# PearCoding/PearRay

Hardware: AMD Instinct MI355X
Metric: Msamples/s (higher is better)
Workload: dtype f32; 1 GPU; C4: Cornell box + 999968-triangle soup (1000000 triangles), 1920x1080, `direct` integrator (NEE+MIS+RR, depth 64), sobol 1024-spp schedule, hero wavelengths (spd CMIS), 308 iterations timed; parallelism=tiles1, collective=none (one rank)

## Files before the change

include/prgpu.h:

```cpp
#ifndef PRGPU_H
#define PRGPU_H

#include <stddef.h>
#include <stdint.h>

#ifdef __cplusplus
extern "C" {
#endif

#define PRGPU_API_VERSION 8
#define PRGPU_INVALID_ID 0xFFFFFFFFu

enum {
	PRGPU_OK          = 0,
	PRGPU_EINVAL      = -1,
	PRGPU_ENODEVICE   = -2,
	PRGPU_EDEVICE     = -3,
	PRGPU_EUNSUPPORTED = -4,
	PRGPU_EIO         = -5
};

enum { PRGPU_SPEC_CONST = 0, PRGPU_SPEC_PARAMETRIC = 1, PRGPU_SPEC_PARAMETRIC_SCALED = 2,
       PRGPU_SPEC_TABLE = 3, PRGPU_SPEC_MUL = 4, PRGPU_SPEC_SELLMEIER = 5, PRGPU_SPEC_CHECKER = 6 };

// ... 84 lines not shown
	float local_direction[3], local_right[3], local_up[3];
	float fstop, aperture_radius;
	uint32_t kind;
	float theta_start, theta_end, phi_start, phi_end;
	float fov;
	uint32_t fisheye_map;
	uint32_t clip_range;
	uint32_t reserved;
} prgpu_camera;

enum { PRGPU_SAMPLER_RANDOM = 0, PRGPU_SAMPLER_MJITT = 1, PRGPU_SAMPLER_SOBOL = 2, PRGPU_SAMPLER_HALTON = 3, PRGPU_SAMPLER_HAMMERSLEY = 4,
       PRGPU_SAMPLER_UNIFORM = 5,
       PRGPU_SAMPLER_STRATIFIED = 6 };
enum { PRGPU_MAPPER_SPD_CMIS = 0, PRGPU_MAPPER_RANDOM = 1, PRGPU_MAPPER_SPD_HERO = 2,
       PRGPU_MAPPER_CIE = 3,
       PRGPU_MAPPER_CIE_Y = 4,
       PRGPU_MAPPER_AGH_CMIS = 5,
       PRGPU_MAPPER_AGH_HERO = 6 };
enum { PRGPU_FILTER_BLOCK = 0, PRGPU_FILTER_TRIANGLE = 1, PRGPU_FILTER_GAUSSIAN = 2,
       PRGPU_FILTER_MITCHELL = 3, PRGPU_FILTER_LANCZOS = 4 };
enum { PRGPU_MIS_BALANCE = 0, PRGPU_MIS_POWER = 1 };

typedef struct prgpu_settings {
	uint32_t width, height;
	uint64_t seed;
	uint32_t aa_sampler;
	uint32_t aa_samples;
	uint32_t lens_samples, time_samples, spectral_samples;
	uint32_t mapper;
	uint32_t filter;
	uint32_t filter_radius;
	uint32_t max_ray_depth;
	uint32_t soft_max_ray_depth;
	uint32_t mis;
	uint32_t nee, direct, emissive_scatter;
	float    spectral_start, spectral_end;
	uint32_t spectral_hero;
	uint32_t spectral_mono;
	uint32_t aa_base_x, aa_base_y;
	uint32_t aa_burnin;
	uint32_t reserved;
} prgpu_settings;

typedef struct prgpu_scene_desc {
	uint32_t api_version;
	uint32_t n_vertices;
	const float*    positions;
	const float*    normals;
	const float*    uvs;
	uint32_t n_triangles;
	const uint32_t* indices;
	const uint32_t* tri_material;
	uint32_t n_entities;
	const prgpu_entity* entities;
	uint32_t n_materials;
	const prgpu_material* materials;
	uint32_t n_emissions;
	const prgpu_emission* emissions;
	uint32_t n_spectra;
	const prgpu_spectrum* spectra;
	uint32_t n_spectral_table_values;
	const float* spectral_tables;
	prgpu_camera   camera;
	prgpu_settings settings;
	uint32_t n_lights;
	const prgpu_light* lights;
} prgpu_scene_desc;

typedef struct prgpu_tile { uint32_t x0, y0, x1, y1; } prgpu_tile;

enum { PRGPU_STAT_CAMERA_RAYS = 0, PRGPU_STAT_LIGHT_RAYS, PRGPU_STAT_PRIMARY_RAYS, PRGPU_STAT_BOUNCE_RAYS,
       PRGPU_STAT_SHADOW_RAYS, PRGPU_STAT_MONOCHROME_RAYS, PRGPU_STAT_PIXEL_SAMPLES, PRGPU_STAT_ENTITY_HITS,
       PRGPU_STAT_BACKGROUND_HITS, PRGPU_STAT_CAMERA_DEPTH, PRGPU_STAT_LIGHT_DEPTH, PRGPU_STAT_COUNT };

typedef struct prgpu_trace_counters {
	uint64_t rays_closest, rays_any;
	uint64_t nodes_closest, leaves_closest;
	uint64_t nodes_any, leaves_any;
	uint32_t node_bytes, leaf_bytes;
	uint32_t ray_bytes, hit_bytes;
	uint64_t wave_steps_closest, wave_steps_any;
	uint64_t shade_batches, shade_lanes;
	uint64_t shade_ticks, idle_ticks, total_ticks;
} prgpu_trace_counters;

typedef struct prgpu_scene prgpu_scene;

const char* prgpu_last_error(void);
int  prgpu_device_count(void);
void prgpu_settings_default(prgpu_settings* s);

int  prgpu_rgb_to_coeffs(const float rgb[3], float coeffs[3]);
int  prgpu_write_rgb_coeff_table(const char* path, uint32_t resolution, int threads);

int  prgpu_scene_create(const prgpu_scene_desc* desc, int device, prgpu_scene** out);
void prgpu_scene_destroy(prgpu_scene* s);

int  prgpu_set_tiles(prgpu_scene* s, const prgpu_tile* tiles, uint32_t n_tiles);

int  prgpu_set_stream(prgpu_scene* s, void* hip_stream);

int  prgpu_bind_framebuffer(prgpu_scene* s, void* d_xyz, void* d_samples, void* d_feedback);

int  prgpu_render(prgpu_scene* s, uint32_t iter_begin, uint32_t iter_end);
int  prgpu_sync(prgpu_scene* s);

int  prgpu_download(prgpu_scene* s, float* xyz, uint32_t* samples, uint32_t* feedback);
int  prgpu_stats(prgpu_scene* s, uint64_t out[PRGPU_STAT_COUNT]);
int  prgpu_film_size(prgpu_scene* s, uint32_t* width, uint32_t* height);
int  prgpu_trace_counters_get(prgpu_scene* s, prgpu_trace_counters* out);
enum { PRGPU_KERNEL_NONE = 0, PRGPU_KERNEL_THROUGHPUT = 1, PRGPU_KERNEL_LATENCY = 2 };
typedef struct prgpu_pipeline_info {
	uint32_t mode;
	int32_t  shader_waves;
	float    shading_share;
	uint32_t calibration_launches;
	uint32_t kernel;
	uint32_t blocks, slots_per_block;
	uint64_t launches;
	uint32_t bvh_width;
	uint32_t bvh_top;
	uint32_t bvh_stack_bound;
	float    bvh_cost_4_wide, bvh_cost_6_wide;
} prgpu_pipeline_info;
int  prgpu_pipeline_info_get(prgpu_scene* s, prgpu_pipeline_info* out);
int  prgpu_set_instrumentation(prgpu_scene* s, int enabled);

int  prgpu_trace_closest(prgpu_scene* s, uint32_t n, const float* org, const float* dir,
                         const float* tmin, const float* tmax,
                         uint32_t* entity, uint32_t* prim, float* u, float* v, float* t);
int  prgpu_trace_any(prgpu_scene* s, uint32_t n, const float* org, const float* dir,
                     const float* tmin, const float* distance, uint8_t* occluded);

int  prgpu_download_primary_hits(prgpu_scene* s, uint32_t* entity, uint32_t* prim);

int  prgpu_set_timing(prgpu_scene* s, int enabled);
int  prgpu_kernel_time_ms(prgpu_scene* s, const char* family, double* total_ms, uint64_t* launches);

#define PRGPU_COMM_ID_BYTES 128
typedef struct prgpu_comm prgpu_comm;
int  prgpu_comm_unique_id(uint8_t id[PRGPU_COMM_ID_BYTES]);
int  prgpu_comm_create(const uint8_t id[PRGPU_COMM_ID_BYTES], int n_ranks, int rank, int device, prgpu_comm** out);
void prgpu_comm_destroy(prgpu_comm* comm);
int  prgpu_comm_size(const prgpu_comm* comm);
int  prgpu_comm_query(const prgpu_comm* comm, int* rccl_ranks, int* rccl_rank);
int  prgpu_reduce(prgpu_scene* s, prgpu_comm* comm, int root);
int  prgpu_reduced_planes(prgpu_scene* s, void** d_xyz, void** d_samples, void** d_feedback);

enum { PRGPU_AOV_POSITION = 0, PRGPU_AOV_NORMAL, PRGPU_AOV_NORMAL_G, PRGPU_AOV_TANGENT, PRGPU_AOV_BITANGENT, PRGPU_AOV_VIEW,
       PRGPU_AOV_ENTITY_ID, PRGPU_AOV_MATERIAL_ID, PRGPU_AOV_EMISSION_ID, PRGPU_AOV_DEPTH,
       PRGPU_AOV_COUNT };
int      prgpu_enable_aovs(prgpu_scene* s, uint32_t mask);
uint32_t prgpu_aov_channels(uint32_t aov);
int      prgpu_download_aov(prgpu_scene* s, uint32_t aov, float* out);
int prgpu_enable_variance(prgpu_scene* s);
int prgpu_download_variance(prgpu_scene* s, float* mean, float* variance);

#define PRGPU_LPE_MAX 4
#define PRGPU_LPE_MAX_STATES 32
int prgpu_lpe_check(const char* expression);
int prgpu_lpe_match(const char* expression, const uint8_t* symbols, uint32_t count);
int prgpu_enable_lpe(prgpu_scene* s, uint32_t n, const char* const* expressions);
int prgpu_download_lpe(prgpu_scene* s, uint32_t index, float* xyz);

int prgpu_enable_ambient_occlusion(prgpu_scene* s, uint32_t sample_count);
int prgpu_download_ao_counts(prgpu_scene* s, uint32_t* occluded);
int prgpu_download_ao_samples(prgpu_scene* s, uint64_t* rng_state, float* org, float* dir, uint8_t* occluded);

int prgpu_path_cost(prgpu_scene* s, uint32_t* vertices);
enum { PRGPU_TONE_SRGB = 0, PRGPU_TONE_XYZ = 1, PRGPU_TONE_XYZ_NORM = 2, PRGPU_TONE_LUMINANCE = 3 };
int prgpu_tonemap(uint32_t mode, float scale, const float* xyz, const float* weight, float* rgb, uint32_t out_elems, size_t pixel_count);
typedef struct prgpu_image_stats {
	uint64_t n;
	float min, min_ref, min_diff, max, max_ref, max_diff;
	float mean, mean_ref, mean_diff, mean_sqr, mean_sqr_ref;
	float mse, mape;
	uint64_t inf_count, nan_count;
} prgpu_image_stats;
int  prgpu_image_compare(const float* image, uint32_t image_stride, const float* reference, uint32_t reference_stride, uint32_t width,
                         uint32_t height, const uint32_t crop[4], prgpu_image_stats* out);
void prgpu_image_stats_merge(prgpu_image_stats* dst, const prgpu_image_stats* src);
enum { PRGPU_CHANNEL_SPECTRAL = 0, PRGPU_CHANNEL_3D = 1, PRGPU_CHANNEL_1D = 2, PRGPU_CHANNEL_COUNTER = 3 };
enum { PRGPU_SPECTRAL_OUTPUT = 0, PRGPU_SPECTRAL_ONLINE_MEAN = 1, PRGPU_SPECTRAL_ONLINE_VARIANCE = 2 };
enum { PRGPU_COUNTER_SAMPLES = 0, PRGPU_COUNTER_FEEDBACK = 1 };
typedef struct prgpu_output_channel {
	uint32_t file;
	uint32_t kind;
	uint32_t variable;
	uint32_t tone;
	char     name[64];
	char     lpe[64];
} prgpu_output_channel;
int prgpu_outputs_enable(prgpu_scene* s, const prgpu_output_channel* channels, uint32_t n_channels);
int prgpu_outputs_save(prgpu_scene* s, const prgpu_output_channel* channels, uint32_t n_channels, uint32_t file, const char* path);
int prgpu_write_exr(const char* path, uint32_t width, uint32_t height, uint32_t n_channels, const char* const* names,
                    const float* const* planes, const uint32_t* strides);

typedef struct prgpu_prc prgpu_prc;
typedef struct prgpu_prc_sky {
	const char*  light_name;
	const float* table;
	uint32_t     azimuth_count, elevation_count;
} prgpu_prc_sky;
typedef struct prgpu_prc_options {
	uint32_t width, height;
	uint32_t aa_samples;
// ... 33 lines not shown
```

pearray_amd/_cabi.py:

```python
import ctypes as C
import os

_HERE = os.path.dirname(os.path.abspath(__file__))
LIB_PATH = os.environ.get("PRGPU_LIBRARY") or os.path.join(_HERE, "csrc", "libprgpu.so")

PRGPU_API_VERSION = 8
INVALID_ID = 0xFFFFFFFF
COMM_ID_BYTES = 128

SPEC_CONST, SPEC_PARAMETRIC, SPEC_PARAMETRIC_SCALED, SPEC_TABLE, SPEC_MUL, SPEC_SELLMEIER, SPEC_CHECKER = range(7)
MAT_LAMBERT, MAT_DIELECTRIC, MAT_CONDUCTOR, MAT_ROUGH_CONDUCTOR, MAT_ROUGH_DIELECTRIC, MAT_PRINCIPLED, MAT_MIRROR = 0, 1, 2, 3, 4, 5, 6
MATF_ANISOTROPIC, MATF_NO_VNDF, MATF_HAS_TRANSMISSION = 1, 2, 4
PRINCIPLED_PARAMS = ("diffuse_transmission", "specular_transmission", "specular_tint", "anisotropic", "flatness", "metallic", "sheen",
                     "sheen_tint", "clearcoat", "clearcoat_gloss")
ENTITY_MESH, ENTITY_PLANE, ENTITY_SPHERE, ENTITY_QUADRIC = 0, 1, 2, 3
LIGHT_ENVIRONMENT, LIGHT_DISTANT, LIGHT_SKY, LIGHT_SUN, LIGHT_CIE_SKY = 0, 1, 2, 3, 4
ENVF_TEXTURED, ENVF_NO_DISTRIBUTION = 16, 32
SKYF_EXTEND, SKYF_COMPENSATION, SKYF_CLOUDY = 1, 2, 8
SKY_BANDS = 11
LPE_MAX, LPE_MAX_STATES = 4, 32
CAMERA_PERSPECTIVE, CAMERA_ORTHO, CAMERA_SPHERICAL, CAMERA_FISHEYE = 0, 1, 2, 3
FISHEYE_CIRCULAR, FISHEYE_CROPPED, FISHEYE_FULL = 0, 1, 2
AOV_NAMES = ("position", "normal", "normal_g", "tangent", "bitangent", "view", "entity_id", "material_id", "emission_id", "depth")
EMS_DIFFUSE = 0
SAMPLER_RANDOM, SAMPLER_MJITT, SAMPLER_SOBOL, SAMPLER_HALTON, SAMPLER_HAMMERSLEY, SAMPLER_UNIFORM, SAMPLER_STRATIFIED = range(7)
MAPPER_SPD_CMIS, MAPPER_RANDOM, MAPPER_SPD_HERO, MAPPER_CIE, MAPPER_CIE_Y, MAPPER_AGH_CMIS, MAPPER_AGH_HERO = range(7)
FILTER_BLOCK, FILTER_TRIANGLE, FILTER_GAUSSIAN, FILTER_MITCHELL, FILTER_LANCZOS = range(5)
MIS_BALANCE, MIS_POWER = range(2)
INTEGRATOR_DIRECT, INTEGRATOR_AO = range(2)

STAT_NAMES = ("camera_rays", "light_rays", "primary_rays", "bounce_rays", "shadow_rays", "monochrome_rays",
              "pixel_samples", "entity_hits", "background_hits", "camera_depth", "light_depth")
STAT_COUNT = len(STAT_NAMES)


class Spectrum(C.Structure):
    _fields_ = [("kind", C.c_uint32), ("p", C.c_float * 4), ("table_offset", C.c_uint32),
                ("table_count", C.c_uint32), ("wl_start", C.c_float), ("wl_end", C.c_float),
                ("lhs", C.c_uint32), ("rhs", C.c_uint32)]


class Material(C.Structure):
    _fields_ = [("kind", C.c_uint32), ("albedo", C.c_uint32), ("two_sided", C.c_uint32), ("ior", C.c_uint32),
                ("transmission", C.c_uint32), ("thin", C.c_uint32), ("k", C.c_uint32), ("flags", C.c_uint32),
                ("roughness_x", C.c_float), ("roughness_y", C.c_float), ("principled", C.c_float * 10)]


class Emission(C.Structure):
    _fields_ = [("kind", C.c_uint32), ("radiance", C.c_uint32)]


class Entity(C.Structure):
    _fields_ = [("first_tri", C.c_uint32), ("n_tris", C.c_uint32), ("emission", C.c_uint32),
                ("has_normals", C.c_uint32), ("kind", C.c_uint32), ("radius", C.c_float), ("has_uvs", C.c_uint32), ("params", C.c_uint32), ("transform", C.c_float * 16)]


class Light(C.Structure):
    _fields_ = [("kind", C.c_uint32), ("radiance", C.c_uint32), ("background", C.c_uint32), ("flags", C.c_uint32),
                ("direction", C.c_float * 3), ("cos_theta", C.c_float), ("transform", C.c_float * 16),
                ("table_offset", C.c_uint32), ("azimuth_count", C.c_uint32), ("elevation_count", C.c_uint32), ("ground_brightness", C.c_float)]


class Camera(C.Structure):
    _fields_ = [("transform", C.c_float * 16), ("width", C.c_float), ("height", C.c_float),
                ("near_t", C.c_float), ("far_t", C.c_float), ("local_direction", C.c_float * 3),
                ("local_right", C.c_float * 3), ("local_up", C.c_float * 3), ("fstop", C.c_float),
                ("aperture_radius", C.c_float), ("kind", C.c_uint32),
                ("theta_start", C.c_float), ("theta_end", C.c_float), ("phi_start", C.c_float), ("phi_end", C.c_float),
                ("fov", C.c_float), ("fisheye_map", C.c_uint32), ("clip_range", C.c_uint32), ("reserved", C.c_uint32)]


class Settings(C.Structure):
    _fields_ = [("width", C.c_uint32), ("height", C.c_uint32), ("seed", C.c_uint64),
                ("aa_sampler", C.c_uint32), ("aa_samples", C.c_uint32), ("lens_samples", C.c_uint32),
                ("time_samples", C.c_uint32), ("spectral_samples", C.c_uint32), ("mapper", C.c_uint32),
                ("filter", C.c_uint32), ("filter_radius", C.c_uint32), ("max_ray_depth", C.c_uint32),
                ("soft_max_ray_depth", C.c_uint32), ("mis", C.c_uint32), ("nee", C.c_uint32),
                ("direct", C.c_uint32), ("emissive_scatter", C.c_uint32), ("spectral_start", C.c_float),
                ("spectral_end", C.c_float), ("spectral_hero", C.c_uint32), ("spectral_mono", C.c_uint32),
                ("aa_base_x", C.c_uint32), ("aa_base_y", C.c_uint32), ("aa_burnin", C.c_uint32), ("reserved", C.c_uint32)]


class SceneDesc(C.Structure):
    _fields_ = [("api_version", C.c_uint32), ("n_vertices", C.c_uint32), ("positions", C.POINTER(C.c_float)),
                ("normals", C.POINTER(C.c_float)), ("uvs", C.POINTER(C.c_float)), ("n_triangles", C.c_uint32),
                ("indices", C.POINTER(C.c_uint32)), ("tri_material", C.POINTER(C.c_uint32)),
                ("n_entities", C.c_uint32), ("entities", C.POINTER(Entity)), ("n_materials", C.c_uint32),
                ("materials", C.POINTER(Material)), ("n_emissions", C.c_uint32),
                ("emissions", C.POINTER(Emission)), ("n_spectra", C.c_uint32), ("spectra", C.POINTER(Spectrum)),
                ("n_spectral_table_values", C.c_uint32), ("spectral_tables", C.POINTER(C.c_float)),
                ("camera", Camera), ("settings", Settings), ("n_lights", C.c_uint32), ("lights", C.POINTER(Light))]


class Tile(C.Structure):
    _fields_ = [("x0", C.c_uint32), ("y0", C.c_uint32), ("x1", C.c_uint32), ("y1", C.c_uint32)]


class TraceCounters(C.Structure):
    _fields_ = [("rays_closest", C.c_uint64), ("rays_any", C.c_uint64), ("nodes_closest", C.c_uint64),
                ("leaves_closest", C.c_uint64), ("nodes_any", C.c_uint64), ("leaves_any", C.c_uint64),
                ("node_bytes", C.c_uint32), ("leaf_bytes", C.c_uint32), ("ray_bytes", C.c_uint32),
                ("hit_bytes", C.c_uint32), ("wave_steps_closest", C.c_uint64), ("wave_steps_any", C.c_uint64),
                ("shade_batches", C.c_uint64), ("shade_lanes", C.c_uint64),
                ("shade_ticks", C.c_uint64), ("idle_ticks", C.c_uint64), ("total_ticks", C.c_uint64)]


class ImageStats(C.Structure):
    _fields_ = [("n", C.c_uint64), ("min", C.c_float), ("min_ref", C.c_float), ("min_diff", C.c_float), ("max", C.c_float),
                ("max_ref", C.c_float), ("max_diff", C.c_float), ("mean", C.c_float), ("mean_ref", C.c_float), ("mean_diff", C.c_float),
                ("mean_sqr", C.c_float), ("mean_sqr_ref", C.c_float), ("mse", C.c_float), ("mape", C.c_float),
                ("inf_count", C.c_uint64), ("nan_count", C.c_uint64)]


class OutputChannel(C.Structure):
    _fields_ = [("file", C.c_uint32), ("kind", C.c_uint32), ("variable", C.c_uint32), ("tone", C.c_uint32), ("name", C.c_char * 64),
                ("lpe", C.c_char * 64)]


CHANNEL_SPECTRAL, CHANNEL_3D, CHANNEL_1D, CHANNEL_COUNTER = range(4)
TONE_SRGB, TONE_XYZ, TONE_XYZ_NORM, TONE_LUMINANCE = range(4)


class PrcSky(C.Structure):
    _fields_ = [("light_name", C.c_char_p), ("table", C.POINTER(C.c_float)), ("azimuth_count", C.c_uint32), ("elevation_count", C.c_uint32)]


class PrcOptions(C.Structure):
    _fields_ = [("width", C.c_uint32), ("height", C.c_uint32), ("aa_samples", C.c_uint32), ("force_direct", C.c_uint32),
                ("seed", C.c_uint64), ("n_skies", C.c_uint32), ("reserved", C.c_uint32), ("skies", C.POINTER(PrcSky))]


def default_settings(width, height):
    s = Settings()
    s.width, s.height, s.seed = width, height, 42
    s.aa_sampler, s.aa_samples = SAMPLER_SOBOL, 128
    s.lens_samples = s.time_samples = s.spectral_samples = 1
    s.mapper, s.filter, s.filter_radius = MAPPER_SPD_CMIS, FILTER_MITCHELL, 1
    s.max_ray_depth, s.soft_max_ray_depth, s.mis = 64, 4, MIS_BALANCE
    s.nee = s.direct = s.emissive_scatter = 1
    s.spectral_start, s.spectral_end, s.spectral_hero, s.spectral_mono = 390.0, 830.0, 1, 0
    return s


class PipelineInfo(C.Structure):
    _fields_ = [("mode", C.c_uint32), ("shader_waves", C.c_int32), ("shading_share", C.c_float), ("calibration_launches", C.c_uint32),
                ("kernel", C.c_uint32), ("blocks", C.c_uint32), ("slots_per_block", C.c_uint32), ("launches", C.c_uint64),
                ("bvh_width", C.c_uint32), ("bvh_top", C.c_uint32), ("bvh_stack_bound", C.c_uint32), ("bvh_cost_4_wide", C.c_float), ("bvh_cost_6_wide", C.c_float)]


class SkyParams(C.Structure):
    _fields_ = [("sun_elevation", C.c_float), ("sun_azimuth", C.c_float), ("turbidity", C.c_float), ("albedo", C.c_float * 11)]


_VP, _U32P, _F32P, _U8P, _U64P = C.c_void_p, C.POINTER(C.c_uint32), C.POINTER(C.c_float), C.POINTER(C.c_uint8), C.POINTER(C.c_uint64)
SYMBOLS = {
    "prgpu_last_error": (C.c_char_p, []),
    "prgpu_device_count": (C.c_int, []),
    "prgpu_settings_default": (None, [C.POINTER(Settings)]),
    "prgpu_rgb_to_coeffs": (C.c_int, [_F32P, _F32P]),
    "prgpu_write_rgb_coeff_table": (C.c_int, [C.c_char_p, C.c_uint32, C.c_int]),
    "prgpu_scene_create": (C.c_int, [C.POINTER(SceneDesc), C.c_int, C.POINTER(_VP)]),
    "prgpu_scene_destroy": (None, [_VP]),
    "prgpu_set_tiles": (C.c_int, [_VP, C.POINTER(Tile), C.c_uint32]),
    "prgpu_set_stream": (C.c_int, [_VP, _VP]),
    "prgpu_bind_framebuffer": (C.c_int, [_VP, _VP, _VP, _VP]),
    "prgpu_render": (C.c_int, [_VP, C.c_uint32, C.c_uint32]),
    "prgpu_sync": (C.c_int, [_VP]),
    "prgpu_download": (C.c_int, [_VP, _F32P, _U32P, _U32P]),
    "prgpu_stats": (C.c_int, [_VP, _U64P]),
    "prgpu_trace_counters_get": (C.c_int, [_VP, C.POINTER(TraceCounters)]),
    "prgpu_set_instrumentation": (C.c_int, [_VP, C.c_int]),
    "prgpu_trace_closest": (C.c_int, [_VP, C.c_uint32, _F32P, _F32P, _F32P, _F32P, _U32P, _U32P, _F32P, _F32P, _F32P]),
    "prgpu_trace_any": (C.c_int, [_VP, C.c_uint32, _F32P, _F32P, _F32P, _F32P, _U8P]),
    "prgpu_download_primary_hits": (C.c_int, [_VP, _U32P, _U32P]),
    "prgpu_set_timing": (C.c_int, [_VP, C.c_int]),
    "prgpu_kernel_time_ms": (C.c_int, [_VP, C.c_char_p, C.POINTER(C.c_double), _U64P]),
    "prgpu_comm_unique_id": (C.c_int, [_U8P]),
    "prgpu_comm_create": (C.c_int, [_U8P, C.c_int, C.c_int, C.c_int, C.POINTER(_VP)]),
    "prgpu_comm_destroy": (None, [_VP]),
    "prgpu_comm_size": (C.c_int, [_VP]),
    "prgpu_comm_query": (C.c_int, [_VP, C.POINTER(C.c_int), C.POINTER(C.c_int)]),
    "prgpu_reduced_planes": (C.c_int, [_VP, C.POINTER(_VP), C.POINTER(_VP), C.POINTER(_VP)]),
    "prgpu_pipeline_info_get": (C.c_int, [_VP, C.POINTER(PipelineInfo)]),
    "prgpu_reduce": (C.c_int, [_VP, _VP, C.c_int]),
    "prgpu_film_size": (C.c_int, [_VP, _U32P, _U32P]),
    "prgpu_enable_variance": (C.c_int, [_VP]),
    "prgpu_download_variance": (C.c_int, [_VP, _F32P, _F32P]),
    "prgpu_path_cost": (C.c_int, [_VP, _U32P]),
    "prgpu_enable_ambient_occlusion": (C.c_int, [_VP, C.c_uint32]),
    "prgpu_download_ao_counts": (C.c_int, [_VP, _U32P]),
    "prgpu_download_ao_samples": (C.c_int, [_VP, _U64P, _F32P, _F32P, _U8P]),
    "prgpu_lpe_check": (C.c_int, [C.c_char_p]),
    "prgpu_lpe_match": (C.c_int, [C.c_char_p, _U8P, C.c_uint32]),
    "prgpu_enable_lpe": (C.c_int, [_VP, C.c_uint32, C.POINTER(C.c_char_p)]),
    "prgpu_download_lpe": (C.c_int, [_VP, C.c_uint32, _F32P]),
    "prgpu_image_compare": (C.c_int, [_F32P, C.c_uint32, _F32P, C.c_uint32, C.c_uint32, C.c_uint32, _U32P, C.POINTER(ImageStats)]),
    "prgpu_image_stats_merge": (None, [C.POINTER(ImageStats), C.POINTER(ImageStats)]),
    "prgpu_tonemap": (C.c_int, [C.c_uint32, C.c_float, _F32P, _F32P, _F32P, C.c_uint32, C.c_size_t]),
    "prgpu_outputs_enable": (C.c_int, [_VP, C.POINTER(OutputChannel), C.c_uint32]),
    "prgpu_outputs_save": (C.c_int, [_VP, C.POINTER(OutputChannel), C.c_uint32, C.c_uint32, C.c_char_p]),
    "prgpu_prc_outputs": (C.POINTER(OutputChannel), [_VP, _U32P]),
    "prgpu_prc_output_name": (C.c_char_p, [_VP, C.c_uint32]),
    "prgpu_enable_aovs": (C.c_int, [_VP, C.c_uint32]),
    "prgpu_aov_channels": (C.c_uint32, [C.c_uint32]),
    "prgpu_download_aov": (C.c_int, [_VP, C.c_uint32, _F32P]),
    "prgpu_write_exr": (C.c_int, [C.c_char_p, C.c_uint32, C.c_uint32, C.c_uint32, C.POINTER(C.c_char_p), C.POINTER(_F32P), _U32P]),
    "prgpu_sun_position": (None, [C.c_int] * 5 + [C.c_float] * 4 + [_F32P, _F32P]),
    "prgpu_sun_radiance": (C.c_float, [C.c_float] * 3),
    "prgpu_sky_table": (C.c_int, [C.c_float, C.c_float, C.c_float, _F32P, C.c_uint32, C.c_uint32, _F32P]),
    "prgpu_prc_sky_info": (C.c_int, [_VP, C.c_uint32, C.POINTER(SkyParams)]),
    "prgpu_prc_load_file": (C.c_int, [C.c_char_p, C.POINTER(PrcOptions), C.POINTER(_VP)]),
    "prgpu_prc_load_string": (C.c_int, [C.c_char_p, C.c_char_p, C.POINTER(PrcOptions), C.POINTER(_VP)]),
    "prgpu_prc_desc": (C.POINTER(SceneDesc), [_VP]),
    "prgpu_prc_warnings": (C.c_char_p, [_VP]),
    "prgpu_prc_integrator": (C.c_int, [_VP, _U32P, _U32P]),
    "prgpu_prc_last_error": (C.c_char_p, []),
    "prgpu_prc_free": (None, [_VP]),
}

_lib = None


def load():
    global _lib
    if _lib is not None:
        return _lib
    if not os.path.exists(LIB_PATH):
        raise ImportError("HIP backend %s not built -- run `python -c 'import __graft_entry__ as g; g.build()'` "
                          "(there is no CPU fallback)" % LIB_PATH)
    lib = C.CDLL(LIB_PATH)
# ... 15 lines not shown
```

pearray_amd/backend.py:

```python
import ctypes as C
import os

import numpy as np

from . import _cabi as abi


def _f32p(a):
    return a.ctypes.data_as(C.POINTER(C.c_float))


def _u32p(a):
    return a.ctypes.data_as(C.POINTER(C.c_uint32))


class RenderContext:

    def __init__(self, scene, device=0):
        self.lib = abi.load()
        self.scene = scene
        self._h = C.c_void_p()
        abi.check(self.lib.prgpu_scene_create(C.byref(scene.desc), int(device), C.byref(self._h)))
        self.width, self.height = scene.width, scene.height
        self.iterations_done = 0
        self.ao_sample_count = 0
        if getattr(scene, "integrator", abi.INTEGRATOR_DIRECT) == abi.INTEGRATOR_AO:
            self.enableAmbientOcclusion(scene.ao_sample_count)

    def close(self):
        if self._h:
            self.lib.prgpu_scene_destroy(self._h)
            self._h = C.c_void_p()

    def __del__(self):
        try:
            self.close()
        except Exception:
            pass

    def setTiles(self, tiles):
        tiles = list(tiles)
        arr = (abi.Tile * max(1, len(tiles)))(*[abi.Tile(*t) for t in tiles])
        abi.check(self.lib.prgpu_set_tiles(self._h, arr, len(tiles)))

    def setStream(self, stream_handle):
        abi.check(self.lib.prgpu_set_stream(self._h, C.c_void_p(stream_handle)))

    def bindFramebuffer(self, xyz_ptr, samples_ptr, feedback_ptr=None):
        abi.check(self.lib.prgpu_bind_framebuffer(self._h, C.c_void_p(xyz_ptr), C.c_void_p(samples_ptr),
                                                  C.c_void_p(feedback_ptr) if feedback_ptr else None))

    def reduce(self, comm, root=0):
        abi.check(self.lib.prgpu_reduce(self._h, comm._h, int(root)))

    def reducedPlanes(self):
        x, s, f = C.c_void_p(), C.c_void_p(), C.c_void_p()
        rc = self.lib.prgpu_reduced_planes(self._h, C.byref(x), C.byref(s), C.byref(f))
        if rc < 0:
            abi.check(rc)
        return (x.value, s.value, f.value) if rc == 1 else None

    def pipelineInfo(self):
        info = abi.PipelineInfo()
        abi.check(self.lib.prgpu_pipeline_info_get(self._h, C.byref(info)))
        out = {f: getattr(info, f) for f, _ in info._fields_}
        out["kernel"] = {0: "none", 1: "throughput", 2: "latency"}.get(out["kernel"], str(out["kernel"]))
        return out

    def setInstrumentation(self, on):
        abi.check(self.lib.prgpu_set_instrumentation(self._h, 1 if on else 0))

    def setTiming(self, on):
        abi.check(self.lib.prgpu_set_timing(self._h, 1 if on else 0))

    def render(self, iterations):
        b = self.iterations_done
        abi.check(self.lib.prgpu_render(self._h, b, b + int(iterations)))
        self.iterations_done = b + int(iterations)

    def start(self):
        self.render(self.scene.spp - self.iterations_done)

    def waitForFinish(self):
        abi.check(self.lib.prgpu_sync(self._h))

    def statistics(self):
        out = (C.c_uint64 * abi.STAT_COUNT)()
        abi.check(self.lib.prgpu_stats(self._h, out))
        return {n: int(out[i]) for i, n in enumerate(abi.STAT_NAMES)}

    def traceCounters(self):
        tc = abi.TraceCounters()
        abi.check(self.lib.prgpu_trace_counters_get(self._h, C.byref(tc)))
        return {f: int(getattr(tc, f)) for f, _ in tc._fields_}

    def kernelTime(self, family):
        ms, n = C.c_double(), C.c_uint64()
        abi.check(self.lib.prgpu_kernel_time_ms(self._h, family.encode(), C.byref(ms), C.byref(n)))
        return ms.value, int(n.value)

    def output(self):
        n = self.width * self.height
        xyz = np.empty(n * 3, dtype=np.float32)
        smp = np.empty(n, dtype=np.uint32)
        fb = np.empty(n, dtype=np.uint32)
        abi.check(self.lib.prgpu_download(self._h, _f32p(xyz), _u32p(smp), _u32p(fb)))
        return xyz.reshape(self.height, self.width, 3), smp.reshape(self.height, self.width), fb.reshape(self.height, self.width)

    def enableAOVs(self, names):
        mask = 0
        for n in names:
            mask |= 1 << abi.AOV_NAMES.index(n)
        abi.check(self.lib.prgpu_enable_aovs(self._h, mask))

    def enableVariance(self):
        abi.check(self.lib.prgpu_enable_variance(self._h))

    def variance(self):
        n = self.width * self.height * 3
        mean, var = np.empty(n, np.float32), np.empty(n, np.float32)
        abi.check(self.lib.prgpu_download_variance(self._h, _f32p(mean), _f32p(var)))
        return mean.reshape(self.height, self.width, 3), var.reshape(self.height, self.width, 3)

    def enableLPE(self, expressions):
        arr = (C.c_char_p * max(1, len(expressions)))(*[e.encode() for e in expressions])
        abi.check(self.lib.prgpu_enable_lpe(self._h, len(expressions), arr))

    def lpe(self, index):
        out = np.empty(self.width * self.height * 3, dtype=np.float32)
        abi.check(self.lib.prgpu_download_lpe(self._h, int(index), _f32p(out)))
        return out.reshape(self.height, self.width, 3)

    def enableAmbientOcclusion(self, sample_count):
        abi.check(self.lib.prgpu_enable_ambient_occlusion(self._h, int(sample_count)))
        self.ao_sample_count = int(sample_count)

    def aoCounts(self):
        out = np.empty(self.width * self.height, dtype=np.uint32)
        abi.check(self.lib.prgpu_download_ao_counts(self._h, _u32p(out)))
        return out.reshape(self.height, self.width)

    def aoSamples(self):
        n, k = self.width * self.height, self.ao_sample_count
        state = np.empty(n, dtype=np.uint64)
        org, direction = np.empty(n * k * 3, dtype=np.float32), np.empty(n * k * 3, dtype=np.float32)
        occ = np.empty(n * k, dtype=np.uint8)
        abi.check(self.lib.prgpu_download_ao_samples(self._h, state.ctypes.data_as(C.POINTER(C.c_uint64)), _f32p(org), _f32p(direction),
                                                     occ.ctypes.data_as(C.POINTER(C.c_uint8))))
# ... 187 lines not shown
```

pearray_amd/csrc/device/bvh.h:

```cpp
#pragma once
#include <string>
#include <vector>

#include "pr_device.h"

namespace prd {
struct BvhBuildInput {
	uint32_t n_tris, n_entities;
	const float* positions;
	const uint32_t* indices;
	const uint32_t* tri_entity;
	const DevEntity* entities;
	const uint8_t* tri_class = nullptr;
	uint32_t stack_capacity = 0xFFFFFFFFu;
	int width = 0;
	int top = -1;
	int parity = -1;
};
struct BvhBuildOutput {
	Rec64* recs = nullptr;
	uint32_t* leaf_units = nullptr;
	uint32_t n_inner = 0, n_leaf = 0, n_units = 0;
	uint32_t stack_bound = 0;
	int top = 0;
	bool wide = false;
	float cost4 = 0.0f, cost6 = 0.0f;
};
bool build_lbvh(const BvhBuildInput& in, BvhBuildOutput& out, hipStream_t stream, std::string& err);
}
```

pearray_amd/csrc/device/bvh.hip:

```cpp
#include "bvh.h"

#include <hipcub/hipcub.hpp>
#include <algorithm>
#include <cstring>

namespace prd {
namespace {

__device__ __forceinline__ uint32_t float_to_ordered(float f)
{
	const uint32_t b = __float_as_uint(f);
	return (b & 0x80000000u) ? ~b : (b | 0x80000000u);
}
__device__ __forceinline__ float ordered_to_float(uint32_t u)
{
	return __uint_as_float((u & 0x80000000u) ? (u & 0x7FFFFFFFu) : ~u);
}

__global__ void k_world_tris(uint32_t n, const float* __restrict__ positions, const uint32_t* __restrict__ indices,
							 const uint32_t* __restrict__ tri_entity, const DevEntity* __restrict__ entities,
							 float4* __restrict__ wv, uint32_t* __restrict__ ebounds )
{
	const uint32_t t = blockIdx.x * blockDim.x + threadIdx.x;
	if (t >= n)
// ... 259 lines not shown
	if (width <= 0) {
		for (int side = 0; side < 2; ++side) {
			const int c = side == 0 ? left[i] : right[i];
			bool expandable;
			const ChildRef direct = make_child(c, expandable, wv, sorted_tri, range_first, range_last, boxes, inner_idx, leaf_idx);
			if (!expandable || (width < 0 && i == 0)) {
				tmp[nc++] = direct;
			} else {
				bool e2;
				tmp[nc++] = make_child(left[c], e2, wv, sorted_tri, range_first, range_last, boxes, inner_idx, leaf_idx);
				tmp[nc++] = make_child(right[c], e2, wv, sorted_tri, range_first, range_last, boxes, inner_idx, leaf_idx);
			}
		}
	} else {
		bool ex[MAX_WIDE];
		tmp[0] = make_child(left[i], ex[0], wv, sorted_tri, range_first, range_last, boxes, inner_idx, leaf_idx);
		tmp[1] = make_child(right[i], ex[1], wv, sorted_tri, range_first, range_last, boxes, inner_idx, leaf_idx);
		nc	   = 2;
		while (nc < width) {
			int best	= -1;
			float bestA = -1.0f;
			for (int k = 0; k < nc; ++k) {
				const float A = half_area(tmp[k]);
				if (ex[k] && (A > bestA || (A == bestA && tmp[k].count > tmp[best].count))) {
					best  = k;
					bestA = A;
				}
			}
			if (best < 0)
				break;
			const int c = tmp[best].node;
			for (int k = nc; k > best + 1; --k) {
				tmp[k] = tmp[k - 1];
				ex[k]  = ex[k - 1];
			}
			tmp[best]	  = make_child(left[c], ex[best], wv, sorted_tri, range_first, range_last, boxes, inner_idx, leaf_idx);
			tmp[best + 1] = make_child(right[c], ex[best + 1], wv, sorted_tri, range_first, range_last, boxes, inner_idx, leaf_idx);
			++nc;
		}
	}
	int n = 0;
	for (int k = 0; k < nc; ++k)
		if (tmp[k].leaf)
			ch[n++] = tmp[k];
	for (int k = 0; k < nc; ++k)
		if (!tmp[k].leaf)
			ch[n++] = tmp[k];
	return nc;
}
__global__ void k_area_sum(int n, const uint32_t* __restrict__ flag, const float* __restrict__ boxes, double* __restrict__ sum)
{
	const int i = blockIdx.x * blockDim.x + threadIdx.x;
	double a	= 0.0;
	if (i < n - 1 && flag[i]) {
		const double dx = (double)boxes[6 * i + 3] - boxes[6 * i], dy = (double)boxes[6 * i + 4] - boxes[6 * i + 1], dz = (double)boxes[6 * i + 5] - boxes[6 * i + 2];
		a				= dx * dy + dy * dz + dz * dx;
	}
	for (int o = 32; o > 0; o >>= 1)
		a += __shfl_down(a, o, 64);
	if ((threadIdx.x & 63) == 0 && a != 0.0)
		atomicAdd(sum, a);
}
__global__ void k_mark_records(int n_front, const int* __restrict__ front, int width, const float4* __restrict__ wv, const uint32_t* __restrict__ sorted_tri,
							   const int* __restrict__ left, const int* __restrict__ right, const int* __restrict__ range_first, const int* __restrict__ range_last,
							   const float* __restrict__ boxes, uint32_t* __restrict__ inner_flag, int* __restrict__ next, uint32_t* __restrict__ n_next,
							   uint32_t* __restrict__ stack_bound , uint32_t* __restrict__ max_stack_bound)
{
	const int t = blockIdx.x * blockDim.x + threadIdx.x;
	if (t >= n_front)
		return;
	ChildRef ch[MAX_WIDE];
	const int nc = gather_children(front[t], ch, width, wv, sorted_tri, left, right, range_first, range_last, boxes, inner_flag , inner_flag);
	const uint32_t below = stack_bound[front[t]] + (uint32_t)(nc - 1);
	atomicMax(max_stack_bound, below);
	for (int k = 0; k < nc; ++k)
		if (!ch[k].leaf) {
			inner_flag[ch[k].node]		= 1u;
			stack_bound[ch[k].node]		= below;
			next[atomicAdd(n_next, 1u)] = ch[k].node;
		}
}

constexpr double GRID_MARGIN = 1.0 / 16384.0;
__device__ void write_inner_q(Rec64* __restrict__ rec, const ChildRef* ch, int nc, uint32_t base_unit, const uint32_t* offs)
{
	float org[3];
	uint32_t ebyte[3];
	uint32_t qlo[3][MAX_WIDE], qhi[3][MAX_WIDE];
	for (int a = 0; a < 3; ++a) {
		float lo = INFINITY, hi = -INFINITY;
		for (int k = 0; k < nc; ++k) {
			lo = fminf(lo, ch[k].lo[a]);
			hi = fmaxf(hi, ch[k].hi[a]);
		}
		const float ext_eff = (hi - lo) + 4.0f * fmaxf(fabsf(lo), fabsf(hi)) * 1.1920929e-7f;
		int e				= (int)fminf(fmaxf((float)ilogbf(fmaxf(ext_eff * (1.0f / 255.0f), 1e-30f)), -100.0f), 30.0f);
		bool fits			= false;
		float o				= lo;
		for (; e <= 30 && !fits; ++e) {
			const double s = ldexp(1.0, e), m = s * GRID_MARGIN;
			o = (float)((double)lo - m);
			if ((double)o > (double)lo - m)
				o = nextafterf(o, -INFINITY);
			fits = true;
			for (int k = 0; k < nc; ++k) {
				const double want_lo = (double)ch[k].lo[a] - m, want_hi = (double)ch[k].hi[a] + m;
				double ql = floor((want_lo - (double)o) / s);
				ql		  = ql < 0.0 ? 0.0 : (ql > 255.0 ? 255.0 : ql);
				while (ql > 0.0 && (double)o + ql * s > want_lo)
					ql -= 1.0;
				double qh = ceil((want_hi - (double)o) / s);
				qh		  = qh < 0.0 ? 0.0 : qh;
				while (qh <= 255.0 && (double)o + qh * s < want_hi)
					qh += 1.0;
				if (qh > 255.0 || (double)o + ql * s > want_lo) {
					fits = false;
					break;
				}
				qlo[a][k] = (uint32_t)ql;
				qhi[a][k] = (uint32_t)qh;
			}
		}
		--e;
		if (!fits)
			for (int k = 0; k < nc; ++k) {
				qlo[a][k] = 0u;
				qhi[a][k] = 255u;
			}
		org[a]	 = o;
		ebyte[a] = (uint32_t)(e + 127);
	}
	uint32_t w[16];
	for (int k = 0; k < 16; ++k)
		w[k] = 0u;
	w[0] = __float_as_uint(org[0]);
	w[1] = __float_as_uint(org[1]);
	w[2] = __float_as_uint(org[2]);
	w[3] = ebyte[0] | (ebyte[1] << 8) | (ebyte[2] << 16);
	for (int k = 0; k < 4; ++k) {
		const bool used = k < nc;
		for (int a = 0; a < 3; ++a) {
			const uint32_t l = used ? qlo[a][k] : 255u, h = used ? qhi[a][k] : 0u;
			w[4 + a] |= l << (8 * k);
			w[7 + a] |= h << (8 * k);
		}
		const int src = used ? k : 0;
		w[11] |= ((offs[src] << REC_UNIT_SHIFT) | (ch[src].leaf ? REC_LEAF_BIT : 0u)) << (8 * k);
	}
	w[10]	   = base_unit << REC_UNIT_SHIFT;
	for (int k = 4; k < 6; ++k) {
		const bool used = k < nc;
		const int j		= k - 4;
		const uint32_t lx = used ? qlo[0][k] : 255u, ly = used ? qlo[1][k] : 255u, lz = used ? qlo[2][k] : 255u;
		const uint32_t hx = used ? qhi[0][k] : 0u, hy = used ? qhi[1][k] : 0u, hz = used ? qhi[2][k] : 0u;
		w[12] |= (lx << (8 * j)) | (ly << (16 + 8 * j));
		w[13] |= (hx << (8 * j)) | (hy << (16 + 8 * j));
		w[14] |= (lz << (8 * j)) | (hz << (16 + 8 * j));
		const int src = used ? k : 0;
		w[15] |= ((offs[src] << REC_UNIT_SHIFT) | (ch[src].leaf ? REC_LEAF_BIT : 0u)) << (8 * j);
	}
	uint4* dst = reinterpret_cast<uint4*>(rec);
	for (int q = 0; q < 4; ++q)
		dst[q] = make_uint4(w[4 * q], w[4 * q + 1], w[4 * q + 2], w[4 * q + 3]);
}

__global__ void k_group_sizes(int n, int width, const float4* __restrict__ wv, const uint32_t* __restrict__ sorted_tri, const int* __restrict__ left,
							  const int* __restrict__ right, const int* __restrict__ range_first, const int* __restrict__ range_last,
							  const float* __restrict__ boxes, const uint32_t* __restrict__ inner_flag, const uint32_t* __restrict__ inner_idx,
							  const uint32_t* __restrict__ leaf_idx, uint32_t* __restrict__ gsize)
{
	const int i = blockIdx.x * blockDim.x + threadIdx.x;
	if (i >= n - 1 || !inner_flag[i])
		return;
	ChildRef ch[MAX_WIDE];
	const int nc = gather_children(i, ch, width, wv, sorted_tri, left, right, range_first, range_last, boxes, inner_idx, leaf_idx);
	uint32_t units = 0;
	for (int k = 0; k < nc; ++k)
		units += ch[k].leaf ? 2u : 1u;
	gsize[inner_idx[i]] = (units + 1u) & ~1u;
}
__global__ void k_assign_units(int n, int width, const float4* __restrict__ wv, const uint32_t* __restrict__ sorted_tri, const int* __restrict__ left,
							   const int* __restrict__ right, const int* __restrict__ range_first, const int* __restrict__ range_last,
							   const float* __restrict__ boxes, const uint32_t* __restrict__ inner_flag, const uint32_t* __restrict__ inner_idx,
							   const uint32_t* __restrict__ leaf_idx, const uint32_t* __restrict__ gbase, uint32_t* __restrict__ inner_unit,
							   uint32_t* __restrict__ leaf_unit)
{
	const int i = blockIdx.x * blockDim.x + threadIdx.x;
	if (i >= n - 1 || !inner_flag[i])
		return;
	if (i == 0)
		inner_unit[inner_idx[0]] = 0u;
	ChildRef ch[MAX_WIDE];
	const int nc  = gather_children(i, ch, width, wv, sorted_tri, left, right, range_first, range_last, boxes, inner_idx, leaf_idx);
	uint32_t unit = 2u + gbase[inner_idx[i]];
	for (int k = 0; k < nc; ++k) {
		if (ch[k].leaf)
			leaf_unit[ch[k].id] = unit;
		else
			inner_unit[ch[k].id] = unit;
		unit += ch[k].leaf ? 2u : 1u;
	}
}
__global__ void k_emit_inner(int n, int width, const float4* __restrict__ wv, const uint32_t* __restrict__ sorted_tri, const int* __restrict__ left,
							 const int* __restrict__ right, const int* __restrict__ range_first, const int* __restrict__ range_last,
							 const float* __restrict__ boxes, const uint32_t* __restrict__ inner_flag, const uint32_t* __restrict__ inner_idx,
							 const uint32_t* __restrict__ leaf_idx, const uint32_t* __restrict__ gbase, const uint32_t* __restrict__ inner_unit,
							 Rec64* __restrict__ recs)
{
	const int i = blockIdx.x * blockDim.x + threadIdx.x;
	if (i >= n - 1 || !inner_flag[i])
		return;
	ChildRef ch[MAX_WIDE];
	const int nc = gather_children(i, ch, width, wv, sorted_tri, left, right, range_first, range_last, boxes, inner_idx, leaf_idx);
	uint32_t offs[MAX_WIDE] = { 0u, 0u, 0u, 0u, 0u, 0u }, off = 0u;
	for (int k = 0; k < nc; ++k) {
		offs[k] = off;
		off += ch[k].leaf ? 2u : 1u;
	}
	write_inner_q(recs + inner_unit[inner_idx[i]], ch, nc, 2u + gbase[inner_idx[i]], offs);
}

__global__ void k_validate(uint32_t n_inner, const uint32_t* __restrict__ inner_unit, const Rec64* __restrict__ recs, uint32_t n_units, uint32_t* __restrict__ bad)
{
	const uint32_t i = blockIdx.x * blockDim.x + threadIdx.x;
	if (i >= n_inner)
		return;
	const uint32_t unit = inner_unit[i];
	if (unit >= n_units) {
		atomicAdd(bad, 1u);
		return;
	}
	const uint32_t* w	= reinterpret_cast<const uint32_t*>(recs + unit);
	const uint32_t base = w[10], pw = w[11];
	bool ok				= (base & 3u) == 0u && base >= (2u << REC_UNIT_SHIFT);
	for (int a = 0; a < 3 && ok; ++a) {
		const uint32_t e = (w[3] >> (8 * a)) & 0xFFu;
		ok				 = e >= 27u && e <= 157u;
	}
	for (int k = 0; k < MAX_WIDE && ok; ++k) {
		const uint32_t ref = base + (((k < 4 ? pw : w[15]) >> (8 * (k & 3))) & 0xFFu), cu = ref >> REC_UNIT_SHIFT;
		ok				   = ok && (ref & 2u) == 0u;
		if (ref & REC_LEAF_BIT) {
			ok = (cu & 1u) == 0u && cu + 2u <= n_units;
			if (ok) {
				const uint32_t cnt = reinterpret_cast<const uint32_t*>(recs + cu)[30];
				ok				   = cnt >= 1u && cnt <= 3u;
			}
		} else {
			ok = cu + 1u <= n_units;
			if (ok) {
				const uint32_t ce = reinterpret_cast<const uint32_t*>(recs + cu)[3] & 0xFFu;
				ok				  = ce >= 27u && ce <= 157u;
			}
		}
	}
	if (!ok)
		atomicAdd(bad, 1u);
}

__global__ void k_emit_leaves(uint32_t n, const float4* __restrict__ wv, const uint32_t* __restrict__ sorted_tri, const uint32_t* __restrict__ leaf_flag,
							  const uint32_t* __restrict__ leaf_count, const uint32_t* __restrict__ leaf_idx, const uint32_t* __restrict__ leaf_unit, Rec64* __restrict__ recs,
							  const uint8_t* __restrict__ tri_class)
{
	const uint32_t pos = blockIdx.x * blockDim.x + threadIdx.x;
	if (pos >= n || !leaf_flag[pos])
		return;
	const uint32_t cnt = leaf_count[pos];
	float f[32];
	for (int k = 0; k < 32; ++k)
		f[k] = 0.0f;
	uint32_t classes = 0u;
	for (uint32_t k = 0; k < cnt; ++k) {
		const uint32_t t = sorted_tri[pos + k];
		classes |= (tri_class ? (uint32_t)tri_class[t] : 0u) << (8u * k);
		if (wv[3 * t].w != 0.0f) {
			const float4 c = wv[3 * t + 2];
			f[10 * k]	   = c.x;
			f[10 * k + 1]  = c.y;
			f[10 * k + 2]  = c.z;
			f[10 * k + 3]  = c.w;
			f[10 * k + 9]  = __uint_as_float(t | PRIM_SPHERE_BIT);
			continue;
		}
		for (int v = 0; v < 3; ++v) {
			const float4 p		 = wv[3 * t + v];
			f[10 * k + 3 * v]	 = p.x;
			f[10 * k + 3 * v + 1] = p.y;
			f[10 * k + 3 * v + 2] = p.z;
		}
		f[10 * k + 9] = __uint_as_float(t);
	}
	f[30]		= __uint_as_float(cnt);
	f[31]		= __uint_as_float(classes);
	float4* dst = reinterpret_cast<float4*>(recs + leaf_unit[leaf_idx[pos]]);
	for (int q = 0; q < 8; ++q)
		dst[q] = make_float4(f[4 * q], f[4 * q + 1], f[4 * q + 2], f[4 * q + 3]);
}

__global__ void k_tiny_scene(uint32_t n, const float4* __restrict__ wv, const uint32_t* __restrict__ sorted_tri, Rec64* __restrict__ recs, uint32_t* __restrict__ leaf_unit,
							 const uint8_t* __restrict__ tri_class)
{
	if (blockIdx.x != 0 || threadIdx.x != 0)
		return;
	float lo[3] = { INFINITY, INFINITY, INFINITY }, hi[3] = { -INFINITY, -INFINITY, -INFINITY };
	float leaf[32];
	for (int k = 0; k < 32; ++k)
		leaf[k] = 0.0f;
	uint32_t classes = 0u;
	for (uint32_t i = 0; i < n; ++i) {
		float a[3], b[3];
		const uint32_t t = sorted_tri[i];
		classes |= (tri_class ? (uint32_t)tri_class[t] : 0u) << (8u * i);
		tri_box(wv, t, a, b);
		for (int k = 0; k < 3; ++k) {
			lo[k] = fminf(lo[k], a[k]);
			hi[k] = fmaxf(hi[k], b[k]);
		}
		if (wv[3 * t].w != 0.0f) {
			const float4 c	 = wv[3 * t + 2];
			leaf[10 * i]	 = c.x;
			leaf[10 * i + 1] = c.y;
			leaf[10 * i + 2] = c.z;
			leaf[10 * i + 3] = c.w;
			leaf[10 * i + 9] = __uint_as_float(t | PRIM_SPHERE_BIT);
			continue;
		}
		for (int v = 0; v < 3; ++v) {
			const float4 p		  = wv[3 * t + v];
			leaf[10 * i + 3 * v]	  = p.x;
			leaf[10 * i + 3 * v + 1] = p.y;
			leaf[10 * i + 3 * v + 2] = p.z;
		}
		leaf[10 * i + 9] = __uint_as_float(t);
	}
	leaf[30] = __uint_as_float(n);
	leaf[31] = __uint_as_float(classes);
	pad_box(lo, hi);
	ChildRef only;
	for (int a = 0; a < 3; ++a) {
		only.lo[a] = lo[a];
		only.hi[a] = hi[a];
	}
	only.leaf			 = true;
	only.id				 = 0u;
	const uint32_t off0[4] = { 0u, 0u, 0u, 0u };
	write_inner_q(recs, &only, 1, 2u, off0);
	leaf_unit[0] = 2u;
	float4* d1	 = reinterpret_cast<float4*>(recs + 2);
	for (int q = 0; q < 8; ++q)
		d1[q] = make_float4(leaf[4 * q], leaf[4 * q + 1], leaf[4 * q + 2], leaf[4 * q + 3]);
}

#define HIPC(x)                                  \
	do {                                         \
		hipError_t _e = (x);                     \
		if (_e != hipSuccess) {                  \
			err = std::string(#x) + ": " + hipGetErrorString(_e); \
			goto done;                           \
		}                                        \
	} while (0)

}

namespace {
struct EntityBox {
	float lo[3], hi[3];
	double weight;
	uint32_t id;
};
void entity_codes_split(std::vector<EntityBox>& set, size_t first, size_t count, uint32_t prefix, int bits_left, std::vector<uint32_t>& code)
{
	if (count == 1 || bits_left == 0) {
		for (size_t k = 0; k < count; ++k)
			code[set[first + k].id] = prefix;
		return;
	}
	const size_t cap = size_t(1) << (bits_left - 1);
	double best_cost = INFINITY;
	int best_axis	 = 0;
	size_t best_left = count / 2;
	std::vector<double> right_area(count), right_weight(count);
	for (int axis = 0; axis < 3; ++axis) {
		std::sort(set.begin() + first, set.begin() + first + count,
				  [axis](const EntityBox& a, const EntityBox& b) { return a.lo[axis] + a.hi[axis] < b.lo[axis] + b.hi[axis] || (a.lo[axis] + a.hi[axis] == b.lo[axis] + b.hi[axis] && a.id < b.id); });
		auto area = [](const float* lo, const float* hi) {
			const double dx = (double)hi[0] - lo[0], dy = (double)hi[1] - lo[1], dz = (double)hi[2] - lo[2];
			return dx * dy + dy * dz + dz * dx;
		};
		float lo[3] = { INFINITY, INFINITY, INFINITY }, hi[3] = { -INFINITY, -INFINITY, -INFINITY };
		double w = 0.0;
		for (size_t k = count; k-- > 1;) {
			for (int a = 0; a < 3; ++a) {
				lo[a] = std::min(lo[a], set[first + k].lo[a]);
				hi[a] = std::max(hi[a], set[first + k].hi[a]);
			}
			w += set[first + k].weight;
			right_area[k]	= area(lo, hi);
			right_weight[k] = w;
		}
		for (int a = 0; a < 3; ++a) {
			lo[a] = INFINITY;
			hi[a] = -INFINITY;
		}
		w = 0.0;
		for (size_t k = 1; k < count; ++k) {
			for (int a = 0; a < 3; ++a) {
				lo[a] = std::min(lo[a], set[first + k - 1].lo[a]);
				hi[a] = std::max(hi[a], set[first + k - 1].hi[a]);
			}
			w += set[first + k - 1].weight;
			if (k > cap || count - k > cap)
				continue;
			const double cost = area(lo, hi) * w + right_area[k] * right_weight[k];
			if (cost < best_cost) {
				best_cost = cost;
				best_axis = axis;
				best_left = k;
			}
		}
	}
	size_t heavy = 0;
	for (size_t k = 1; k < count; ++k)
		if (set[first + k].weight > set[first + heavy].weight)
			heavy = k;
	{
		auto area = [](const float* lo, const float* hi) {
			const double dx = (double)hi[0] - lo[0], dy = (double)hi[1] - lo[1], dz = (double)hi[2] - lo[2];
// ... 192 lines not shown
				const uint32_t one = 1u;
				const int root	   = 0;
				HIPC(hipMemcpyAsync(greedy_flag, &one, 4, hipMemcpyHostToDevice, stream));
				HIPC(hipMemcpyAsync(front, &root, 4, hipMemcpyHostToDevice, stream));
				uint32_t n_front = 1u;
				while (n_front != 0u) {
					HIPC(hipMemsetAsync(front_count, 0, sizeof(uint32_t), stream));
					hipLaunchKernelGGL(k_mark_records, dim3((n_front + B - 1) / B), dim3(B), 0, stream, (int)n_front, front, MAX_WIDE, wv, vals_sorted, left, right, rf, rl, boxes,
									   greedy_flag, front_next, front_count, stack_bound, bounds_dev + 2);
					HIPC(hipMemcpyAsync(&n_front, front_count, 4, hipMemcpyDeviceToHost, stream));
					HIPC(hipStreamSynchronize(stream));
					std::swap(front, front_next);
				}
				hipLaunchKernelGGL(k_area_sum, dim3(G), dim3(B), 0, stream, (int)n, greedy_flag, boxes, area_sums + 2);
			}
			{
				double sums[3] = { 0.0, 0.0, 0.0 };
				float root_box[6];
				hipLaunchKernelGGL(k_area_sum, dim3(G), dim3(B), 0, stream, (int)n, inner_flag, boxes, area_sums);
				hipLaunchKernelGGL(k_area_sum, dim3(G), dim3(B), 0, stream, (int)n, odd_flag, boxes, area_sums + 1);
				HIPC(hipMemcpyAsync(bounds_host, bounds_dev, sizeof(bounds_host), hipMemcpyDeviceToHost, stream));
				HIPC(hipMemcpyAsync(sums, area_sums, sizeof(sums), hipMemcpyDeviceToHost, stream));
				HIPC(hipMemcpyAsync(root_box, boxes, sizeof(root_box), hipMemcpyDeviceToHost, stream));
				HIPC(hipStreamSynchronize(stream));
				const double rx = (double)root_box[3] - root_box[0], ry = (double)root_box[4] - root_box[1], rz = (double)root_box[5] - root_box[2];
				const double ra = std::max(rx * ry + ry * rz + rz * rx, 1e-300);
				const uint32_t bound_even = 3u * (bounds_host[0] + 1u), bound_odd = 3u * (bounds_host[1] + 1u), bound6 = bounds_host[2];
				const bool fit_even = bound_even <= in.stack_capacity, fit_odd = bound_odd <= in.stack_capacity;
				const bool odd = in.parity >= 0 ? in.parity == 1 : fit_odd && (!fit_even || sums[1] < sums[0]);
				const uint32_t bound4 = odd ? bound_odd : bound_even;
				if (in.parity >= 0 && in.width != 6 && bound4 > in.stack_capacity) {
					err = "the four-wide BVH of the forced parity is " + std::to_string(bound4) + " stack entries deep in the worst case, the traversal stack holds "
						  + std::to_string(in.stack_capacity);
					goto done;
				}
				if (odd) {
					width = -1;
					std::swap(inner_flag, odd_flag);
				}
				out.cost4		= (float)(sums[odd ? 1 : 0] / ra);
				out.stack_bound = bound4;
				if (in.width != 4) {
					out.cost6 = (float)(sums[2] / ra);
					const bool fit4 = bound4 <= in.stack_capacity, fit6 = bound6 <= in.stack_capacity;
					const bool cheaper6 = (double)out.cost6 * WIDE_STEP_COST < (double)out.cost4;
					if (in.width == 6 || (cheaper6 ? (fit6 || !fit4) : (!fit4 && fit6))) {
						out.stack_bound = bound6;
						width			= MAX_WIDE;
						out.wide		= true;
						std::swap(inner_flag, greedy_flag);
					}
				}
			}
			{
				const double cost = out.stack_bound > in.stack_capacity ? INFINITY
																		: (out.wide ? (double)out.cost6 * WIDE_STEP_COST : (double)out.cost4);
				if (pass < n_orders && (pass == 0 ? cost < best_cost : cost < 0.98 * first_cost && cost < best_cost)) {
					best_cost  = cost;
					best_order = order;
				}
				if (pass == 0)
					first_cost = cost;
				if (top_forced)
					break;
				if (pass + 1 < n_orders) {
					order = pass + 1;
					continue;
				}
				if (pass + 1 == n_orders && best_order != order) {
					order = best_order;
					continue;
				}
				break;
			}
		}
		if (n <= 3) {
			HIPC(hipMalloc(&out.recs, sizeof(Rec64) * 4));
			HIPC(hipMemsetAsync(out.recs, 0, sizeof(Rec64) * 4, stream));
			HIPC(hipMalloc(&out.leaf_units, sizeof(uint32_t)));
			hipLaunchKernelGGL(k_tiny_scene, dim3(1), dim3(64), 0, stream, n, wv, vals_sorted, out.recs, out.leaf_units, in.tri_class);
			out.n_inner = 1;
			out.n_leaf	= 1;
			out.n_units = 4;
		} else {
			HIPC(hipcub::DeviceScan::ExclusiveSum(nullptr, t2a, inner_flag, inner_idx, (int)n, stream));
			HIPC(hipcub::DeviceScan::ExclusiveSum(nullptr, t2b, leaf_flag, leaf_idx, (int)n, stream));
			temp2_bytes = std::max(t2a, t2b);
			HIPC(hipMalloc(&temp2, temp2_bytes));
			HIPC(hipcub::DeviceScan::ExclusiveSum(temp2, temp2_bytes, inner_flag, inner_idx, (int)n, stream));
			HIPC(hipcub::DeviceScan::ExclusiveSum(temp2, temp2_bytes, leaf_flag, leaf_idx, (int)n, stream));
			uint32_t last[4] = { 0, 0, 0, 0 };
			HIPC(hipMemcpyAsync(&last[0], inner_idx + (n - 1), 4, hipMemcpyDeviceToHost, stream));
			HIPC(hipMemcpyAsync(&last[1], inner_flag + (n - 1), 4, hipMemcpyDeviceToHost, stream));
			HIPC(hipMemcpyAsync(&last[2], leaf_idx + (n - 1), 4, hipMemcpyDeviceToHost, stream));
			HIPC(hipMemcpyAsync(&last[3], leaf_flag + (n - 1), 4, hipMemcpyDeviceToHost, stream));
			HIPC(hipStreamSynchronize(stream));
			if (out.stack_bound > in.stack_capacity) {
				err = "the BVH of this scene is " + std::to_string(out.stack_bound) + " stack entries deep in the worst case, the traversal stack holds "
					  + std::to_string(in.stack_capacity);
				goto done;
			}
			out.n_inner = last[0] + last[1];
			out.n_leaf	= last[2] + last[3];
			HIPC(hipMalloc(&gsize, sizeof(uint32_t) * (size_t(out.n_inner) + 1)));
			HIPC(hipMalloc(&gbase, sizeof(uint32_t) * (size_t(out.n_inner) + 1)));
			HIPC(hipMalloc(&inner_unit, sizeof(uint32_t) * std::max<size_t>(out.n_inner, 1)));
			HIPC(hipMalloc(&out.leaf_units, sizeof(uint32_t) * std::max<size_t>(out.n_leaf, 1)));
			HIPC(hipMemsetAsync(gsize, 0, sizeof(uint32_t) * (size_t(out.n_inner) + 1), stream));
			hipLaunchKernelGGL(k_group_sizes, dim3(G), dim3(B), 0, stream, (int)n, width, wv, vals_sorted, left, right, rf, rl, boxes, inner_flag, inner_idx, leaf_idx, gsize);
			HIPC(hipGetLastError());
			{
				size_t t3 = 0;
				HIPC(hipcub::DeviceScan::ExclusiveSum(nullptr, t3, gsize, gbase, (int)out.n_inner + 1, stream));
				if (t3 > temp2_bytes) {
					(void)hipFree(temp2);
					temp2 = nullptr;
					HIPC(hipMalloc(&temp2, t3));
					temp2_bytes = t3;
				}
				HIPC(hipcub::DeviceScan::ExclusiveSum(temp2, temp2_bytes, gsize, gbase, (int)out.n_inner + 1, stream));
			}
			uint32_t group_units = 0;
			HIPC(hipMemcpyAsync(&group_units, gbase + out.n_inner, 4, hipMemcpyDeviceToHost, stream));
			HIPC(hipStreamSynchronize(stream));
			out.n_units = 2u + group_units;
			if (size_t(out.n_units) >= (size_t(1) << 30)) {
				err = "the BVH needs more than 2^30 record units";
				goto done;
			}
			HIPC(hipMalloc(&out.recs, sizeof(Rec64) * size_t(out.n_units)));
			HIPC(hipMemsetAsync(out.recs, 0, sizeof(Rec64) * size_t(out.n_units), stream));
			hipLaunchKernelGGL(k_assign_units, dim3(G), dim3(B), 0, stream, (int)n, width, wv, vals_sorted, left, right, rf, rl, boxes, inner_flag, inner_idx, leaf_idx, gbase,
							   inner_unit, out.leaf_units);
			hipLaunchKernelGGL(k_emit_inner, dim3(G), dim3(B), 0, stream, (int)n, width, wv, vals_sorted, left, right, rf, rl, boxes, inner_flag, inner_idx, leaf_idx, gbase,
							   inner_unit, out.recs);
			hipLaunchKernelGGL(k_emit_leaves, dim3(G), dim3(B), 0, stream, n, wv, vals_sorted, leaf_flag, leaf_cnt, leaf_idx, out.leaf_units, out.recs, in.tri_class);
			HIPC(hipGetLastError());
			{
				uint32_t bad = 0;
				HIPC(hipMemsetAsync(gsize, 0, sizeof(uint32_t), stream));
				hipLaunchKernelGGL(k_validate, dim3((out.n_inner + B - 1) / B), dim3(B), 0, stream, out.n_inner, inner_unit, out.recs, out.n_units, gsize);
				HIPC(hipMemcpyAsync(&bad, gsize, 4, hipMemcpyDeviceToHost, stream));
				HIPC(hipStreamSynchronize(stream));
				if (bad != 0u) {
					err = "internal error: " + std::to_string(bad) + " inner records failed the structure check";
					goto done;
				}
			}
		}
		HIPC(hipGetLastError());
		HIPC(hipStreamSynchronize(stream));
		ok = true;
	}
done:
	(void)hipFree(wv); (void)hipFree(ebounds); (void)hipFree(entity_rank); (void)hipFree(keys); (void)hipFree(keys_sorted); (void)hipFree(vals); (void)hipFree(vals_sorted);
	(void)hipFree(left); (void)hipFree(right); (void)hipFree(rf); (void)hipFree(rl); (void)hipFree(parent); (void)hipFree(boxes); (void)hipFree(arrive);
	(void)hipFree(inner_flag); (void)hipFree(inner_idx); (void)hipFree(leaf_flag); (void)hipFree(leaf_cnt); (void)hipFree(leaf_idx);
	(void)hipFree(front); (void)hipFree(front_next); (void)hipFree(front_count); (void)hipFree(area_sums); (void)hipFree(greedy_flag); (void)hipFree(stack_bound); (void)hipFree(bounds_dev); (void)hipFree(odd_flag);
	(void)hipFree(temp); (void)hipFree(temp2); (void)hipFree(gsize); (void)hipFree(gbase); (void)hipFree(inner_unit);
	if (!ok) {
		(void)hipFree(out.recs);
		(void)hipFree(out.leaf_units);
		out.recs	   = nullptr;
		out.leaf_units = nullptr;
	}
	return ok;
}

}
```

pearray_amd/csrc/device/pr_device.h:

```cpp
#pragma once

#include <hip/hip_runtime.h>
#include <stdint.h>

#include "../../../include/prgpu.h"

#ifndef PR_INLINE_CLOSURES
#define PR_INLINE_CLOSURES 0
#endif

#if PR_INLINE_CLOSURES
#define PR_CLOSURE __forceinline__
#else
#define PR_CLOSURE __noinline__
#endif

namespace prd {

constexpr float PR_EPS		= 1.1920928955078125e-7f;
constexpr float PR_INV_PI_F = 0.31830988618379067154f;
constexpr float PR_PI_F	  = 3.14159265358979323846f;
constexpr uint32_t INVALID	= PRGPU_INVALID_ID;
constexpr float SHADOW_RAY_MIN = 0.0001f;
constexpr float BOUNCE_RAY_MIN = 0.0001f;
constexpr float DISTANCE_EPS   = 1e-5f;
constexpr float GEOMETRY_EPS   = 1e-5f;
constexpr float PDF_EPS		   = 1e-6f;
constexpr int CIE_SAMPLES	   = 441;
constexpr float CIE_START	   = 390.0f;
constexpr float CIE_END		   = 830.0f;
constexpr float CIE_Y_NORM_SUM = 113.042314572337f;
constexpr float CIE_RANGE	   = CIE_END - CIE_START;
constexpr float CIE_DELTA	   = CIE_RANGE / (CIE_SAMPLES - 1);
constexpr float CIE_Y_NORM	   = CIE_Y_NORM_SUM * CIE_DELTA;

struct __attribute__((aligned(64))) Rec64 {
	float4 q[4];
};
static_assert(sizeof(Rec64) == 64, "Rec64 must be 64 bytes");
constexpr uint32_t REC_LEAF_BIT = 1u;
constexpr uint32_t REC_EMPTY	= 0xFFFFFFFFu;
constexpr uint32_t REC_UNIT_SHIFT = 2u;
__host__ __device__ __forceinline__ const float4* rec_ptr(const Rec64* recs, uint32_t ref)
{
	return reinterpret_cast<const float4*>(reinterpret_cast<const char*>(recs) + (size_t(ref & ~3u) << 4));
}
constexpr float SLAB_REL		= 1.0000028610229492f;
constexpr float INV_D_MAX		= 1.2089258196146292e24f;
constexpr float SCENE_COORD_MAX = 268435456.0f;

struct DevEntity {
	float m[12];
	float nm[9];
	uint32_t first_tri, n_tris, emission, has_normals;
	float vol_scale, world_area;
	uint32_t light_id, kind;
	float sphere_r;
	uint32_t has_uvs;
};

constexpr uint32_t FEAT_DELTA_MATERIALS = 1u, FEAT_INFINITE_LIGHTS = 2u, FEAT_PLANES = 4u, FEAT_SPHERES = 8u, FEAT_AOVS = 16u, FEAT_SHAPE_LIGHTS = 32u, FEAT_TEXTURES = 64u,
				   FEAT_ROUGH_MATERIALS = 128u, FEAT_LPE = 256u, FEAT_QUADRICS = 512u, FEAT_ALL = 1023u;

struct DevQuadric {
	float p[10];
	float lo[3], hi[3];
	float wlo[3], whi[3];
	float inv[12];
	uint32_t tri;
	uint32_t entity;
};

struct DevShapeLight {
	float S[3], Ex[3], Ey[3], Ez[3], nrm[3];
	float width, height;
	float inv[12];
	float pdf_cache;
	float radius;
	float pad[2];
};
struct __attribute__((aligned(128))) DevLight {
	float m[12];
	float nm[9];
	uint32_t entity, kind, n_tris, tri_offset;
	uint32_t has_normals, radiance;
	float vol_scale;
	prgpu_spectrum node, lhs, rhs;
	uint32_t pad[3];
};
static_assert(sizeof(DevLight) == 256, "DevLight must be two 128-byte lines");
struct __attribute__((aligned(128))) DevMaterial {
	prgpu_material m;
	prgpu_spectrum albedo;
};
static_assert(sizeof(DevMaterial) == 128, "DevMaterial must be one 128-byte line");
constexpr uint32_t LIGHT_TRI_FLOATS = 20;
constexpr uint32_t PRIM_SPHERE_BIT = 0x40000000u;

struct DevInfLight {
	uint32_t kind, radiance, background, flags;
	float nm[9], inv_nm[9];
	float outgoing[3];
	float dx[3], dy[3];
	float cos_theta, cone_pdf;
	uint32_t table_offset, az_count, el_count;
	uint32_t dist_offset, dist_w, dist_h;
	float ground_brightness;
};
constexpr int SKY_BANDS			 = PRGPU_SKY_BANDS;
constexpr float SKY_BAND_START	 = 320.0f;
constexpr float SKY_BAND_DELTA	 = 40.0f;
constexpr float ELEVATION_RANGE = PR_PI_F * 0.5f;
constexpr float AZIMUTH_RANGE	 = PR_PI_F * 2;

struct DevCamera {
	float o[3], right[3], up[3], focal[3], xap[3], yap[3];
	float near_t, far_t;
	uint32_t dof, ortho;
	uint32_t kind;
	float angles[4];
	float fov, xaspect, yaspect;
	uint32_t clip;
};

struct DevScene {
	const Rec64* recs;
	uint32_t n_tris, n_inner, n_leaf;
	uint32_t bvh_wide;
	const float* positions;
// ... 1192 lines not shown
```

pearray_amd/csrc/device/render.h:

```cpp
#pragma once
#include "pr_device.h"

namespace prd {
constexpr int N_DEVICE_COUNTERS = PRGPU_STAT_COUNT + 30;

struct TraceWorkspace {
	uint32_t* queue_head = nullptr;
	uint2* spill		 = nullptr;
	uint32_t max_blocks	 = 0;
	int refill_below	 = 44;
	uint32_t* bl_list	 = nullptr;
	uint32_t* bl_word	 = nullptr;
	uint32_t* slot_unit	 = nullptr;
	size_t bl_entries	 = 0;
};
size_t trace_workspace_spill_entries(uint32_t max_blocks);
uint32_t trace_stack_capacity();

void launch_raygen(const DevScene& sc, const PathState& ps, uint32_t slot_base, uint32_t n_slots, uint32_t iter, unsigned long long* gstats, hipStream_t st);
void launch_trace_closest(const DevScene& sc, const PathState& ps, const uint32_t* active, uint32_t slot_base, uint32_t n_active, bool count,
						  const TraceWorkspace& ws, uint32_t* shade_counters, unsigned long long* gstats, hipStream_t st);
void launch_shade(const DevScene& sc, const PathState& ps, const uint32_t* active, uint32_t slot_base, uint32_t n_active, uint32_t* next_active,
				  uint32_t* counters, uint32_t* dead_list, uint32_t* queue_head_closest, uint32_t* queue_head_shadow, unsigned long long* gstats,
				  hipStream_t st);
void launch_regen(const DevScene& sc, const PathState& ps, const uint32_t* dead, uint32_t n_dead, uint32_t iter_end, uint32_t* next_active,
				  uint32_t* counters, unsigned long long* gstats, hipStream_t st);
void launch_trace_shadow(const DevScene& sc, const PathState& ps, uint32_t n_items, bool count, const TraceWorkspace& ws, unsigned long long* gstats,
						 hipStream_t st);
struct PersistentGeometry {
	uint32_t n_blocks, slots_per_block;
};
PersistentGeometry persistent_geometry(uint32_t n_owned, uint32_t max_blocks, uint32_t max_slots_per_block);
uint32_t persistent_slot_padding();
uint32_t slot_array_padding();
uint32_t persistent_block_threads();
int shade_ticks_counter();
struct PersistentTuning {
	uint32_t slots	  = 384;
	int shade_min	  = 64;
	int shade_partial = 16;
	int fin_batch	  = 16;
	int occupancy	  = 3;
	int shader_wave	  = -1;
	bool resident	  = true;
};
void launch_path_persistent(const DevScene& sc, const PathState& ps, const uint32_t* owned, uint32_t n_owned, uint32_t iter_begin, uint32_t iter_end,
							bool count, const TraceWorkspace& ws, const PersistentTuning& tune, int shader_waves , uint32_t* next_pixel, uint32_t* error,
							unsigned long long* gstats, hipStream_t st);
struct LatencyGeometry {
	uint32_t n_blocks, slots_per_wave, total_slots;
};
struct LatencyTuning {
	uint32_t slots_per_wave = 256;
	int shade_min			= 48;
	int refill_below		= 40;
};
LatencyGeometry latency_geometry(uint32_t n_owned, uint32_t max_blocks_throughput, uint32_t max_slots_per_wave);
bool latency_variant_built(uint32_t features);
void launch_path_latency(const DevScene& sc, const PathState& ps, const uint32_t* owned, uint32_t n_owned, uint32_t iter_begin, uint32_t iter_end, bool count,
						 const TraceWorkspace& ws, const LatencyTuning& tune, uint32_t* error, unsigned long long* gstats, hipStream_t st);
void launch_resolve(const DevScene& sc, const PathState& ps, uint32_t iter, hipStream_t st);
size_t sort_active_temp_bytes(uint32_t n_max);
void launch_sort_active(const DevScene& sc, const PathState& ps, const uint32_t* active, uint32_t n, uint32_t* keys_in, uint32_t* keys_out, uint32_t* active_out,
						void* temp, size_t temp_bytes, hipStream_t st);
void launch_service_closest(const DevScene& sc, uint32_t n, const float* org, const float* dir, const float* tmin, const float* tmax,
							uint32_t* entity, uint32_t* prim, float* u, float* v, float* t, const TraceWorkspace& ws, unsigned long long* gstats,
							hipStream_t st);
void launch_tri_slot(const DevScene& sc, const uint32_t* leaf_units , uint32_t* tri_slot, hipStream_t st);
void launch_service_closest_split(const DevScene& sc, uint32_t n, const float* org, const float* dir, const float* tmin, const float* tmax,
								  uint32_t* entity, uint32_t* prim, float* u, float* v, float* t, const TraceWorkspace& ws, uint32_t* tri_slot,
								  unsigned long long* gstats, hipStream_t st);
void launch_service_any(const DevScene& sc, uint32_t n, const float* org, const float* dir, const float* tmin, const float* distance,
						uint8_t* occluded, const TraceWorkspace& ws, unsigned long long* gstats, hipStream_t st);
struct AoState {
	float4* rec;
	uint32_t* occluded;
	const uint64_t* jump;
	uint32_t* counts;
	uint64_t jump_all;
	uint32_t sample_count;
	uint64_t* dbg_state;
	float* dbg_org;
	float* dbg_dir;
	uint8_t* dbg_occluded;
};

void launch_ao_hits(const DevScene& sc, const PathState& ps, const AoState& ao, uint32_t n_slots, bool instrumented, uint32_t* n_hits, uint32_t* queue_head_closest,
// ... 7 lines not shown
```

pearray_amd/csrc/device/render.hip:

```cpp
#ifndef PR_TU
#error "compile with -DPR_TU=0..5 or 11..15 (see the Makefile)"
#endif
#include "render.h"

#include <algorithm>
#if PR_TU == 0
#include <hipcub/hipcub.hpp>
#endif

namespace prd {

__device__ __forceinline__ unsigned long long lane_ballot(bool p) { return __builtin_amdgcn_ballot_w64(p); }
__device__ __forceinline__ bool lane_in(unsigned long long m) { return __builtin_amdgcn_inverse_ballot_w64(m); }
__device__ __forceinline__ int wave_popc(unsigned long long m)
{
	int n = __builtin_popcountll(m);
	asm volatile("" : "+s"(n));
	return n;
}

struct Hit {
	float t, u, v;
	uint32_t tri;
};

enum { CNT_NODES_CLOSEST = PRGPU_STAT_COUNT, CNT_TRIS_CLOSEST, CNT_NODES_ANY, CNT_TRIS_ANY, CNT_WAVE_ITERS_CLOSEST, CNT_WAVE_ITERS_ANY, CNT_SHADE_BATCHES, CNT_SHADE_LANES, CNT_SHADE_TICKS, CNT_IDLE_TICKS, CNT_TOTAL_TICKS, CNT_LEAF_TICKS, CNT_INNER_TICKS, CNT_TOTAL_CYCLES, CNT_REFILL_TICKS, CNT_FIN_TICKS, CNT_CAMERA_TICKS, CNT_VERTEX_TICKS,
	   CNT_CLS_TICKS0, CNT_CLS_BATCHES0 = CNT_CLS_TICKS0 + 4, CNT_CLS_LANES0 = CNT_CLS_BATCHES0 + 4 };

#ifndef PR_PEEK
#define PR_PEEK 0
#endif
#ifndef PR_PL_VARIANTS
#define PR_PL_VARIANTS 31
#endif
#ifndef PR_PP_BLOCK
#define PR_PP_BLOCK 256
#endif
constexpr int PP_BLOCK		= PR_PP_BLOCK;
constexpr int TRAV_BLOCK	= PR_TU >= 1 ? PP_BLOCK : 256;
constexpr int STACK_LDS		= 16;
constexpr int STACK_SPILL	= 64;

struct Stack {
	uint2* lds;
	uint2* spill;
	uint32_t spill_stride;
	int sp, base;
	__device__ __forceinline__ void reset() { sp = base = 0; }
	__device__ __forceinline__ void reserve(int k)
	{
		while (sp - base + k > STACK_LDS) {
			if (base < STACK_SPILL)
				spill[(uint32_t)base * spill_stride] = lds[(base & (STACK_LDS - 1)) * TRAV_BLOCK];
			++base;
		}
	}
	__device__ __forceinline__ void push_if(bool valid, uint32_t ref, uint32_t key)
	{
		lds[(sp & (STACK_LDS - 1)) * TRAV_BLOCK] = make_uint2(ref, key);
		sp += valid ? 1 : 0;
	}
	__device__ __forceinline__ uint2 peek() const { return lds[((sp - 1) & (STACK_LDS - 1)) * TRAV_BLOCK]; }
	__device__ __forceinline__ uint2 pop_peeked(uint2 top)
	{
		--sp;
		if (__builtin_expect(sp < base, 0)) {
			base = sp;
			top	 = make_uint2(REC_EMPTY, 0x7F800000u);
			if (sp < STACK_SPILL)
				top = spill[(uint32_t)sp * spill_stride];
		}
		return top;
	}
	__device__ __forceinline__ uint2 pop()
	{
		--sp;
		uint2 e = lds[(sp & (STACK_LDS - 1)) * TRAV_BLOCK];
		if (__builtin_expect(sp < base, 0)) {
			base = sp;
			e	 = make_uint2(REC_EMPTY, 0x7F800000u);
			if (sp < STACK_SPILL)
				e = spill[(uint32_t)sp * spill_stride];
		}
		return e;
	}
};
static_assert((STACK_LDS & (STACK_LDS - 1)) == 0, "STACK_LDS must be a power of two");

struct Trav {
	RayPre r;
	float tmin;
	Hit best;
	uint32_t cur;
	bool any;
	uint32_t cls;
};

enum { MODE_CLOSEST = 0, MODE_ANY = 1, MODE_MIXED = 2 };

template <typename STK>
__device__ __forceinline__ void trav_begin(Trav& s, STK& st, V3 o, V3 d, float tmin, float tmax, float eps_t)
{
	s.r	   = ray_prepare(o, d, eps_t);
	s.tmin = tmin + 0.0f;
	s.best = Hit{ tmax, 0.0f, 0.0f, INVALID };
	s.cur  = 0u;
	s.any  = false;
	s.cls  = 0u;
	st.reset();
}
// ... 13 lines not shown
			s.cur = e.x;
	}
}

#define PR_UB(w, k) ((float)(((w) >> (8 * (k))) & 0xFFu))
__device__ __forceinline__ void inner_keys(const Trav& s, const float4& q0, const float4& q1, const float4& q2, const float4& q3, bool wide, uint32_t key[6])
{
	const uint32_t eb = __float_as_uint(q0.w);
	const float sx = __uint_as_float((eb & 0xFFu) << 23), sy = __uint_as_float(((eb >> 8) & 0xFFu) << 23), sz = __uint_as_float(((eb >> 16) & 0xFFu) << 23);
	const bool nx = s.r.inv_d.x < 0.0f, ny = s.r.inv_d.y < 0.0f, nz = s.r.inv_d.z < 0.0f;
	const uint32_t wlx = __float_as_uint(q1.x), wly = __float_as_uint(q1.y), wlz = __float_as_uint(q1.z);
	const uint32_t whx = __float_as_uint(q1.w), why = __float_as_uint(q2.x), whz = __float_as_uint(q2.y);
	const uint32_t wnx = nx ? whx : wlx, wfx = nx ? wlx : whx, wny = ny ? why : wly, wfy = ny ? wly : why, wnz = nz ? whz : wlz, wfz = nz ? wlz : whz;
	const float Ax = sx * s.r.inv_d.x, Ay = sy * s.r.inv_d.y, Az = sz * s.r.inv_d.z;
	const float Bx = (q0.x - s.r.o.x) * s.r.inv_d.x, By = (q0.y - s.r.o.y) * s.r.inv_d.y, Bz = (q0.z - s.r.o.z) * s.r.inv_d.z;
	const uint32_t pw = __float_as_uint(q2.w);
#pragma unroll
	for (int k = 0; k < 4; ++k) {
		const float axk = __fmaf_rn(PR_UB(wnx, k), Ax, Bx), bxk = __fmaf_rn(PR_UB(wfx, k), Ax, Bx);
		const float ayk = __fmaf_rn(PR_UB(wny, k), Ay, By), byk = __fmaf_rn(PR_UB(wfy, k), Ay, By);
		const float azk = __fmaf_rn(PR_UB(wnz, k), Az, Bz), bzk = __fmaf_rn(PR_UB(wfz, k), Az, Bz);
		const float t0 = fmaxf(fmaxf(axk, ayk), fmaxf(azk, s.tmin));
		const float t1 = fminf(fminf(bxk, byk), fminf(bzk, s.best.t));
		const bool h   = t0 <= __fmaf_rn(t1, SLAB_REL, s.r.eps_t);
		key[k] = h ? __builtin_amdgcn_perm(__float_as_uint(t0), pw, 0x07060500u | (uint32_t)k) : 0xFFFFFFFFu;
	}
	if (wide) {
		const uint32_t ea = __float_as_uint(q3.x), eh = __float_as_uint(q3.y), ez = __float_as_uint(q3.z), pw2 = __float_as_uint(q3.w);
		const uint32_t enx = nx ? eh : ea, efx = nx ? ea : eh, eny = ny ? eh : ea, efy = ny ? ea : eh;
		const uint32_t ezn = nz ? (ez >> 16) : ez, ezf = nz ? ez : (ez >> 16);
#pragma unroll
		for (int k = 0; k < 2; ++k) {
			const float axk = __fmaf_rn(PR_UB(enx, k), Ax, Bx), bxk = __fmaf_rn(PR_UB(efx, k), Ax, Bx);
			const float ayk = __fmaf_rn(PR_UB(eny, 2 + k), Ay, By), byk = __fmaf_rn(PR_UB(efy, 2 + k), Ay, By);
			const float azk = __fmaf_rn(PR_UB(ezn, k), Az, Bz), bzk = __fmaf_rn(PR_UB(ezf, k), Az, Bz);
			const float t0 = fmaxf(fmaxf(axk, ayk), fmaxf(azk, s.tmin));
			const float t1 = fminf(fminf(bxk, byk), fminf(bzk, s.best.t));
			const bool h   = t0 <= __fmaf_rn(t1, SLAB_REL, s.r.eps_t);
			key[4 + k]	   = h ? __builtin_amdgcn_perm(__float_as_uint(t0), pw2, 0x07060500u | (uint32_t)k) : 0xFFFFFFFFu;
		}
	}
}
template <int M, typename STK>
__device__ __forceinline__ void trav_inner_rec(Trav& s, STK& st, const float4& q0, const float4& q1, const float4& q2, const float4& q3, bool wide, const uint2* top = nullptr)
{
	uint32_t key[6];
	inner_keys(s, q0, q1, q2, q3, wide, key);
#define PR_CSWAP(a, b)                                  \
	{                                                   \
		const uint32_t lo = min(key[a], key[b]);        \
		key[b]			  = max(key[a], key[b]);        \
		key[a]			  = lo;                         \
	}
	const uint32_t base = __float_as_uint(q2.z);
	if (wide) {
		PR_CSWAP(0, 5) PR_CSWAP(1, 3) PR_CSWAP(2, 4) PR_CSWAP(1, 2) PR_CSWAP(3, 4) PR_CSWAP(0, 3) PR_CSWAP(2, 5) PR_CSWAP(0, 1) PR_CSWAP(2, 3) PR_CSWAP(4, 5) PR_CSWAP(1, 2) PR_CSWAP(3, 4)
		st.reserve(5);
		st.push_if(key[5] != 0xFFFFFFFFu, base + (key[5] & 0xFFu), key[5]);
		st.push_if(key[4] != 0xFFFFFFFFu, base + (key[4] & 0xFFu), key[4]);
	} else {
		PR_CSWAP(0, 1) PR_CSWAP(2, 3) PR_CSWAP(0, 2) PR_CSWAP(1, 3) PR_CSWAP(1, 2)
		st.reserve(3);
	}
#undef PR_CSWAP
	st.push_if(key[3] != 0xFFFFFFFFu, base + (key[3] & 0xFFu), key[3]);
	st.push_if(key[2] != 0xFFFFFFFFu, base + (key[2] & 0xFFu), key[2]);
	st.push_if(key[1] != 0xFFFFFFFFu, base + (key[1] & 0xFFu), key[1]);
	s.cur = key[0] != 0xFFFFFFFFu ? base + (key[0] & 0xFFu) : REC_EMPTY;
	trav_pop<M>(s, st, top);
}
template <int M>
__device__ __forceinline__ void trav_inner(const DevScene& sc, Trav& s, Stack& st)
{
	const float4* __restrict__ rec = rec_ptr(sc.recs, s.cur);
	const float4 q0 = rec[0], q1 = rec[1], q2 = rec[2];
	const bool wide = sc.bvh_wide != 0u;
	float4 q3		= make_float4(0.0f, 0.0f, 0.0f, 0.0f);
	if (wide)
		q3 = rec[3];
	const uint2 top = st.peek();
	trav_inner_rec<M>(s, st, q0, q1, q2, q3, wide, &top);
}

template <int M, bool SPH, bool CLS = false>
__device__ __forceinline__ void leaf_test(Trav& s, const float4& q0, const float4& q1, const float4& q2, const float4& q3, const float4& q4, const float4& q5,
										  const float4& q6, const float4& q7)
{
	const bool ANY = M == MODE_ANY || (M == MODE_MIXED && s.any);
	const float f[32] = { q0.x, q0.y, q0.z, q0.w, q1.x, q1.y, q1.z, q1.w, q2.x, q2.y, q2.z, q2.w, q3.x, q3.y, q3.z, q3.w,
						  q4.x, q4.y, q4.z, q4.w, q5.x, q5.y, q5.z, q5.w, q6.x, q6.y, q6.z, q6.w, q7.x, q7.y, q7.z, q7.w };
	const uint32_t count = __float_as_uint(f[30]);
#pragma unroll
	for (int k = 0; k < 3; ++k) {
		if ((uint32_t)k < count) {
			float t, u, v;
			const uint32_t prim = __float_as_uint(f[10 * k + 9]);
			bool hit;
			if (SPH && (prim & PRIM_SPHERE_BIT)) {
				u = v = 0.0f;
				hit	  = sphere_hit(s.r, v3(f[10 * k], f[10 * k + 1], f[10 * k + 2]), f[10 * k + 3], s.tmin, s.best.t, t);
			} else {
				hit = woop(s.r, v3(f[10 * k], f[10 * k + 1], f[10 * k + 2]), v3(f[10 * k + 3], f[10 * k + 4], f[10 * k + 5]),
						   v3(f[10 * k + 6], f[10 * k + 7], f[10 * k + 8]), t, u, v)
					  && t > s.tmin;
			}
			if (hit) {
				const uint32_t tri = prim & ~PRIM_SPHERE_BIT;
				if (ANY) {
					if (t <= s.best.t)
						s.best.tri = tri;
				} else if (t < s.best.t || (t == s.best.t && tri < s.best.tri)) {
					s.best = Hit{ t, u, v, tri };
					if (CLS)
						s.cls = (__float_as_uint(f[31]) >> (8 * k)) & 0xFFu;
				}
			}
		}
	}
}
template <int M, bool SPH, bool CLS = false, typename STK>
__device__ __forceinline__ void trav_leaf_rec(Trav& s, STK& st, const float4& q0, const float4& q1, const float4& q2, const float4& q3, const float4& q4,
											  const float4& q5, const float4& q6, const float4& q7, const uint2* top = nullptr)
{
	const bool ANY = M == MODE_ANY || (M == MODE_MIXED && s.any);
	leaf_test<M, SPH, CLS>(s, q0, q1, q2, q3, q4, q5, q6, q7);
	s.cur = REC_EMPTY;
	if (ANY && s.best.tri != INVALID) {
		st.reset();
		return;
	}
	trav_pop<M>(s, st, top);
}
template <int M>
__device__ __forceinline__ void trav_leaf(const DevScene& sc, Trav& s, Stack& st)
{
	const float4* __restrict__ rec = rec_ptr(sc.recs, s.cur);
	const float4 q0 = rec[0], q1 = rec[1], q2 = rec[2], q3 = rec[3], q4 = rec[4], q5 = rec[5], q6 = rec[6], q7 = rec[7];
	const uint2 top = st.peek();
	trav_leaf_rec<M, true>(s, st, q0, q1, q2, q3, q4, q5, q6, q7, &top);
}

template <bool CLS>
__device__ __forceinline__ void trav_quadrics(const DevScene& sc, Trav& s, bool any)
{
	for (uint32_t k = 0; k < sc.n_quadrics; ++k) {
		const DevQuadric& Q = sc.quadrics[k];
		float tq;
		if (quadric_hit(Q, sc.entities[Q.entity].m, s.r.o, s.r.d, s.tmin, s.best.t, any, tq)) {
			if (any) {
				s.best.tri = Q.tri;
				s.best.t   = -INFINITY;
				break;
			}
			if (tq < s.best.t || (tq == s.best.t && Q.tri < s.best.tri)) {
				s.best = Hit{ tq, 0.0f, 0.0f, Q.tri };
				if (CLS)
					s.cls = sc.tri_class[Q.tri];
			}
		}
	}
}

template <bool ANY, bool COUNT, typename LoadF, typename StoreF>
__device__ __forceinline__ void trace_persistent(const DevScene& sc, uint32_t n_rays, uint32_t* queue_head, uint2* spill, int refill_below, LoadF load,
												 StoreF store, unsigned long long* gstats)
{
	__shared__ uint2 lds_stack[STACK_LDS * TRAV_BLOCK];
	Stack st;
	st.lds			= lds_stack + threadIdx.x;
	st.spill_stride = gridDim.x * TRAV_BLOCK;
	st.spill		= spill + (blockIdx.x * TRAV_BLOCK + threadIdx.x);
	st.reset();
	Trav s;
	s.cur			   = REC_EMPTY;
	uint32_t my_ray	   = 0;
	bool has_ray	   = false;
	bool exhausted	   = false;
	uint32_t cn = 0, cl = 0, witers = 0;
	const uint32_t lane = threadIdx.x & 63u;
	for (;;) {
		if (!exhausted) {
			const unsigned long long idle = __ballot(!has_ray);
			if (idle) {
				uint32_t base = 0;
				const int leader = __ffsll((long long)idle) - 1;
				if ((int)lane == leader)
					base = atomicAdd(queue_head, (uint32_t)__popcll(idle));
				base = __shfl(base, leader, 64);
				if (!has_ray) {
					const uint32_t i = base + __popcll(idle & ((1ull << lane) - 1ull));
					if (i < n_rays) {
						V3 o, d;
						float tmin, tmax;
						load(i, o, d, tmin, tmax);
						const V3 so = sane_ray(o, tmax);
						trav_begin(s, st, so, d, tmin, tmax, sc.eps_t);
						if (sc.n_quadrics)
							trav_quadrics<false>(sc, s, ANY);
						my_ray	= i;
						has_ray = true;
					}
				}
				exhausted = base + (uint32_t)__popcll(idle) >= n_rays;
			}
		}
		if (!__any(has_ray))
			break;
		unsigned long long m_has = lane_ballot(has_ray);
		for (;;) {
			const unsigned long long m_lb	 = lane_ballot((s.cur & REC_LEAF_BIT) != 0u);
			const unsigned long long m_leaf	 = m_has & m_lb, m_inner = m_has & ~m_lb;
			const int n_leaf = wave_popc(m_leaf), n_inner = wave_popc(m_inner);
			if (COUNT && lane == 0)
				++witers;
			const bool do_inner = n_inner >= n_leaf;
			if (lane_in(do_inner ? m_inner : m_leaf)) {
				if (do_inner) {
					if (COUNT)
						++cn;
					trav_inner<ANY>(sc, s, st);
				} else {
					if (COUNT)
// ... 1837 lines not shown
constexpr uint32_t BL_UNWRITTEN = 0xFFFFFFFEu, BL_HOLE = 0xFFFFFFFFu;

template <bool COUNT, uint32_t FEATS, int WIDE>
__device__ __forceinline__ void path_persistent(const DevScene& sc, const PathState& ps, const PersistentArgs& a)
{
	constexpr int NQ = (FEATS & FEAT_ROUGH_MATERIALS) ? 2 : 1;
	constexpr int QR = NQ;
	constexpr uint32_t FEATS_PLAIN = FEATS & ~FEAT_ROUGH_MATERIALS;
	__shared__ PPShared<NQ> sh;
	constexpr uint32_t RAY_MASK = 2 * PP_SLOTS_MAX - 1, SHADE_MASK = PP_SLOTS_MAX - 1;
	const uint32_t lane	 = threadIdx.x & 63u;
	const uint32_t block_slots = a.slots_per_block;
	const uint32_t slot0	   = blockIdx.x * block_slots;
	for (uint32_t i = threadIdx.x; i < 2 * PP_SLOTS_MAX; i += TRAV_BLOCK)
		sh.q_ray[i] = PP_EMPTY;
	for (uint32_t i = threadIdx.x; i < PP_SLOTS_MAX; i += TRAV_BLOCK) {
		sh.q_shade[QR][i] = i < block_slots ? i : PP_EMPTY;
		for (int q = 0; q < NQ; ++q)
			sh.q_shade[q][i] = PP_EMPTY;
		sh.pending[i] = 0;
		if (i < block_slots)
			ps.pixel[slot0 + i] = INVALID;
	}
	if (threadIdx.x == 0) {
		sh.ray_head = sh.ray_tail = 0;
		for (int q = 0; q < NQ; ++q)
			sh.shade_head[q] = sh.shade_tail[q] = 0;
		sh.shade_head[QR] = 0;
		sh.shade_tail[QR] = block_slots;
		sh.live					  = block_slots;
		sh.error				  = 0;
		sh.n_list = sh.unit_next = sh.exhausted = sh.n_frozen = 0;
	}
	uint32_t* const bl_list = a.bl_list + size_t(blockIdx.x) * a.bl_cap;
	uint32_t* const bl_word = a.bl_word + size_t(blockIdx.x) * a.bl_cap;
	if (a.resident)
		for (uint32_t i = threadIdx.x; i < a.bl_cap; i += TRAV_BLOCK) {
			bl_list[i] = BL_UNWRITTEN;
			bl_word[i] = 0u;
		}
	const bool wl_in_lds = sc.wl_cdf_size >= 2u && sc.wl_cdf_size <= WL_LDS && sc.cfg.mapper == PRGPU_MAPPER_SPD_CMIS;
	if (wl_in_lds)
		for (uint32_t i = threadIdx.x; i < sc.wl_cdf_size; i += TRAV_BLOCK)
			sh.wl_cdf[i] = sc.wl_cdf[i];
	stats_init(sh.bs);
	__syncthreads();
	if (wl_in_lds) {
		for (uint32_t b = threadIdx.x; b <= CDF_GUIDE_BUCKETS; b += TRAV_BLOCK) {
			const float x = (float)b / (float)CDF_GUIDE_BUCKETS;
			int first = 0, len = (int)sc.wl_cdf_size;
			while (len > 0) {
				const int half = len / 2, middle = first + half;
				if (sh.wl_cdf[middle] <= x) {
					first = middle + 1;
					len -= half + 1;
				} else {
					len = half;
				}
			}
			sh.wl_guide[b] = (uint16_t)first;
		}
		__syncthreads();
	}
	WlTable wlt;
	if (wl_in_lds) {
		wlt.cdf	  = sh.wl_cdf;
		wlt.guide = sh.wl_guide;
	}

	Stack st;
	st.lds			= sh.stack + threadIdx.x;
	st.spill_stride = gridDim.x * TRAV_BLOCK;
	st.spill		= a.spill + (blockIdx.x * TRAV_BLOCK + threadIdx.x);
	st.reset();
	Trav s;
	s.cur			  = REC_EMPTY;
	s.any			  = false;
	bool has_ray	  = false;
	uint32_t my_entry = 0;

	uint32_t spins	  = 0;
	unsigned long long t_idle_since = 0;
	uint32_t cn_c = 0, cl_c = 0, cn_a = 0, cl_a = 0, witers = 0, wleaf = 0, sbatches = 0, slanes = 0;
	unsigned long long t_shade = 0, t_idle = 0, t_leaf = 0, t_inner = 0, t_refill = 0, t_fin = 0, t_cam = 0, t_vert = 0;
	unsigned long long t_cls[4] = { 0, 0, 0, 0 };
	uint32_t b_cls[4] = { 0, 0, 0, 0 }, l_cls[4] = { 0, 0, 0, 0 };
	const unsigned long long t_start = COUNT ? wall_clock64() : 0ull;
	const unsigned long long c_start = COUNT ? (unsigned long long)clock64() : 0ull;

	const uint32_t shader_idx = 3u;
	const bool shader		  = a.shader_wave != 0u && ((threadIdx.x >> 6) & 3u) + a.shader_wave > shader_idx;
	const uint32_t shade_full = a.shader_wave != 0u ? PP_SHADE_HELP : a.shade_min;
	for (;;) {
		const int n_act	  = __popcll(__ballot(has_ray));
		uint32_t n_shade = wave_bcast0(lds_load(&sh.shade_tail[0]) - lds_load(&sh.shade_head[0]));
		int cls			 = 0;
		for (int q = 1; q < NQ + 1; ++q) {
			const uint32_t nq = wave_bcast0(lds_load(&sh.shade_tail[q]) - lds_load(&sh.shade_head[q]));
			if (nq > n_shade) {
				n_shade = nq;
				cls		= q;
			}
		}
		uint32_t n_queued = wave_bcast0(lds_load(&sh.ray_tail) - lds_load(&sh.ray_head));

		bool shade_now;
		if (shader)
			shade_now = n_shade > 0u;
		else if (a.shader_wave != 0u)
			shade_now = n_shade >= shade_full || (n_queued == 0u && n_shade > 0u && n_act == 0);
		else
			shade_now = n_shade >= a.shade_min || (n_queued == 0u && ((n_shade >= a.shade_partial && n_act < a.refill_below) || (n_shade > 0u && n_act == 0)));
		if (shade_now) {
			uint32_t first;
			const uint32_t n = ring_claim(&sh.shade_head[cls], &sh.shade_tail[cls], 64u, first);
			if (n) {
				spins			  = 0;
#if PR_SHADE_PRIO
				__builtin_amdgcn_s_setprio(PR_SHADE_PRIO);
#endif
				const unsigned long long t0 = COUNT ? wall_clock64() : 0ull;
				if (COUNT && lane == 0) {
					++sbatches;
					slanes += n;
				}
				const bool mine	  = lane < n;
				uint32_t slot_l	  = 0;
				const bool regen_pass = cls == QR;
				const bool regen	  = regen_pass;
				if (mine)
					slot_l = ring_take(sh.q_shade[cls], SHADE_MASK, first + lane);
				const uint32_t slot = slot0 + slot_l;
				if (mine) {
					const uint32_t pw = lds_load(&sh.pending[slot_l]);
					if (pw & PP_SHADOW) {
						const float4 x		 = ps.st[slot].sh_xyz;
						const uint32_t fbs	 = __float_as_uint(x.w);
						const uint32_t pixel = ps.pixel[slot];
						if (pw & PP_VISIBLE) {
							const float xyz[3] = { x.x, x.y, x.z };
							apply_fragment(ps, pixel, iter_entry(ps, slot, pixel), fbs & 0xFFu, xyz, (FEATS & FEAT_LPE) ? (fbs >> 16) & 0xFu : 0u);
						} else if ((fbs >> 8) & 0xFFu) {
							ps.feedback[pixel] |= (fbs >> 8) & 0xFFu;
						}
					}
				}
				bool alive = false, want_shadow = false;
				float4 sh_o = make_float4(0, 0, 0, 0), sh_d = sh_o, sh_xyz = sh_o;
				const unsigned long long t0v = COUNT ? wall_clock64() : 0ull;
				if (regen_pass) {
				} else if (NQ > 1 && cls == 1) {
					if (mine)
						shade_vertex<FEATS>(sc, ps, slot, sh.bs, alive, want_shadow, sh_o, sh_d, sh_xyz);
				} else {
					if (mine)
						shade_vertex<FEATS_PLAIN>(sc, ps, slot, sh.bs, alive, want_shadow, sh_o, sh_d, sh_xyz);
				}
				if (COUNT)
					t_vert += wall_clock64() - t0v;
				const bool to_regen = !regen_pass && mine && !alive && !want_shadow;
				const bool ended	= mine && regen;
				bool need_pixel	 = false;
				uint32_t iter	 = 0;
				if (ended) {
					const uint32_t pixel = ps.pixel[slot];
					need_pixel			 = true;
// ... 139 lines not shown
				{
					const uint32_t pslot = slot0 + (has_ray ? (my_entry & ~PP_ANY) : 0u);
					const bool pany		 = has_ray && (my_entry & PP_ANY) != 0;
					const float4 ro = pany ? ps.st[pslot].sh_o : ps.st[pslot].ray_o, rd = pany ? ps.st[pslot].sh_d : ps.st[pslot].ray_d;
					s.r	   = ray_prepare(v3(ro.x, ro.y, ro.z), v3(rd.x, rd.y, rd.z), sc.eps_t);
					s.tmin = ro.w + 0.0f;
					s.any  = pany;
				}
#if PR_SHADE_PRIO
				__builtin_amdgcn_s_setprio(0);
#endif
				if (COUNT)
					t_shade += wall_clock64() - t0;
				if (COUNT && lane == 0)
					for (int q = 0; q < NQ + 1; ++q)
						if (q == cls) {
							t_cls[q] += wall_clock64() - t0;
							b_cls[q] += 1u;
							l_cls[q] += n;
						}
			}
			continue;
		}

		const unsigned long long idle = __ballot(!has_ray);
		if (!shader && idle != 0ull && n_queued > 0u) {
#if PR_REFILL_PRIO
			__builtin_amdgcn_s_setprio(PR_REFILL_PRIO);
#endif
			const unsigned long long t0r = COUNT ? wall_clock64() : 0ull;
			uint32_t first;
			const uint32_t n = ring_claim(&sh.ray_head, &sh.ray_tail, (uint32_t)__popcll(idle), first);
			const uint32_t r = __popcll(idle & ((1ull << lane) - 1ull));
			if (!has_ray && r < n) {
				my_entry			= ring_take(sh.q_ray, RAY_MASK, first + r);
				const uint32_t slot = slot0 + (my_entry & ~PP_ANY);
				const bool any		= (my_entry & PP_ANY) != 0;
				const float4 ro = any ? ps.st[slot].sh_o : ps.st[slot].ray_o, rd = any ? ps.st[slot].sh_d : ps.st[slot].ray_d;
				trav_begin(s, st, v3(ro.x, ro.y, ro.z), v3(rd.x, rd.y, rd.z), ro.w, any ? rd.w - 0.001f : rd.w, sc.eps_t);
				s.any	= any;
				has_ray = true;
				if (FEATS & FEAT_QUADRICS)
					trav_quadrics<(NQ > 1)>(sc, s, any);
			}
#if PR_REFILL_PRIO
			__builtin_amdgcn_s_setprio(0);
#endif
			if (COUNT)
				t_refill += wall_clock64() - t0r;
		}
		if (!__any(has_ray)) {
			if (lds_load(&sh.live) == 0u || lds_load(&sh.error) != 0u)
				break;
			const unsigned long long t0 = COUNT ? wall_clock64() : 0ull;
			__builtin_amdgcn_s_sleep(8);
			if (COUNT)
				t_idle += wall_clock64() - t0;
			if (n_shade == 0u && n_queued == 0u) {
				if (spins++ == 0u)
					t_idle_since = wall_clock64();
				else if ((spins & 1023u) == 0u && wall_clock64() - t_idle_since > PP_IDLE_LIMIT_TICKS) {
					if (lane == 0) {
						__hip_atomic_store(&sh.error, 1u, __ATOMIC_RELAXED, __HIP_MEMORY_SCOPE_WORKGROUP);
						atomicExch(a.error, 1u);
					}
					break;
				}
			}
			continue;
		}
		spins = 0;
		unsigned long long m_has  = lane_ballot(has_ray);
		unsigned long long m_wait = m_has & lane_ballot(s.cur == REC_EMPTY);
		for (;;) {
			const unsigned long long m_lb	 = lane_ballot((s.cur & REC_LEAF_BIT) != 0u);
			const unsigned long long m_leaf	 = m_has & m_lb & ~m_wait;
			const unsigned long long m_inner = m_has & ~m_lb;
			const int n_leaf = wave_popc(m_leaf), n_inner = wave_popc(m_inner);
			if (COUNT && lane == 0)
				++witers;
			const bool do_inner = n_inner >= n_leaf;
			const unsigned long long t0s = COUNT ? wall_clock64() : 0ull;
			if (lane_in(do_inner ? m_inner : m_leaf)) {
				const float4* __restrict__ rec = rec_ptr(sc.recs, s.cur);
				const float4 q0 = rec[0], q1 = rec[1], q2 = rec[2];
				const bool wide = WIDE == 2 ? sc.bvh_wide != 0u : WIDE == 1;
				float4 qw		= make_float4(0.0f, 0.0f, 0.0f, 0.0f);
				if (wide && do_inner)
					qw = rec[3];
				const uint2 top_e	   = PR_PEEK ? st.peek() : make_uint2(0u, 0u);
				const uint2* const top = PR_PEEK ? &top_e : nullptr;
				if (do_inner) {
					if (COUNT) {
						cn_c += s.any ? 0 : 1;
						cn_a += s.any ? 1 : 0;
					}
					trav_inner_rec<MODE_MIXED>(s, st, q0, q1, q2, qw, wide, top);
				} else {
					const float4 q3 = rec[3], q4 = rec[4], q5 = rec[5], q6 = rec[6], q7 = rec[7];
					if (COUNT) {
						cl_c += s.any ? 0 : 1;
						cl_a += s.any ? 1 : 0;
					}
					trav_leaf_rec<MODE_MIXED, (FEATS & FEAT_SPHERES) != 0, (NQ > 1)>(s, st, q0, q1, q2, q3, q4, q5, q6, q7, top);
				}
			}
			if (COUNT) {
				if (do_inner)
					t_inner += wall_clock64() - t0s;
				else
					t_leaf += wall_clock64() - t0s;
			}
			const unsigned long long m_done = m_has & lane_ballot(s.cur == REC_EMPTY);
			unsigned long long m_fin		= m_done;
			if (a.fin_batch > 1) {
				const int n_done = wave_popc(m_done);
				const int n_run	 = wave_popc(m_has & ~m_done);
				if (n_done < a.fin_batch && n_run >= a.refill_below)
					m_fin = 0ull;
			}
			const unsigned long long t0f = COUNT ? wall_clock64() : 0ull;
			if (m_fin != 0ull) {
#if PR_FIN_PRIO
				__builtin_amdgcn_s_setprio(PR_FIN_PRIO);
#endif
				const bool fin = lane_in(m_fin);
				bool last	   = false;
				uint32_t entry = 0;
				int qcls	   = 0;
				if (fin) {
					const uint32_t slot_l = my_entry & ~PP_ANY;
					const uint32_t slot	  = slot0 + slot_l;
					uint32_t add = 0xFFFFFFFFu;
					if (s.any) {
						if (s.best.tri == INVALID)
							add += PP_VISIBLE;
					} else {
						ps.st[slot].hit = make_float4(s.best.t, s.best.u, s.best.v, __uint_as_float(s.best.tri));
						if (NQ > 1)
							add += (s.cls & 3u) << PP_CLS_SHIFT;
					}
					const uint32_t old = __hip_atomic_fetch_add(&sh.pending[slot_l], add, __ATOMIC_ACQ_REL, __HIP_MEMORY_SCOPE_WORKGROUP);
					last			   = (old & 0xFFu) == 1u;
					entry			   = slot_l;
					if (last && (old & PP_DEAD))
						qcls = QR;
					if (NQ > 1 && last && !(old & PP_DEAD))
						qcls = s.any ? (int)((old >> PP_CLS_SHIFT) & 3u) : (int)(s.cls & 3u);
				}
				m_has &= ~m_fin;
				for (int q = 0; q < NQ + 1; ++q)
					ring_push(sh.q_shade[q], SHADE_MASK, &sh.shade_tail[q], last && qcls == q, entry);
#if PR_FIN_PRIO
				__builtin_amdgcn_s_setprio(0);
#endif
				if (COUNT)
					t_fin += wall_clock64() - t0f;
			}
			m_wait			 = m_done & m_has;
			const int active = wave_popc(m_has);
			if (active == 0)
				break;
			if (active < a.refill_below) {
				uint32_t nsh = lds_load(&sh.shade_tail[0]) - lds_load(&sh.shade_head[0]);
				for (int q = 1; q < NQ + 1; ++q)
					nsh = max(nsh, lds_load(&sh.shade_tail[q]) - lds_load(&sh.shade_head[q]));
				const uint32_t nq = lds_load(&sh.ray_tail) - lds_load(&sh.ray_head);
				if (wave_bcast0((nq > 0u || nsh >= shade_full || (a.shader_wave == 0u && nsh >= a.shade_partial)) ? 1u : 0u))
					break;
			}
		}
		has_ray = lane_in(m_has);
	}
	if (COUNT) {
		if (cn_c)
			atomicAdd(&a.gstats[CNT_NODES_CLOSEST], (unsigned long long)cn_c);
		if (cl_c)
			atomicAdd(&a.gstats[CNT_TRIS_CLOSEST], (unsigned long long)cl_c);
		if (cn_a)
			atomicAdd(&a.gstats[CNT_NODES_ANY], (unsigned long long)cn_a);
		if (cl_a)
			atomicAdd(&a.gstats[CNT_TRIS_ANY], (unsigned long long)cl_a);
		if (witers)
			atomicAdd(&a.gstats[CNT_WAVE_ITERS_CLOSEST], (unsigned long long)witers);
		if (wleaf)
			atomicAdd(&a.gstats[CNT_WAVE_ITERS_ANY], (unsigned long long)wleaf);
		if (sbatches) {
			atomicAdd(&a.gstats[CNT_SHADE_BATCHES], (unsigned long long)sbatches);
			atomicAdd(&a.gstats[CNT_SHADE_LANES], (unsigned long long)slanes);
		}
		if (lane == 0) {
			atomicAdd(&a.gstats[CNT_SHADE_TICKS], t_shade);
			atomicAdd(&a.gstats[CNT_IDLE_TICKS], t_idle);
			atomicAdd(&a.gstats[CNT_TOTAL_TICKS], wall_clock64() - t_start);
			atomicAdd(&a.gstats[CNT_LEAF_TICKS], t_leaf);
			atomicAdd(&a.gstats[CNT_INNER_TICKS], t_inner);
			atomicAdd(&a.gstats[CNT_REFILL_TICKS], t_refill);
			atomicAdd(&a.gstats[CNT_FIN_TICKS], t_fin);
			atomicAdd(&a.gstats[CNT_CAMERA_TICKS], t_cam);
			atomicAdd(&a.gstats[CNT_VERTEX_TICKS], t_vert);
			atomicAdd(&a.gstats[CNT_TOTAL_CYCLES], (unsigned long long)clock64() - c_start);
			for (int q = 0; q < NQ + 1; ++q) {
				atomicAdd(&a.gstats[CNT_CLS_TICKS0 + q], t_cls[q]);
				atomicAdd(&a.gstats[CNT_CLS_BATCHES0 + q], (unsigned long long)b_cls[q]);
				atomicAdd(&a.gstats[CNT_CLS_LANES0 + q], (unsigned long long)l_cls[q]);
			}
		}
		if (threadIdx.x == 0)
			a.spill[blockIdx.x * TRAV_BLOCK] = make_uint2((uint32_t)(wall_clock64() - t_start), sh.bs.v[PRGPU_STAT_CAMERA_DEPTH] + sh.bs.v[PRGPU_STAT_BACKGROUND_HITS]);
	}
	stats_flush(sh.bs, a.gstats);
}
template <bool COUNT, uint32_t FEATS>
__global__ void __launch_bounds__(TRAV_BLOCK) __attribute__((amdgpu_waves_per_eu(2, 2))) k_path_persistent(DevScene sc, PathState ps, PersistentArgs a)
{
	path_persistent<COUNT, FEATS, 2>(sc, ps, a);
}
template <bool COUNT, uint32_t FEATS, bool WIDE>
__global__ void __launch_bounds__(TRAV_BLOCK) __attribute__((amdgpu_waves_per_eu(3, 3))) k_path_persistent_occ3(DevScene sc, PathState ps, PersistentArgs a)
{
	path_persistent<COUNT, FEATS, WIDE ? 1 : 0>(sc, ps, a);
}

#include "path_wave.inl"

#if PR_TU == 0
#include "ao.inl"

__global__ void __launch_bounds__(TRAV_BLOCK) k_service_closest(DevScene sc, uint32_t n, const float* __restrict__ org, const float* __restrict__ dir,
															   const float* __restrict__ tmin_a, const float* __restrict__ tmax_a, uint32_t* entity,
															   uint32_t* prim, float* u, float* v, float* t, uint32_t* queue_head, uint2* spill,
															   int refill_below, unsigned long long* gstats)
{
	auto load = [&](uint32_t i, V3& o, V3& d, float& tmin, float& tmax) {
		o	 = v3(org[3 * i], org[3 * i + 1], org[3 * i + 2]);
		d	 = v3(dir[3 * i], dir[3 * i + 1], dir[3 * i + 2]);
		tmin = tmin_a[i];
		tmax = tmax_a[i];
	};
	auto store = [&](uint32_t i, const Hit& h) {
		const bool ok	 = h.tri != INVALID;
		const uint32_t e = ok ? sc.tri_entity[h.tri] : INVALID;
		entity[i]		 = e;
		prim[i]			 = ok ? prim_id(sc, h.tri) : INVALID;
		u[i]			 = ok ? h.u : 0.0f;
		v[i]			 = ok ? h.v : 0.0f;
		t[i]			 = ok ? h.t : tmax_a[i];
	};
	trace_persistent<false, true>(sc, n, queue_head, spill, refill_below, load, store, gstats);
}
template <bool WIDE>
struct SplitRing {
	static constexpr uint32_t N = WIDE ? 2048u : 1024u;
};
template <bool WIDE, typename STK>
__device__ __forceinline__ void trav_inner_split(Trav& s, STK& st, const float4& q0, const float4& q1, const float4& q2, const float4& q3, uint32_t* q, uint32_t* q_tail,
												 uint32_t* pending_own, uint32_t tid, bool active, const uint32_t* q_head, uint32_t* overflow)
{
	constexpr int NW		= WIDE ? 6 : 4;
	constexpr uint32_t SQ	= SplitRing<WIDE>::N;
	uint32_t key[6] = { 0xFFFFFFFFu, 0xFFFFFFFFu, 0xFFFFFFFFu, 0xFFFFFFFFu, 0xFFFFFFFFu, 0xFFFFFFFFu };
	if (active)
		inner_keys(s, q0, q1, q2, q3, WIDE, key);
	const uint32_t base = __float_as_uint(q2.z);
	bool lf[NW];
	uint32_t cnt = 0;
#pragma unroll
	for (int k = 0; k < NW; ++k) {
		lf[k] = key[k] != 0xFFFFFFFFu && (key[k] & REC_LEAF_BIT) != 0u;
		cnt += lf[k] ? 1u : 0u;
	}
	{
		const uint32_t lane			   = tid & 63u;
		const unsigned long long below = (1ull << lane) - 1ull;
		const unsigned long long b0 = __ballot((cnt & 1u) != 0u), b1 = __ballot((cnt & 2u) != 0u), b2 = __ballot((cnt & 4u) != 0u);
		const uint32_t total = (uint32_t)__popcll(b0) + 2u * (uint32_t)__popcll(b1) + 4u * (uint32_t)__popcll(b2);
		if (total != 0u) {
			uint32_t pos0 = 0;
			if (lane == 0)
				pos0 = __hip_atomic_fetch_add(q_tail, total, __ATOMIC_RELAXED, __HIP_MEMORY_SCOPE_WORKGROUP);
			pos0 = wave_bcast0(pos0);
			if (lane == 0 && pos0 + total - lds_load(q_head) > SQ)
				__hip_atomic_store(overflow, 1u, __ATOMIC_RELAXED, __HIP_MEMORY_SCOPE_WORKGROUP);
			uint32_t pos = pos0 + (uint32_t)__popcll(b0 & below) + 2u * (uint32_t)__popcll(b1 & below) + 4u * (uint32_t)__popcll(b2 & below);
			if (cnt)
				__hip_atomic_fetch_add(pending_own, cnt, __ATOMIC_RELAXED, __HIP_MEMORY_SCOPE_WORKGROUP);
#pragma unroll
			for (int k = 0; k < NW; ++k)
				if (lf[k])
					__hip_atomic_store(&q[(pos++) & (SQ - 1u)], (((base + (key[k] & 0xFFu)) >> REC_UNIT_SHIFT) << 8) | tid, __ATOMIC_RELEASE, __HIP_MEMORY_SCOPE_WORKGROUP);
		}
	}
	if (!active)
		return;
#pragma unroll
	for (int k = 0; k < NW; ++k)
		key[k] = lf[k] ? 0xFFFFFFFFu : key[k];
#define PR_CSWAP(a, b)                                  \
	{                                                   \
		const uint32_t lo = min(key[a], key[b]);        \
		key[b]			  = max(key[a], key[b]);        \
		key[a]			  = lo;                         \
	}
	if (WIDE) {
		PR_CSWAP(0, 5) PR_CSWAP(1, 3) PR_CSWAP(2, 4) PR_CSWAP(1, 2) PR_CSWAP(3, 4) PR_CSWAP(0, 3) PR_CSWAP(2, 5) PR_CSWAP(0, 1) PR_CSWAP(2, 3) PR_CSWAP(4, 5) PR_CSWAP(1, 2) PR_CSWAP(3, 4)
		st.reserve(5);
		st.push_if(key[5] != 0xFFFFFFFFu, base + (key[5] & 0xFFu), key[5]);
		st.push_if(key[4] != 0xFFFFFFFFu, base + (key[4] & 0xFFu), key[4]);
	} else {
		PR_CSWAP(0, 1) PR_CSWAP(2, 3) PR_CSWAP(0, 2) PR_CSWAP(1, 3) PR_CSWAP(1, 2)
		st.reserve(3);
	}
#undef PR_CSWAP
	st.push_if(key[3] != 0xFFFFFFFFu, base + (key[3] & 0xFFu), key[3]);
	st.push_if(key[2] != 0xFFFFFFFFu, base + (key[2] & 0xFFu), key[2]);
	st.push_if(key[1] != 0xFFFFFFFFu, base + (key[1] & 0xFFu), key[1]);
	s.cur = key[0] != 0xFFFFFFFFu ? base + (key[0] & 0xFFu) : REC_EMPTY;
	trav_pop<MODE_CLOSEST>(s, st);
}

constexpr bool COUNT_SPLIT_STEPS = true;
template <bool WIDE>
struct SplitShared {
	uint2 stack[STACK_LDS * TRAV_BLOCK];
	float4 rc[2][TRAV_BLOCK];
	unsigned long long best[TRAV_BLOCK];
	uint32_t pending[TRAV_BLOCK];
	uint32_t q[SplitRing<WIDE>::N];
	uint32_t q_head, q_tail, overflow;
};
__global__ void k_tri_slot(DevScene sc, const uint32_t* __restrict__ leaf_units, uint32_t* __restrict__ tri_slot)
{
	const uint32_t i = blockIdx.x * blockDim.x + threadIdx.x;
	if (i >= sc.n_leaf)
		return;
	const uint32_t unit = leaf_units[i];
	const float* f		= reinterpret_cast<const float*>(sc.recs + unit);
	const uint32_t cnt	= __float_as_uint(f[30]);
	for (uint32_t k = 0; k < cnt && k < 3u; ++k)
		tri_slot[__float_as_uint(f[10 * k + 9]) & ~PRIM_SPHERE_BIT] = (unit << 2) | k;
}
template <bool WIDE>
__global__ void __launch_bounds__(TRAV_BLOCK) k_service_closest_split(DevScene sc, uint32_t n, const float* __restrict__ org, const float* __restrict__ dir,
																	 const float* __restrict__ tmin_a, const float* __restrict__ tmax_a, uint32_t* entity,
																	 uint32_t* prim, float* u, float* v, float* t, uint32_t* queue_head, uint2* spill,
																	 const uint32_t* __restrict__ tri_slot, int refill_below, unsigned long long* gstats)
{
	constexpr uint32_t SQ = SplitRing<WIDE>::N;
	__shared__ SplitShared<WIDE> sh;
	const uint32_t tid = threadIdx.x, lane = tid & 63u;
	for (uint32_t i = tid; i < SQ; i += TRAV_BLOCK)
		sh.q[i] = PP_EMPTY;
	sh.pending[tid] = 0;
	if (tid == 0)
		sh.q_head = sh.q_tail = 0;
	__syncthreads();
	Stack st;
	st.lds			= sh.stack + tid;
	st.spill_stride = gridDim.x * TRAV_BLOCK;
	st.spill		= spill + (blockIdx.x * TRAV_BLOCK + tid);
	st.reset();
	Trav s;
	s.cur		   = REC_EMPTY;
	s.any		   = false;
	uint32_t my_ray = 0;
	bool has_ray   = false;
	bool exhausted = false;
	uint32_t cn = 0, cl = 0, witers = 0, spins = 0;

	auto leaf_batch = [&]() -> bool {
		uint32_t first;
		const uint32_t nt = ring_claim(&sh.q_head, &sh.q_tail, 64u, first);
		if (nt == 0u)
			return false;
		if (lane < nt) {
			const uint32_t task	 = ring_take(sh.q, SQ - 1u, first + lane);
			const uint32_t owner = task & 0xFFu, unit = task >> 8;
			RayPre r;
			const float4 ra = sh.rc[0][owner], rb = sh.rc[1][owner];
			r.o				  = v3(ra.x, ra.y, ra.z);
			const uint32_t kk = __float_as_uint(ra.w);
			r.kx			  = (int)(kk & 3u);
			r.ky			  = (int)((kk >> 2) & 3u);
			r.kz			  = (int)((kk >> 4) & 3u);
			r.Sx			  = rb.x;
			r.Sy			  = rb.y;
			r.Sz			  = rb.z;
			const float tmin  = rb.w;
			const float4* __restrict__ rec = reinterpret_cast<const float4*>(sc.recs + unit);
			const float4 q0 = rec[0], q1 = rec[1], q2 = rec[2], q3 = rec[3], q4 = rec[4], q5 = rec[5], q6 = rec[6], q7 = rec[7];
			const float f[32] = { q0.x, q0.y, q0.z, q0.w, q1.x, q1.y, q1.z, q1.w, q2.x, q2.y, q2.z, q2.w, q3.x, q3.y, q3.z, q3.w,
								  q4.x, q4.y, q4.z, q4.w, q5.x, q5.y, q5.z, q5.w, q6.x, q6.y, q6.z, q6.w, q7.x, q7.y, q7.z, q7.w };
			const uint32_t count = __float_as_uint(f[30]);
			unsigned long long key = ~0ull;
#pragma unroll
			for (int k = 0; k < 3; ++k) {
				if ((uint32_t)k < count) {
					float tt, uu, vv;
					if (woop(r, v3(f[10 * k], f[10 * k + 1], f[10 * k + 2]), v3(f[10 * k + 3], f[10 * k + 4], f[10 * k + 5]), v3(f[10 * k + 6], f[10 * k + 7], f[10 * k + 8]), tt, uu, vv)
						&& tt > tmin) {
						const unsigned long long kk2 = ((unsigned long long)__float_as_uint(tt) << 32) | __float_as_uint(f[10 * k + 9]);
						key							 = kk2 < key ? kk2 : key;
					}
				}
			}
			if (key != ~0ull)
				__hip_atomic_fetch_min(&sh.best[owner], key, __ATOMIC_RELAXED, __HIP_MEMORY_SCOPE_WORKGROUP);
			__hip_atomic_fetch_sub(&sh.pending[owner], 1u, __ATOMIC_RELEASE, __HIP_MEMORY_SCOPE_WORKGROUP);
			++cl;
		}
		return true;
	};

	bool drained = false;
	for (;;) {
		if (drained) {
			const unsigned long long key = __hip_atomic_load(&sh.best[tid], __ATOMIC_RELAXED, __HIP_MEMORY_SCOPE_WORKGROUP);
			const uint32_t tri			 = (uint32_t)key;
			float tt = tmax_a[my_ray], uu = 0.0f, vv = 0.0f;
			if (tri != INVALID) {
				const uint32_t slot = tri_slot[tri];
				const float* f		= reinterpret_cast<const float*>(sc.recs + (slot >> 2)) + 10u * (slot & 3u);
				(void)woop(s.r, v3(f[0], f[1], f[2]), v3(f[3], f[4], f[5]), v3(f[6], f[7], f[8]), tt, uu, vv);
			}
			entity[my_ray] = tri != INVALID ? sc.tri_entity[tri] : INVALID;
			prim[my_ray]   = tri != INVALID ? prim_id(sc, tri) : INVALID;
			u[my_ray]	   = uu;
			v[my_ray]	   = vv;
			t[my_ray]	   = tt;
			has_ray		   = false;
			drained		   = false;
		}
		if (!exhausted) {
			const unsigned long long idle = __ballot(!has_ray);
			if (idle) {
				uint32_t base	 = 0;
				const int leader = __ffsll((long long)idle) - 1;
				if ((int)lane == leader)
					base = atomicAdd(queue_head, (uint32_t)__popcll(idle));
				base = __shfl(base, leader, 64);
				if (!has_ray) {
					const uint32_t i = base + __popcll(idle & ((1ull << lane) - 1ull));
					if (i < n) {
						const V3 o = v3(org[3 * i], org[3 * i + 1], org[3 * i + 2]), d = v3(dir[3 * i], dir[3 * i + 1], dir[3 * i + 2]);
						float tmax_i = tmax_a[i];
						const V3 so = sane_ray(o, tmax_i);
						trav_begin(s, st, so, d, tmin_a[i], tmax_i, sc.eps_t);
						sh.rc[0][tid] = make_float4(so.x, so.y, so.z, __uint_as_float((uint32_t)s.r.kx | ((uint32_t)s.r.ky << 2) | ((uint32_t)s.r.kz << 4)));
						sh.rc[1][tid] = make_float4(s.r.Sx, s.r.Sy, s.r.Sz, s.tmin);
						__hip_atomic_store(&sh.best[tid], ((unsigned long long)__float_as_uint(tmax_i) << 32) | 0xFFFFFFFFull, __ATOMIC_RELAXED, __HIP_MEMORY_SCOPE_WORKGROUP);
						my_ray	= i;
						has_ray = true;
					}
				}
				exhausted = base + (uint32_t)__popcll(idle) >= n;
			}
		}
		if (!__any(has_ray))
			break;
		for (;;) {
			const uint32_t nq	 = wave_bcast0(lds_load(&sh.q_tail) - lds_load(&sh.q_head));
			const bool can_inner = __any(has_ray && s.cur != REC_EMPTY);
			if (nq >= 64u || (nq > 0u && !can_inner)) {
				(void)leaf_batch();
				spins = 0;
			} else if (can_inner) {
				if (COUNT_SPLIT_STEPS && lane == 0)
					++witers;
				while (wave_bcast0(lds_load(&sh.q_tail) - lds_load(&sh.q_head)) > SQ / 4u)
					if (!leaf_batch())
						__builtin_amdgcn_s_sleep(1);
				{
					const bool act = has_ray && s.cur != REC_EMPTY;
					float4 q0 = make_float4(0, 0, 0, 0), q1 = q0, q2 = q0, q3 = q0;
					if (act) {
						s.best.t = __uint_as_float((uint32_t)(__hip_atomic_load(&sh.best[tid], __ATOMIC_RELAXED, __HIP_MEMORY_SCOPE_WORKGROUP) >> 32));
// ... 387 lines not shown
```

pearray_amd/csrc/prgpu_api.hip:

```cpp
#include <hip/hip_runtime.h>
#include <dlfcn.h>

#include <algorithm>
#include <cmath>
#include <cstdlib>
#include <cstring>
#include <map>
#include <string>
#include <vector>

#include "../../include/prgpu.h"
#include "device/bvh.h"
#include "device/render.h"
#include "host/setup.h"

namespace {

thread_local std::string g_error;

int fail(int code, const std::string& msg)
{
	g_error = msg;
	return code;
}
// ... 73 lines not shown
	k.pp_slots_set		  = getenv("PRGPU_PP_SLOTS") != nullptr;
	k.pp.slots			  = (uint32_t)num("PRGPU_PP_SLOTS", k.pp.slots, 256, prd::persistent_slot_padding());
	k.pp.shade_min		  = (int)num("PRGPU_PP_SHADE_MIN", k.pp.shade_min, 1, 64);
	k.pp.shade_partial	  = (int)num("PRGPU_PP_SHADE_PARTIAL", k.pp.shade_partial, 1, 64);
	k.pp.fin_batch		  = (int)num("PRGPU_PP_FIN_BATCH", k.pp.fin_batch, 1, 64);
	k.pp.occupancy		  = (int)num("PRGPU_PP_OCCUPANCY", k.pp.occupancy, 2, 3);
	k.pp.shader_wave	  = (int)num("PRGPU_PP_SHADER", k.pp.shader_wave, -1, 2);
	k.pp.resident		  = num("PRGPU_PP_RESIDENT", 1, 0, 1) != 0;
	k.pp_refill			  = (int)num("PRGPU_PP_REFILL", k.pp_refill, 1, 64);
	k.pp_blocks_per_cu	  = (int)num("PRGPU_PP_BLOCKS_PER_CU", 0, 0, 8);
	k.pp_max_blocks		  = (int)num("PRGPU_PP_MAX_BLOCKS", 0, 0, 1 << 20);
	k.pp_planes			  = (int)num("PRGPU_PP_PLANES", k.pp_planes, 1, 64);
	k.pp_launch_samples	  = (uint64_t)num("PRGPU_PP_LAUNCH_SAMPLES", (long long)k.pp_launch_samples, 1, 1ll << 40);
	k.pp_launch_min_iters = (int)num("PRGPU_PP_LAUNCH_MIN_ITERS", k.pp_launch_min_iters, 1, 1 << 15);
	k.pp_tune_order		  = num("PRGPU_PP_TUNE_ORDER", 1, 0, 1) != 0;
	k.groups			  = (int)num("PRGPU_GROUPS", k.groups, 1, 16);
	k.sort_rays			  = num("PRGPU_SORT_RAYS", 0, 0, 1) != 0;
	k.trace_split		  = num("PRGPU_TRACE_SPLIT", 1, 0, 1) != 0;
	k.comm_force_rccl	  = num("PRGPU_COMM_FORCE_RCCL", 0, 0, 1) != 0;
	if (const char* env = getenv("PRGPU_FORCE_FEATURES"))
		k.force_features = (uint32_t)strtoul(env, nullptr, 0);
	k.debug_counters  = getenv("PRGPU_DEBUG_COUNTERS") != nullptr;
	k.dump_block_life = getenv("PRGPU_DUMP_BLOCK_LIFE");
	k.trace_ranges	  = (int)num("PRGPU_TRACE_RANGES", -1, -1, 1);
	return k;
}

struct TraceRange {
	typedef int (*PushFn)(const char*);
	typedef int (*PopFn)();
	static PushFn& push_fn() { static PushFn f = nullptr; return f; }
	static PopFn& pop_fn() { static PopFn f = nullptr; return f; }
	static bool bind()
	{
		static const bool bound = [] {
			const int knob	 = read_knobs().trace_ranges;
			const bool force = knob == 1;
			if (knob == 0)
				return false;
			for (const char* name : { "librocprofiler-sdk-roctx.so.1", "librocprofiler-sdk-roctx.so", "libroctx64.so.4", "libroctx64.so" }) {
				void* lib = dlopen(name, RTLD_NOW | RTLD_LOCAL | RTLD_NOLOAD);
				if (!lib && force)
					lib = dlopen(name, RTLD_NOW | RTLD_LOCAL);
				if (!lib)
					continue;
				push_fn() = reinterpret_cast<PushFn>(dlsym(lib, "roctxRangePushA"));
				pop_fn()  = reinterpret_cast<PopFn>(dlsym(lib, "roctxRangePop"));
				if (push_fn() && pop_fn())
					return true;
				push_fn() = nullptr;
				pop_fn()  = nullptr;
				dlclose(lib);
			}
			return false;
		}();
		return bound;
	}
	bool active;
	explicit TraceRange(const char* name) : active(bind()) { if (active) (void)push_fn()(name); }
	~TraceRange() { if (active) (void)pop_fn()(); }
	TraceRange(const TraceRange&) = delete;
	TraceRange& operator=(const TraceRange&) = delete;
};

struct TimedLaunch {
	hipEvent_t start, stop;
	int family;
};
const char* const FAMILY_NAMES[] = { "raygen", "trace_closest", "shade", "trace_any", "resolve", "sort", "path", "reduce", "ao" };
constexpr int N_FAMILIES		 = 9;

}

struct prgpu_scene {
	int device = 0;
	hipStream_t own_stream = nullptr, stream = nullptr;
	prd::DevScene sc{};
	prd::PathState ps{};
	prgpu_settings cfg{};
	uint32_t n_pixels = 0, n_slots = 0;
	std::vector<void*> allocations;
	uint32_t bvh_units = 0;
	uint32_t bvh_stack_bound = 0, bvh_top = 0;
	float bvh_cost4 = 0.0f, bvh_cost6 = 0.0f;
	int pp_shader_waves = -1;
	double pp_shading_share = 0.0;
	uint64_t pp_launches = 0;
	int pp_calibration_tries = 0;
	unsigned long long *gstats_before = nullptr, *gstats_after = nullptr;
	uint32_t pp_last_blocks = 0, pp_last_slots = 0, pp_last_kernel = 0;
	float* own_xyz = nullptr;
	uint32_t *own_samples = nullptr, *own_feedback = nullptr;
	uint32_t *active_a = nullptr, *active_b = nullptr, *dead_a = nullptr, *dead_b = nullptr;
	enum Mode { LOCKSTEP, STREAMING, PERSISTENT };
	Mode mode = LOCKSTEP;
	Knobs knobs;
	uint32_t pp_planes = 1;
	uint32_t *pp_pixel = nullptr, *pp_next = nullptr, *pp_error = nullptr;
	unsigned long long* gstats = nullptr;
	prd::TraceWorkspace ws;
	prd::TraceWorkspace ws_pp;
	struct Group {
		hipStream_t s_main = nullptr, s_shadow = nullptr;
		hipEvent_t ev_shade = nullptr, ev_shadow = nullptr;
		uint32_t slot_begin = 0, n_slots = 0;
		uint32_t *active_a = nullptr, *active_b = nullptr, *counters = nullptr, *h_counters = nullptr;
		uint32_t *dead_a = nullptr, *dead_b = nullptr;
		uint32_t *dead_cur = nullptr, *dead_prev = nullptr;
		uint32_t *sort_keys_a = nullptr, *sort_keys_b = nullptr, *sort_active = nullptr;
		void* sort_temp = nullptr;
		size_t sort_temp_bytes = 0;
		uint32_t n_dead_prev = 0;
		prd::TraceWorkspace ws_closest, ws_shadow;
		prd::PathState ps;
		const uint32_t* active = nullptr;
		uint32_t* next = nullptr;
		uint32_t n_active = 0, depth = 0;
		bool done = true, shadow_pending = false;
	};
	std::vector<Group> groups;
	hipEvent_t ev_resolve = nullptr;
	bool resolve_recorded = false;
	bool instrument = false, timing = false;
	std::vector<TimedLaunch> pending;
	double family_ms[N_FAMILIES] = { 0 };
	uint64_t family_launches[N_FAMILIES] = { 0 };
	uint64_t rays_closest = 0, rays_any = 0;
	uint32_t next_iteration = 0;
	bool ao_enabled = false;
	prd::AoState ao{};
	prd::TraceWorkspace ws_ao;
	std::vector<prgpu_tile> tiles;
	prd::DevLpe lpe_host{};
	uint32_t order_tuned_at = 0;
	bool poisoned = false;
	uint32_t reduced_at = 0xFFFFFFFFu;
	struct Reduced {
		float* xyz = nullptr;
		uint32_t *samples = nullptr, *feedback = nullptr;
		float *online_mean = nullptr, *online_variance = nullptr;
		float* aov[PRGPU_AOV_COUNT] = {};
		std::vector<float*> lpe;
		bool valid = false;
	} reduced;

	template <typename T>
	int alloc(T*& ptr, size_t count, bool zero = false)
	{
		void* p = nullptr;
		HIP_TRY(hipMalloc(&p, std::max<size_t>(count, 1) * sizeof(T)));
		allocations.push_back(p);
		ptr = static_cast<T*>(p);
		if (zero)
			HIP_TRY(hipMemsetAsync(p, 0, std::max<size_t>(count, 1) * sizeof(T), stream));
		return PRGPU_OK;
	}
	template <typename T>
	int upload(const T*& ptr, const T* src, size_t count)
	{
		T* p = nullptr;
		const int rc = alloc(p, count);
		if (rc != PRGPU_OK)
			return rc;
		if (count)
			HIP_TRY(hipMemcpyAsync(p, src, count * sizeof(T), hipMemcpyHostToDevice, stream));
		ptr = p;
// ... 219 lines not shown
	}
	{
		std::vector<prd::DevInfLight> il = t.inf_lights;
		if (il.empty())
			il.resize(1);
		UP(sc.inf_lights, il);
	}
	sc.sky_cdf = nullptr;
	if (!t.sky_cdf.empty())
		UP(sc.sky_cdf, t.sky_cdf);
	UP(sc.wl_cdf, t.wl_cdf);
	UP(sc.sobol2d, t.sobol2d);
	UP(sc.rr_prob, t.rr_prob);
	UP(sc.filter, t.filter);
	UP(sc.cie, t.cie);
	sc.n_lights = 0;
	for (uint32_t e = 0; e < d->n_entities; ++e)
		sc.n_lights += d->entities[e].emission != PRGPU_INVALID_ID;
	sc.n_inf_lights	 = d->n_lights;
	sc.shape_lights	 = nullptr;
	if (!t.shape_lights.empty())
		UP(sc.shape_lights, t.shape_lights);
	sc.quadrics	  = nullptr;
	sc.n_quadrics = (uint32_t)t.quadrics.size();
	if (!t.quadrics.empty())
		UP(sc.quadrics, t.quadrics);
	sc.features		 = d->n_lights ? prd::FEAT_INFINITE_LIGHTS : 0u;
	if (!t.quadrics.empty())
		sc.features |= prd::FEAT_QUADRICS;
	if (!t.shape_lights.empty())
		sc.features |= prd::FEAT_SHAPE_LIGHTS;
	for (uint32_t i = 0; i < d->n_spectra; ++i)
		if (d->spectra[i].kind == PRGPU_SPEC_CHECKER)
			sc.features |= prd::FEAT_TEXTURES;
	for (uint32_t e = 0; e < d->n_entities; ++e)
		if (d->entities[e].has_uvs && d->uvs && d->entities[e].kind == PRGPU_ENTITY_MESH)
			sc.features |= prd::FEAT_TEXTURES;
	for (uint32_t i = 0; i < d->n_materials; ++i) {
		const uint32_t kind = d->materials[i].kind;
		if (kind == PRGPU_MAT_DIELECTRIC || kind == PRGPU_MAT_CONDUCTOR || kind == PRGPU_MAT_MIRROR)
			sc.features |= prd::FEAT_DELTA_MATERIALS;
		else if (kind != PRGPU_MAT_LAMBERT)
			sc.features |= prd::FEAT_DELTA_MATERIALS | prd::FEAT_ROUGH_MATERIALS;
	}
	for (uint32_t e = 0; e < d->n_entities; ++e)
		if (d->entities[e].kind == PRGPU_ENTITY_PLANE)
			sc.features |= prd::FEAT_PLANES;
		else if (d->entities[e].kind == PRGPU_ENTITY_SPHERE)
			sc.features |= prd::FEAT_SPHERES;
	sc.features |= read_knobs().force_features & prd::FEAT_ALL & ~(prd::FEAT_LPE | prd::FEAT_QUADRICS);
	sc.scene_radius	 = t.scene_radius;
	sc.wl_cdf_size	 = (uint32_t)t.wl_cdf.size();
	sc.wl_u_offset	 = t.wl_u_offset;
	sc.wl_u_scale	 = t.wl_u_scale;
	sc.agh_c		 = t.agh_c;
	sc.agh_n		 = t.agh_n;
	sc.rr_size		 = (uint32_t)t.rr_prob.size();
	sc.cam			 = t.cam;
	sc.cfg			 = d->settings;
	sc.spp			 = t.spp;
	sc.mj_x			 = t.mj_x;
	sc.mj_y			 = t.mj_y;
	sc.mj_seed		 = t.mj_seed;
	sc.halton_bx	 = t.halton_bx;
	sc.halton_by	 = t.halton_by;
	sc.halton_burnin = t.halton_burnin;
	sc.single_tap	 = t.single_tap;
	sc.centre_weight = t.centre_weight;
	sc.eps_t		 = t.eps_t;
	if (!(t.coord_scale <= prd::SCENE_COORD_MAX))
		return fail(PRGPU_EINVAL, "scene coordinates must be finite and at most 2^28 in magnitude (the BVH's quantisation grid)");
	sc.n_tris		 = d->n_triangles;

	prd::BvhBuildInput bin{ d->n_triangles, d->n_entities, sc.positions, sc.indices, sc.tri_entity, sc.entities, sc.tri_class };
	if (s->knobs.bvh_width_invalid)
		return fail(PRGPU_EINVAL, "PRGPU_BVH_WIDTH must be auto, 4 or 6");
	if (s->knobs.bvh_top_invalid)
		return fail(PRGPU_EINVAL, "PRGPU_BVH_TOP must be auto, file, area or morton");
	if (s->knobs.bvh_parity_invalid)
		return fail(PRGPU_EINVAL, "PRGPU_BVH_PARITY must be auto, even or odd");
	bin.width = s->knobs.bvh_width;
	bin.top	  = s->knobs.bvh_top;
	bin.parity = s->knobs.bvh_parity;
	bin.stack_capacity = prd::trace_stack_capacity();
	prd::BvhBuildOutput bout;
	{
		TraceRange bvh_range("prgpu_scene_create: LBVH build");
		if (!prd::build_lbvh(bin, bout, s->stream, err))
			return fail(PRGPU_EDEVICE, "LBVH build failed: " + err);
	}
	s->allocations.push_back(bout.recs);
	if (bout.leaf_units)
		s->allocations.push_back(bout.leaf_units);
	sc.recs	   = bout.recs;
	sc.n_inner = bout.n_inner;
	sc.bvh_wide = bout.wide ? 1u : 0u;
	s->bvh_cost4 = bout.cost4;
	s->bvh_cost6 = bout.cost6;
	s->bvh_stack_bound = bout.stack_bound;
	s->bvh_top = (uint32_t)bout.top;
	sc.n_leaf  = bout.n_leaf;
	s->bvh_units = bout.n_units;
	{
		uint32_t* map = nullptr;
		const int rc2 = s->alloc(map, std::max<size_t>(1, d->n_triangles), true);
		if (rc2 != PRGPU_OK)
			return rc2;
		prd::launch_tri_slot(sc, bout.leaf_units, map, s->stream);
		sc.tri_slot = map;
	}

	const uint32_t np = d->settings.width * d->settings.height;
	s->n_pixels		  = np;
	prd::PathState& ps = s->ps;
#define AL(ptr, count, zero)                      \
	do {                                          \
		rc = s->alloc(ptr, count, zero);          \
		if (rc != PRGPU_OK)                       \
			return rc;                            \
	} while (0)
	const size_t ns = size_t(np) + prd::slot_array_padding();
	AL(ps.rng, np, false);
	HIP_TRY(hipMemcpyAsync(ps.rng, t.rng.data(), size_t(np) * 8, hipMemcpyHostToDevice, s->stream));
	AL(ps.pixel, np, false);
	AL(ps.st, ns, false);
	AL(ps.sh_o, ns, false);
	AL(ps.sh_d, ns, false);
	AL(ps.sh_xyz, ns, false);
	AL(ps.sh_slot, ns, false);
	s->pp_planes = t.single_tap ? 1u : (uint32_t)s->knobs.pp_planes;
	AL(ps.iter_xyz, size_t(np) * 3 * s->pp_planes, true);
	ps.plane_stride = 0;
	ps.iter_base	= 0;
	AL(s->own_xyz, size_t(np) * 3, true);
	AL(s->own_samples, np, true);
	AL(s->own_feedback, np, true);
	AL(ps.prim_entity, np, false);
	AL(ps.prim_prim, np, false);
	HIP_TRY(hipMemsetAsync(ps.prim_entity, 0xFF, size_t(np) * 4, s->stream));
	HIP_TRY(hipMemsetAsync(ps.prim_prim, 0xFF, size_t(np) * 4, s->stream));
	ps.out_xyz	= s->own_xyz;
	ps.samples	= s->own_samples;
	ps.feedback = s->own_feedback;
	AL(s->active_a, np, false);
	AL(s->active_b, np, false);
	AL(s->dead_a, np, false);
	AL(s->dead_b, np, false);
	AL(ps.iter, ns, true);
	AL(ps.cost, np, true);
	s->mode = prgpu_scene::PERSISTENT;
	if (s->knobs.mode_invalid)
		return fail(PRGPU_EINVAL, "PRGPU_MODE must be lockstep, streaming or persistent");
	if (s->knobs.pp_kernel_invalid)
		return fail(PRGPU_EINVAL, "PRGPU_PP_KERNEL must be auto, throughput or latency");
	if (s->knobs.mode == 0)
		s->mode = prgpu_scene::LOCKSTEP;
	else if (s->knobs.mode == 1)
		s->mode = t.single_tap ? prgpu_scene::STREAMING : prgpu_scene::LOCKSTEP;
	AL(s->pp_pixel, ns, false);
	AL(s->pp_next, 1, true);
	AL(s->pp_error, 1, true);
	AL(s->gstats, prd::N_DEVICE_COUNTERS, true);
	AL(s->gstats_before, prd::N_DEVICE_COUNTERS, true);
	AL(s->gstats_after, prd::N_DEVICE_COUNTERS, true);
	{
		hipDeviceProp_t prop;
		HIP_TRY(hipGetDeviceProperties(&prop, device));
		const uint32_t blocks_per_cu = 2;
		const int refill			 = 44;
		const uint32_t max_blocks = (uint32_t)std::max(1, prop.multiProcessorCount) * blocks_per_cu;
		auto make_ws = [&](prd::TraceWorkspace& w, uint32_t n_blocks) -> int {
			w.max_blocks   = n_blocks;
			w.refill_below = refill;
			AL(w.queue_head, 1, true);
			AL(w.spill, prd::trace_workspace_spill_entries(n_blocks), false);
			return PRGPU_OK;
		};
		rc = make_ws(s->ws, (uint32_t)std::max(1, prop.multiProcessorCount) * 3u);
		if (rc != PRGPU_OK)
			return rc;
		{
			uint32_t pp_blocks_per_cu = 768u / prd::persistent_block_threads();
			if (!s->knobs.pp_slots_set)
// ... 707 lines not shown
	}
	if (const char* path = s->instrument && s->mode == prgpu_scene::PERSISTENT ? read_knobs().dump_block_life : nullptr) {
		const size_t bt = prd::persistent_block_threads();
		std::vector<uint2> rows(size_t(s->ws_pp.max_blocks) * bt);
		HIP_TRY(hipMemcpy(rows.data(), s->ws_pp.spill, rows.size() * sizeof(uint2), hipMemcpyDeviceToHost));
		if (FILE* f = std::fopen(path, "w")) {
			for (uint32_t b = 0; b < s->ws_pp.max_blocks; ++b)
				std::fprintf(f, "%u %u %u\n", b, rows[size_t(b) * bt].x, rows[size_t(b) * bt].y);
			std::fclose(f);
		}
	}
	return check_watchdog(s);
}

int prgpu_download(prgpu_scene* s, float* xyz, uint32_t* samples, uint32_t* feedback)
{
	TraceRange trace_range("prgpu_download");
	if (!s)
		return fail(PRGPU_EINVAL, "null scene");
	HIP_TRY(hipSetDevice(s->device));
	HIP_TRY(hipStreamSynchronize(s->stream));
	if (xyz)
		HIP_TRY(hipMemcpy(xyz, s->reduced.valid ? s->reduced.xyz : s->ps.out_xyz, size_t(s->n_pixels) * 12, hipMemcpyDeviceToHost));
	if (samples)
		HIP_TRY(hipMemcpy(samples, s->reduced.valid ? s->reduced.samples : s->ps.samples, size_t(s->n_pixels) * 4, hipMemcpyDeviceToHost));
	if (feedback)
		HIP_TRY(hipMemcpy(feedback, s->reduced.valid ? s->reduced.feedback : s->ps.feedback, size_t(s->n_pixels) * 4, hipMemcpyDeviceToHost));
	return PRGPU_OK;
}

int prgpu_stats(prgpu_scene* s, uint64_t out[PRGPU_STAT_COUNT])
{
	if (!s || !out)
		return fail(PRGPU_EINVAL, "null argument");
	HIP_TRY(hipSetDevice(s->device));
	HIP_TRY(hipStreamSynchronize(s->stream));
	unsigned long long host[prd::N_DEVICE_COUNTERS];
	HIP_TRY(hipMemcpy(host, s->gstats, sizeof(host), hipMemcpyDeviceToHost));
	for (int k = 0; k < PRGPU_STAT_COUNT; ++k)
		out[k] = host[k];
	return PRGPU_OK;
}

int prgpu_film_size(prgpu_scene* s, uint32_t* width, uint32_t* height)
{
	if (!s)
		return fail(PRGPU_EINVAL, "null scene");
	if (width)
		*width = s->cfg.width;
	if (height)
		*height = s->cfg.height;
	return PRGPU_OK;
}

int prgpu_trace_counters_get(prgpu_scene* s, prgpu_trace_counters* out)
{
	if (!s || !out)
		return fail(PRGPU_EINVAL, "null argument");
	HIP_TRY(hipSetDevice(s->device));
	HIP_TRY(hipStreamSynchronize(s->stream));
	unsigned long long host[prd::N_DEVICE_COUNTERS];
	HIP_TRY(hipMemcpy(host, s->gstats, sizeof(host), hipMemcpyDeviceToHost));
	out->rays_closest  = s->rays_closest;
	out->rays_any	   = s->rays_any;
	if (s->mode == prgpu_scene::PERSISTENT || s->ao_enabled) {
		out->rays_closest += host[PRGPU_STAT_PRIMARY_RAYS] + host[PRGPU_STAT_BOUNCE_RAYS];
		out->rays_any += host[PRGPU_STAT_SHADOW_RAYS];
	}
	out->nodes_closest = host[PRGPU_STAT_COUNT + 0];
	out->leaves_closest  = host[PRGPU_STAT_COUNT + 1];
	out->nodes_any	   = host[PRGPU_STAT_COUNT + 2];
	out->leaves_any	   = host[PRGPU_STAT_COUNT + 3];
	out->node_bytes	   = sizeof(prd::Rec64);
	out->leaf_bytes	   = 2 * sizeof(prd::Rec64);
	out->ray_bytes	   = 32;
	out->hit_bytes	   = 16;
	out->wave_steps_closest = host[PRGPU_STAT_COUNT + 4];
	out->wave_steps_any		= host[PRGPU_STAT_COUNT + 5];
	out->shade_batches		= host[PRGPU_STAT_COUNT + 6];
	out->shade_lanes		= host[PRGPU_STAT_COUNT + 7];
	out->shade_ticks		= host[PRGPU_STAT_COUNT + 8];
	out->idle_ticks			= host[PRGPU_STAT_COUNT + 9];
	out->total_ticks		= host[PRGPU_STAT_COUNT + 10];
	if (read_knobs().debug_counters)
		if (host[PRGPU_STAT_COUNT + 10]) {
			const double T = double(host[PRGPU_STAT_COUNT + 10]);
			fprintf(stderr, "[prgpu] wave time: shading %.1f %%, idle %.1f %%, leaf steps %.1f %%, inner steps %.1f %%, refill %.1f %%, ray ends %.1f %%; of the shading: vertices %.1f %%, camera paths %.1f %%; shader clock %.0f MHz\n",
					100 * host[PRGPU_STAT_COUNT + 8] / T, 100 * host[PRGPU_STAT_COUNT + 9] / T, 100 * host[PRGPU_STAT_COUNT + 11] / T, 100 * host[PRGPU_STAT_COUNT + 12] / T,
					100 * host[PRGPU_STAT_COUNT + 14] / T, 100 * host[PRGPU_STAT_COUNT + 15] / T, 100 * host[PRGPU_STAT_COUNT + 17] / T, 100 * host[PRGPU_STAT_COUNT + 16] / T,
					100.0 * double(host[PRGPU_STAT_COUNT + 13]) / T);
			for (int q = 0; q < 4; ++q)
				if (host[PRGPU_STAT_COUNT + 22 + q])
					fprintf(stderr, "[prgpu]   shade queue %d: %.1f %% of wave time, %.0f passes, fill %.3f, %.2f us per pass\n", q, 100 * host[PRGPU_STAT_COUNT + 18 + q] / T,
							double(host[PRGPU_STAT_COUNT + 22 + q]), double(host[PRGPU_STAT_COUNT + 26 + q]) / (64.0 * double(host[PRGPU_STAT_COUNT + 22 + q])),
							0.01 * double(host[PRGPU_STAT_COUNT + 18 + q]) / double(host[PRGPU_STAT_COUNT + 22 + q]));
		}
	return PRGPU_OK;
}

int prgpu_set_instrumentation(prgpu_scene* s, int enabled)
{
	if (!s)
		return fail(PRGPU_EINVAL, "null scene");
	s->instrument = enabled != 0;
	return PRGPU_OK;
}

int prgpu_set_timing(prgpu_scene* s, int enabled)
{
	if (!s)
		return fail(PRGPU_EINVAL, "null scene");
	HIP_TRY(hipSetDevice(s->device));
	HIP_TRY(hipStreamSynchronize(s->stream));
	s->collect_timing();
	s->timing = enabled != 0;
	return PRGPU_OK;
}

int prgpu_kernel_time_ms(prgpu_scene* s, const char* family, double* total_ms, uint64_t* launches)
{
	if (!s || !family)
		return fail(PRGPU_EINVAL, "null argument");
	HIP_TRY(hipSetDevice(s->device));
	HIP_TRY(hipStreamSynchronize(s->stream));
	s->collect_timing();
	for (int f = 0; f < N_FAMILIES; ++f)
		if (std::strcmp(family, FAMILY_NAMES[f]) == 0) {
			if (total_ms)
				*total_ms = s->family_ms[f];
			if (launches)
				*launches = s->family_launches[f];
			return PRGPU_OK;
		}
	return fail(PRGPU_EINVAL, "unknown kernel family");
}

int prgpu_trace_closest(prgpu_scene* s, uint32_t n, const float* org, const float* dir, const float* tmin, const float* tmax,
						uint32_t* entity, uint32_t* prim, float* u, float* v, float* t)
{
	if (!s || (n && (!org || !dir || !tmin || !tmax)))
		return fail(PRGPU_EINVAL, "null argument");
	if (n == 0)
		return PRGPU_OK;
	for (uint32_t i = 0; i < n; ++i)
		if (!(tmin[i] >= 0.0f))
			return fail(PRGPU_EINVAL, "prgpu_trace_closest: tmin must not be negative (ray " + std::to_string(i) + ")");
	HIP_TRY(hipSetDevice(s->device));
	float *d_org = nullptr, *d_dir = nullptr, *d_tmin = nullptr, *d_tmax = nullptr, *d_u = nullptr, *d_v = nullptr, *d_t = nullptr;
	uint32_t *d_e = nullptr, *d_p = nullptr;
	int rc = PRGPU_OK;
	auto cleanup = [&]() {
		(void)hipFree(d_org); (void)hipFree(d_dir); (void)hipFree(d_tmin); (void)hipFree(d_tmax);
		(void)hipFree(d_u); (void)hipFree(d_v); (void)hipFree(d_t); (void)hipFree(d_e); (void)hipFree(d_p);
	};
#define TRY_OR_CLEAN(expr)                                                                          \
	do {                                                                                            \
		hipError_t _e = (expr);                                                                     \
		if (_e != hipSuccess) {                                                                     \
			cleanup();                                                                              \
			return fail(PRGPU_EDEVICE, std::string(#expr) + " failed: " + hipGetErrorString(_e));   \
		}                                                                                           \
	} while (0)
	TRY_OR_CLEAN(hipMalloc(&d_org, size_t(n) * 12));
	TRY_OR_CLEAN(hipMalloc(&d_dir, size_t(n) * 12));
	TRY_OR_CLEAN(hipMalloc(&d_tmin, size_t(n) * 4));
	TRY_OR_CLEAN(hipMalloc(&d_tmax, size_t(n) * 4));
	TRY_OR_CLEAN(hipMalloc(&d_u, size_t(n) * 4));
	TRY_OR_CLEAN(hipMalloc(&d_v, size_t(n) * 4));
	TRY_OR_CLEAN(hipMalloc(&d_t, size_t(n) * 4));
	TRY_OR_CLEAN(hipMalloc(&d_e, size_t(n) * 4));
	TRY_OR_CLEAN(hipMalloc(&d_p, size_t(n) * 4));
	TRY_OR_CLEAN(hipMemcpyAsync(d_org, org, size_t(n) * 12, hipMemcpyHostToDevice, s->stream));
	TRY_OR_CLEAN(hipMemcpyAsync(d_dir, dir, size_t(n) * 12, hipMemcpyHostToDevice, s->stream));
	TRY_OR_CLEAN(hipMemcpyAsync(d_tmin, tmin, size_t(n) * 4, hipMemcpyHostToDevice, s->stream));
	TRY_OR_CLEAN(hipMemcpyAsync(d_tmax, tmax, size_t(n) * 4, hipMemcpyHostToDevice, s->stream));
	s->time_begin(1, s->stream);
	const bool split = read_knobs().trace_split;
	if (split && s->sc.n_leaf > 0 && s->bvh_units < (1u << 24) && !(s->sc.features & (prd::FEAT_SPHERES | prd::FEAT_QUADRICS))) {
		prd::launch_service_closest_split(s->sc, n, d_org, d_dir, d_tmin, d_tmax, d_e, d_p, d_u, d_v, d_t, s->ws, const_cast<uint32_t*>(s->sc.tri_slot), s->gstats, s->stream);
	} else
		prd::launch_service_closest(s->sc, n, d_org, d_dir, d_tmin, d_tmax, d_e, d_p, d_u, d_v, d_t, s->ws, s->gstats, s->stream);
	s->time_end(s->stream);
	s->rays_closest += n;
	TRY_OR_CLEAN(hipGetLastError());
	TRY_OR_CLEAN(hipStreamSynchronize(s->stream));
	if (entity)
		TRY_OR_CLEAN(hipMemcpy(entity, d_e, size_t(n) * 4, hipMemcpyDeviceToHost));
	if (prim)
		TRY_OR_CLEAN(hipMemcpy(prim, d_p, size_t(n) * 4, hipMemcpyDeviceToHost));
	if (u)
		TRY_OR_CLEAN(hipMemcpy(u, d_u, size_t(n) * 4, hipMemcpyDeviceToHost));
	if (v)
		TRY_OR_CLEAN(hipMemcpy(v, d_v, size_t(n) * 4, hipMemcpyDeviceToHost));
	if (t)
		TRY_OR_CLEAN(hipMemcpy(t, d_t, size_t(n) * 4, hipMemcpyDeviceToHost));
	cleanup();
	return rc;
}

int prgpu_trace_any(prgpu_scene* s, uint32_t n, const float* org, const float* dir, const float* tmin, const float* distance, uint8_t* occluded)
{
	if (!s || (n && (!org || !dir || !tmin || !distance || !occluded)))
		return fail(PRGPU_EINVAL, "null argument");
	if (n == 0)
		return PRGPU_OK;
	for (uint32_t i = 0; i < n; ++i)
		if (!(tmin[i] >= 0.0f))
			return fail(PRGPU_EINVAL, "prgpu_trace_any: tmin must not be negative (ray " + std::to_string(i) + ")");
	HIP_TRY(hipSetDevice(s->device));
	float *d_org = nullptr, *d_dir = nullptr, *d_tmin = nullptr, *d_dist = nullptr;
	uint8_t* d_occ = nullptr;
	auto cleanup = [&]() {
		(void)hipFree(d_org); (void)hipFree(d_dir); (void)hipFree(d_tmin); (void)hipFree(d_dist); (void)hipFree(d_occ);
	};
	TRY_OR_CLEAN(hipMalloc(&d_org, size_t(n) * 12));
	TRY_OR_CLEAN(hipMalloc(&d_dir, size_t(n) * 12));
	TRY_OR_CLEAN(hipMalloc(&d_tmin, size_t(n) * 4));
	TRY_OR_CLEAN(hipMalloc(&d_dist, size_t(n) * 4));
	TRY_OR_CLEAN(hipMalloc(&d_occ, size_t(n)));
	TRY_OR_CLEAN(hipMemcpyAsync(d_org, org, size_t(n) * 12, hipMemcpyHostToDevice, s->stream));
	TRY_OR_CLEAN(hipMemcpyAsync(d_dir, dir, size_t(n) * 12, hipMemcpyHostToDevice, s->stream));
	TRY_OR_CLEAN(hipMemcpyAsync(d_tmin, tmin, size_t(n) * 4, hipMemcpyHostToDevice, s->stream));
	TRY_OR_CLEAN(hipMemcpyAsync(d_dist, distance, size_t(n) * 4, hipMemcpyHostToDevice, s->stream));
	s->time_begin(3, s->stream);
	prd::launch_service_any(s->sc, n, d_org, d_dir, d_tmin, d_dist, d_occ, s->ws, s->gstats, s->stream);
	s->time_end(s->stream);
	s->rays_any += n;
	TRY_OR_CLEAN(hipGetLastError());
	TRY_OR_CLEAN(hipStreamSynchronize(s->stream));
	TRY_OR_CLEAN(hipMemcpy(occluded, d_occ, size_t(n), hipMemcpyDeviceToHost));
	cleanup();
	return PRGPU_OK;
}

}
namespace {
typedef int nccl_result_t;
struct NcclId {
	char internal[PRGPU_COMM_ID_BYTES];
};
struct Rccl {
	void* lib = nullptr;
	nccl_result_t (*GetUniqueId)(NcclId*)									= nullptr;
	nccl_result_t (*CommInitRank)(void**, int, NcclId, int)				= nullptr;
	nccl_result_t (*CommDestroy)(void*)										= nullptr;
	nccl_result_t (*GroupStart)()											= nullptr;
	nccl_result_t (*GroupEnd)()												= nullptr;
	nccl_result_t (*Reduce)(const void*, void*, size_t, int, int, int, void*, hipStream_t) = nullptr;
	const char* (*GetErrorString)(nccl_result_t)							= nullptr;
	nccl_result_t (*CommCount)(void*, int*)									= nullptr;
	nccl_result_t (*CommUserRank)(void*, int*)								= nullptr;
	std::string error;
};
Rccl& rccl()
{
	static Rccl r;
	if (r.lib || !r.error.empty())
		return r;
	for (const char* name : { "librccl.so.1", "librccl.so", "/opt/rocm/lib/librccl.so.1" }) {
		r.lib = dlopen(name, RTLD_NOW | RTLD_GLOBAL);
		if (r.lib)
// ... 153 lines not shown
			rc = need(R.online_mean, size_t(s->n_pixels) * 3);
			if (rc == PRGPU_OK)
				rc = need(R.online_variance, size_t(s->n_pixels) * 3);
		}
		for (uint32_t k = 0; rc == PRGPU_OK && k < PRGPU_AOV_COUNT; ++k)
			if (s->ps.aov[k])
				rc = need(R.aov[k], size_t(s->n_pixels) * prgpu_aov_channels(k));
		R.lpe.resize(s->lpe_host.n, nullptr);
		for (uint32_t k = 0; rc == PRGPU_OK && k < s->lpe_host.n; ++k)
			rc = need(R.lpe[k], size_t(s->n_pixels) * 3);
		if (rc != PRGPU_OK)
			return rc;
	}
	Rccl& r = rccl();
	NCCL_TRY(r.GroupStart());
	nccl_result_t first_error = 0;
	const char* first_what	  = nullptr;
	auto reduce = [&](const void* src, void* dst, size_t count, int type, int op, const char* what) {
		if (first_error != 0)
			return;
		const nccl_result_t rc = r.Reduce(src, dst, count, type, op, root, c->nccl, s->stream);
		if (rc != 0) {
			first_error = rc;
			first_what	= what;
		}
	};
	s->time_begin(7, s->stream);
	reduce(s->ps.out_xyz, is_root ? R.xyz : s->ps.out_xyz, size_t(s->n_pixels) * 3, NCCL_FLOAT32, NCCL_SUM, "ncclReduce(xyz)");
	reduce(s->ps.samples, is_root ? R.samples : s->ps.samples, size_t(s->n_pixels), NCCL_UINT32, NCCL_SUM, "ncclReduce(samples)");
	reduce(s->ps.feedback, is_root ? R.feedback : s->ps.feedback, size_t(s->n_pixels), NCCL_UINT32, NCCL_MAX, "ncclReduce(feedback)");
	if (s->ps.online_mean) {
		reduce(s->ps.online_mean, is_root ? R.online_mean : s->ps.online_mean, size_t(s->n_pixels) * 3, NCCL_FLOAT32, NCCL_SUM, "ncclReduce(online mean)");
		reduce(s->ps.online_variance, is_root ? R.online_variance : s->ps.online_variance, size_t(s->n_pixels) * 3, NCCL_FLOAT32, NCCL_SUM, "ncclReduce(online variance)");
	}
	for (uint32_t k = 0; k < PRGPU_AOV_COUNT; ++k)
		if (s->ps.aov[k])
			reduce(s->ps.aov[k], is_root ? R.aov[k] : s->ps.aov[k], size_t(s->n_pixels) * prgpu_aov_channels(k), NCCL_FLOAT32, NCCL_SUM, "ncclReduce(aov)");
	for (uint32_t k = 0; k < s->lpe_host.n; ++k)
		reduce(s->lpe_host.out[k], is_root ? R.lpe[k] : s->lpe_host.out[k], size_t(s->n_pixels) * 3, NCCL_FLOAT32, NCCL_SUM, "ncclReduce(lpe)");
	const nccl_result_t end_rc = r.GroupEnd();
	s->time_end(s->stream);
	if (first_error != 0)
		return fail(PRGPU_EDEVICE, std::string(first_what) + " failed: " + (r.GetErrorString ? r.GetErrorString(first_error) : "?") + " (the group was closed)");
	if (end_rc != 0)
		return fail(PRGPU_EDEVICE, std::string("ncclGroupEnd failed: ") + (r.GetErrorString ? r.GetErrorString(end_rc) : "?"));
	s->reduced_at = s->next_iteration;
	if (is_root)
		R.valid = true;
	return PRGPU_OK;
}

int prgpu_reduced_planes(prgpu_scene* s, void** d_xyz, void** d_samples, void** d_feedback)
{
	if (!s)
		return fail(PRGPU_EINVAL, "null scene");
	const bool v = s->reduced.valid;
	if (d_xyz)
		*d_xyz = v ? static_cast<void*>(s->reduced.xyz) : nullptr;
	if (d_samples)
		*d_samples = v ? static_cast<void*>(s->reduced.samples) : nullptr;
	if (d_feedback)
		*d_feedback = v ? static_cast<void*>(s->reduced.feedback) : nullptr;
	return v ? 1 : 0;
}

int prgpu_pipeline_info_get(prgpu_scene* s, prgpu_pipeline_info* out)
{
	if (!s || !out)
		return fail(PRGPU_EINVAL, "null argument");
	std::memset(out, 0, sizeof(*out));
	out->mode			 = s->mode == prgpu_scene::PERSISTENT ? 2u : (s->mode == prgpu_scene::STREAMING ? 1u : 0u);
	out->shader_waves	 = s->knobs.pp.shader_wave >= 0 ? s->knobs.pp.shader_wave : s->pp_shader_waves;
	out->shading_share	 = (float)s->pp_shading_share;
	out->launches		 = s->pp_launches;
	out->calibration_launches = (uint32_t)s->pp_calibration_tries;
	out->blocks			 = s->pp_last_blocks;
	out->slots_per_block = s->pp_last_slots;
	out->kernel			 = s->pp_last_kernel;
	out->bvh_width		 = s->sc.bvh_wide ? 6u : 4u;
	out->bvh_cost_4_wide = s->bvh_cost4;
	out->bvh_cost_6_wide = s->bvh_cost6;
	out->bvh_stack_bound = s->bvh_stack_bound;
	out->bvh_top		 = s->bvh_top;
	return PRGPU_OK;
}

uint32_t prgpu_aov_channels(uint32_t aov) { return aov < PRGPU_AOV_ENTITY_ID ? 3u : (aov < PRGPU_AOV_COUNT ? 1u : 0u); }

int prgpu_enable_aovs(prgpu_scene* s, uint32_t mask)
{
	if (!s)
		return fail(PRGPU_EINVAL, "null scene");
	if (s->next_iteration != 0)
		return fail(PRGPU_EINVAL, "AOVs must be enabled before the first iteration");
	if (mask >> PRGPU_AOV_COUNT)
		return fail(PRGPU_EINVAL, "unknown AOV bit");
	HIP_TRY(hipSetDevice(s->device));
	for (uint32_t k = 0; k < PRGPU_AOV_COUNT; ++k) {
		if (!((mask >> k) & 1u) || s->ps.aov[k])
			continue;
		const int rc = s->alloc(s->ps.aov[k], size_t(s->n_pixels) * prgpu_aov_channels(k), true);
		if (rc != PRGPU_OK)
			return rc;
	}
	s->ps.aov_mask |= mask;
	if (s->ps.aov_mask)
		s->sc.features |= prd::FEAT_AOVS;
	for (auto& g : s->groups) {
		std::memcpy(g.ps.aov, s->ps.aov, sizeof(s->ps.aov));
		g.ps.aov_mask = s->ps.aov_mask;
	}
	HIP_TRY(hipStreamSynchronize(s->stream));
	return PRGPU_OK;
}

int prgpu_enable_variance(prgpu_scene* s)
{
	if (!s)
		return fail(PRGPU_EINVAL, "null scene");
	if (s->next_iteration != 0)
		return fail(PRGPU_EINVAL, "the variance estimator must be enabled before the first iteration");
	HIP_TRY(hipSetDevice(s->device));
	if (!s->ps.online_mean) {
		int rc = s->alloc(s->ps.online_mean, size_t(s->n_pixels) * 3, true);
		if (rc != PRGPU_OK)
			return rc;
		rc = s->alloc(s->ps.online_variance, size_t(s->n_pixels) * 3, true);
		if (rc != PRGPU_OK)
			return rc;
	}
	for (auto& g : s->groups) {
		g.ps.online_mean	 = s->ps.online_mean;
		g.ps.online_variance = s->ps.online_variance;
	}
	HIP_TRY(hipStreamSynchronize(s->stream));
	return PRGPU_OK;
}

int prgpu_download_variance(prgpu_scene* s, float* mean, float* variance)
{
	if (!s)
		return fail(PRGPU_EINVAL, "null scene");
	if (!s->ps.online_mean)
		return fail(PRGPU_EINVAL, "variance estimator not enabled");
	HIP_TRY(hipSetDevice(s->device));
	HIP_TRY(hipStreamSynchronize(s->stream));
	if (mean)
		HIP_TRY(hipMemcpy(mean, s->reduced.valid && s->reduced.online_mean ? s->reduced.online_mean : s->ps.online_mean, size_t(s->n_pixels) * 12, hipMemcpyDeviceToHost));
	if (variance)
		HIP_TRY(hipMemcpy(variance, s->reduced.valid && s->reduced.online_variance ? s->reduced.online_variance : s->ps.online_variance, size_t(s->n_pixels) * 12, hipMemcpyDeviceToHost));
	return PRGPU_OK;
}

int prgpu_lpe_check(const char* expression)
{
	if (!expression)
		return fail(PRGPU_EINVAL, "null expression");
	std::vector<uint8_t> next, accepting;
	std::string err;
	const int rc = prgpu_host::compile_lpe(expression, next, accepting, err);
	return rc == PRGPU_OK ? PRGPU_OK : fail(rc, err);
}

int prgpu_lpe_match(const char* expression, const uint8_t* symbols, uint32_t count)
{
	if (!expression || (count && !symbols))
// ... 193 lines not shown
```

Before: 214.1 Msamples/s.

## Encode leaf triangle count in child refs to skip unused leaf record loads

```diff
diff --git a/include/prgpu.h b/include/prgpu.h
--- a/include/prgpu.h
+++ b/include/prgpu.h
@@ -190,6 +190,7 @@
 	uint64_t wave_steps_closest, wave_steps_any;
 	uint64_t shade_batches, shade_lanes;
 	uint64_t shade_ticks, idle_ticks, total_ticks;
+	uint64_t leaves_1tri, leaves_2tri;
 } prgpu_trace_counters;
 
 typedef struct prgpu_scene prgpu_scene;
@@ -230,6 +231,7 @@
 	uint32_t bvh_top;
 	uint32_t bvh_stack_bound;
 	float    bvh_cost_4_wide, bvh_cost_6_wide;
+	uint32_t bvh_leaf_fill[3];
 } prgpu_pipeline_info;
 int  prgpu_pipeline_info_get(prgpu_scene* s, prgpu_pipeline_info* out);
 int  prgpu_set_instrumentation(prgpu_scene* s, int enabled);
diff --git a/pearray_amd/_cabi.py b/pearray_amd/_cabi.py
--- a/pearray_amd/_cabi.py
+++ b/pearray_amd/_cabi.py
@@ -102,7 +102,8 @@
                 ("node_bytes", C.c_uint32), ("leaf_bytes", C.c_uint32), ("ray_bytes", C.c_uint32),
                 ("hit_bytes", C.c_uint32), ("wave_steps_closest", C.c_uint64), ("wave_steps_any", C.c_uint64),
                 ("shade_batches", C.c_uint64), ("shade_lanes", C.c_uint64),
-                ("shade_ticks", C.c_uint64), ("idle_ticks", C.c_uint64), ("total_ticks", C.c_uint64)]
+                ("shade_ticks", C.c_uint64), ("idle_ticks", C.c_uint64), ("total_ticks", C.c_uint64),
+                ("leaves_1tri", C.c_uint64), ("leaves_2tri", C.c_uint64)]
 
 
 class ImageStats(C.Structure):
@@ -145,7 +146,8 @@
 class PipelineInfo(C.Structure):
     _fields_ = [("mode", C.c_uint32), ("shader_waves", C.c_int32), ("shading_share", C.c_float), ("calibration_launches", C.c_uint32),
                 ("kernel", C.c_uint32), ("blocks", C.c_uint32), ("slots_per_block", C.c_uint32), ("launches", C.c_uint64),
-                ("bvh_width", C.c_uint32), ("bvh_top", C.c_uint32), ("bvh_stack_bound", C.c_uint32), ("bvh_cost_4_wide", C.c_float), ("bvh_cost_6_wide", C.c_float)]
+                ("bvh_width", C.c_uint32), ("bvh_top", C.c_uint32), ("bvh_stack_bound", C.c_uint32), ("bvh_cost_4_wide", C.c_float), ("bvh_cost_6_wide", C.c_float),
+                ("bvh_leaf_fill", C.c_uint32 * 3)]
 
 
 class SkyParams(C.Structure):
diff --git a/pearray_amd/backend.py b/pearray_amd/backend.py
--- a/pearray_amd/backend.py
+++ b/pearray_amd/backend.py
@@ -64,6 +64,7 @@
         info = abi.PipelineInfo()
         abi.check(self.lib.prgpu_pipeline_info_get(self._h, C.byref(info)))
         out = {f: getattr(info, f) for f, _ in info._fields_}
+        out["bvh_leaf_fill"] = [int(x) for x in info.bvh_leaf_fill]
         out["kernel"] = {0: "none", 1: "throughput", 2: "latency"}.get(out["kernel"], str(out["kernel"]))
         return out
 
diff --git a/pearray_amd/csrc/device/bvh.h b/pearray_amd/csrc/device/bvh.h
--- a/pearray_amd/csrc/device/bvh.h
+++ b/pearray_amd/csrc/device/bvh.h
@@ -15,6 +15,7 @@
 	uint32_t stack_capacity = 0xFFFFFFFFu;
 	int width = 0;
 	int top = -1;
+	bool corrupt_leaf_count = false;
 	int parity = -1;
 };
 struct BvhBuildOutput {
@@ -24,6 +25,7 @@
 	uint32_t stack_bound = 0;
 	int top = 0;
 	bool wide = false;
+	uint32_t leaf_fill[3] = { 0u, 0u, 0u };
 	float cost4 = 0.0f, cost6 = 0.0f;
 };
 bool build_lbvh(const BvhBuildInput& in, BvhBuildOutput& out, hipStream_t stream, std::string& err);
diff --git a/pearray_amd/csrc/device/bvh.hip b/pearray_amd/csrc/device/bvh.hip
--- a/pearray_amd/csrc/device/bvh.hip
+++ b/pearray_amd/csrc/device/bvh.hip
@@ -365,6 +365,10 @@
 }
 
 constexpr double GRID_MARGIN = 1.0 / 16384.0;
+__device__ __forceinline__ uint32_t child_payload(const ChildRef& c, uint32_t off)
+{
+	return (off << REC_UNIT_SHIFT) | (c.leaf ? REC_LEAF_BIT | ((uint32_t)(c.count - 1) << REC_COUNT_SHIFT) : 0u);
+}
 __device__ void write_inner_q(Rec64* __restrict__ rec, const ChildRef* ch, int nc, uint32_t base_unit, const uint32_t* offs)
 {
 	float org[3];
@@ -428,7 +432,7 @@
 			w[7 + a] |= h << (8 * k);
 		}
 		const int src = used ? k : 0;
-		w[11] |= ((offs[src] << REC_UNIT_SHIFT) | (ch[src].leaf ? REC_LEAF_BIT : 0u)) << (8 * k);
+		w[11] |= child_payload(ch[src], offs[src]) << (8 * k);
 	}
 	w[10]	   = base_unit << REC_UNIT_SHIFT;
 	for (int k = 4; k < 6; ++k) {
@@ -440,7 +444,7 @@
 		w[13] |= (hx << (8 * j)) | (hy << (16 + 8 * j));
 		w[14] |= (lz << (8 * j)) | (hz << (16 + 8 * j));
 		const int src = used ? k : 0;
-		w[15] |= ((offs[src] << REC_UNIT_SHIFT) | (ch[src].leaf ? REC_LEAF_BIT : 0u)) << (8 * j);
+		w[15] |= child_payload(ch[src], offs[src]) << (8 * j);
 	}
 	uint4* dst = reinterpret_cast<uint4*>(rec);
 	for (int q = 0; q < 4; ++q)
@@ -521,16 +525,15 @@
 		ok				 = e >= 27u && e <= 157u;
 	}
 	for (int k = 0; k < MAX_WIDE && ok; ++k) {
-		const uint32_t ref = base + (((k < 4 ? pw : w[15]) >> (8 * (k & 3))) & 0xFFu), cu = ref >> REC_UNIT_SHIFT;
-		ok				   = ok && (ref & 2u) == 0u;
+		const uint32_t ref = base + (((k < 4 ? pw : w[15]) >> (8 * (k & 3))) & 0xFFu);
 		if (ref & REC_LEAF_BIT) {
-			ok = (cu & 1u) == 0u && cu + 2u <= n_units;
-			if (ok) {
-				const uint32_t cnt = reinterpret_cast<const uint32_t*>(recs + cu)[30];
-				ok				   = cnt >= 1u && cnt <= 3u;
-			}
+			const uint32_t cu = (ref & REC_LEAF_ADDR) >> REC_UNIT_SHIFT, pc = leaf_ref_count(ref);
+			ok				  = (cu & 1u) == 0u && cu + 2u <= n_units && pc <= 3u;
+			if (ok)
+				ok = reinterpret_cast<const uint32_t*>(recs + cu)[30] == pc;
 		} else {
-			ok = cu + 1u <= n_units;
+			const uint32_t cu = ref >> REC_UNIT_SHIFT;
+			ok				  = (ref & 2u) == 0u && cu + 1u <= n_units;
 			if (ok) {
 				const uint32_t ce = reinterpret_cast<const uint32_t*>(recs + cu)[3] & 0xFFu;
 				ok				  = ce >= 27u && ce <= 157u;
@@ -541,14 +544,26 @@
 		atomicAdd(bad, 1u);
 }
 
+__global__ void k_corrupt_leaf_count(uint32_t n_inner, const uint32_t* __restrict__ inner_unit, Rec64* __restrict__ recs, uint32_t* __restrict__ claimed)
+{
+	const uint32_t i = blockIdx.x * blockDim.x + threadIdx.x;
+	if (i >= n_inner)
+		return;
+	uint32_t* w = reinterpret_cast<uint32_t*>(recs + inner_unit[i]);
+	if ((w[11] & REC_LEAF_BIT) != 0u && atomicCAS(claimed, 0u, 1u) == 0u)
+		w[11] ^= 1u << REC_COUNT_SHIFT;
+}
+
 __global__ void k_emit_leaves(uint32_t n, const float4* __restrict__ wv, const uint32_t* __restrict__ sorted_tri, const uint32_t* __restrict__ leaf_flag,
 							  const uint32_t* __restrict__ leaf_count, const uint32_t* __restrict__ leaf_idx, const uint32_t* __restrict__ leaf_unit, Rec64* __restrict__ recs,
-							  const uint8_t* __restrict__ tri_class)
+							  const uint8_t* __restrict__ tri_class, uint32_t* __restrict__ fill )
 {
 	const uint32_t pos = blockIdx.x * blockDim.x + threadIdx.x;
 	if (pos >= n || !leaf_flag[pos])
 		return;
 	const uint32_t cnt = leaf_count[pos];
+	if (cnt >= 1u && cnt <= 3u)
+		atomicAdd(&fill[cnt], 1u);
 	float f[32];
 	for (int k = 0; k < 32; ++k)
 		f[k] = 0.0f;
@@ -626,6 +641,8 @@
 	}
 	only.leaf			 = true;
 	only.id				 = 0u;
+	only.node			 = -1;
+	only.count			 = (int)n;
 	const uint32_t off0[4] = { 0u, 0u, 0u, 0u };
 	write_inner_q(recs, &only, 1, 2u, off0);
 	leaf_unit[0] = 2u;
@@ -984,6 +1001,7 @@
 			out.n_inner = 1;
 			out.n_leaf	= 1;
 			out.n_units = 4;
+			out.leaf_fill[n - 1] = 1u;
 		} else {
 			HIPC(hipcub::DeviceScan::ExclusiveSum(nullptr, t2a, inner_flag, inner_idx, (int)n, stream));
 			HIPC(hipcub::DeviceScan::ExclusiveSum(nullptr, t2b, leaf_flag, leaf_idx, (int)n, stream));
@@ -1004,7 +1022,7 @@
 			}
 			out.n_inner = last[0] + last[1];
 			out.n_leaf	= last[2] + last[3];
-			HIPC(hipMalloc(&gsize, sizeof(uint32_t) * (size_t(out.n_inner) + 1)));
+			HIPC(hipMalloc(&gsize, sizeof(uint32_t) * (size_t(out.n_inner) + 5)));
 			HIPC(hipMalloc(&gbase, sizeof(uint32_t) * (size_t(out.n_inner) + 1)));
 			HIPC(hipMalloc(&inner_unit, sizeof(uint32_t) * std::max<size_t>(out.n_inner, 1)));
 			HIPC(hipMalloc(&out.leaf_units, sizeof(uint32_t) * std::max<size_t>(out.n_leaf, 1)));
@@ -1036,14 +1054,19 @@
 							   inner_unit, out.leaf_units);
 			hipLaunchKernelGGL(k_emit_inner, dim3(G), dim3(B), 0, stream, (int)n, width, wv, vals_sorted, left, right, rf, rl, boxes, inner_flag, inner_idx, leaf_idx, gbase,
 							   inner_unit, out.recs);
-			hipLaunchKernelGGL(k_emit_leaves, dim3(G), dim3(B), 0, stream, n, wv, vals_sorted, leaf_flag, leaf_cnt, leaf_idx, out.leaf_units, out.recs, in.tri_class);
+			HIPC(hipMemsetAsync(gsize, 0, 5 * sizeof(uint32_t), stream));
+			hipLaunchKernelGGL(k_emit_leaves, dim3(G), dim3(B), 0, stream, n, wv, vals_sorted, leaf_flag, leaf_cnt, leaf_idx, out.leaf_units, out.recs, in.tri_class, gsize);
 			HIPC(hipGetLastError());
+			if (in.corrupt_leaf_count)
+				hipLaunchKernelGGL(k_corrupt_leaf_count, dim3((out.n_inner + B - 1) / B), dim3(B), 0, stream, out.n_inner, inner_unit, out.recs, gsize + 4);
 			{
-				uint32_t bad = 0;
-				HIPC(hipMemsetAsync(gsize, 0, sizeof(uint32_t), stream));
+				uint32_t chk[4] = { 0u, 0u, 0u, 0u };
 				hipLaunchKernelGGL(k_validate, dim3((out.n_inner + B - 1) / B), dim3(B), 0, stream, out.n_inner, inner_unit, out.recs, out.n_units, gsize);
-				HIPC(hipMemcpyAsync(&bad, gsize, 4, hipMemcpyDeviceToHost, stream));
+				HIPC(hipMemcpyAsync(chk, gsize, sizeof(chk), hipMemcpyDeviceToHost, stream));
 				HIPC(hipStreamSynchronize(stream));
+				const uint32_t bad = chk[0];
+				for (int k = 0; k < 3; ++k)
+					out.leaf_fill[k] = chk[1 + k];
 				if (bad != 0u) {
 					err = "internal error: " + std::to_string(bad) + " inner records failed the structure check";
 					goto done;
diff --git a/pearray_amd/csrc/device/pr_device.h b/pearray_amd/csrc/device/pr_device.h
--- a/pearray_amd/csrc/device/pr_device.h
+++ b/pearray_amd/csrc/device/pr_device.h
@@ -34,6 +34,7 @@
 constexpr float CIE_DELTA	   = CIE_RANGE / (CIE_SAMPLES - 1);
 constexpr float CIE_Y_NORM	   = CIE_Y_NORM_SUM * CIE_DELTA;
 
+constexpr uint32_t REC_FORMAT_VERSION = 10u;
 struct __attribute__((aligned(64))) Rec64 {
 	float4 q[4];
 };
@@ -41,10 +42,13 @@
 constexpr uint32_t REC_LEAF_BIT = 1u;
 constexpr uint32_t REC_EMPTY	= 0xFFFFFFFFu;
 constexpr uint32_t REC_UNIT_SHIFT = 2u;
-__host__ __device__ __forceinline__ const float4* rec_ptr(const Rec64* recs, uint32_t ref)
-{
-	return reinterpret_cast<const float4*>(reinterpret_cast<const char*>(recs) + (size_t(ref & ~3u) << 4));
-}
+constexpr uint32_t REC_COUNT_SHIFT = 1u, REC_COUNT_BITS = 3u << REC_COUNT_SHIFT;
+constexpr uint32_t REC_INNER_ADDR = ~3u, REC_LEAF_ADDR = ~(3u | REC_COUNT_BITS);
+__host__ __device__ __forceinline__ const float4* rec_ptr(const Rec64* recs, uint32_t ref, uint32_t addr = REC_INNER_ADDR)
+{
+	return reinterpret_cast<const float4*>(reinterpret_cast<const char*>(recs) + (size_t(ref & addr) << 4));
+}
+__host__ __device__ __forceinline__ uint32_t leaf_ref_count(uint32_t ref) { return ((ref & REC_COUNT_BITS) >> REC_COUNT_SHIFT) + 1u; }
 constexpr float SLAB_REL		= 1.0000028610229492f;
 constexpr float INV_D_MAX		= 1.2089258196146292e24f;
 constexpr float SCENE_COORD_MAX = 268435456.0f;
diff --git a/pearray_amd/csrc/device/render.h b/pearray_amd/csrc/device/render.h
--- a/pearray_amd/csrc/device/render.h
+++ b/pearray_amd/csrc/device/render.h
@@ -2,7 +2,7 @@
 #include "pr_device.h"
 
 namespace prd {
-constexpr int N_DEVICE_COUNTERS = PRGPU_STAT_COUNT + 30;
+constexpr int N_DEVICE_COUNTERS = PRGPU_STAT_COUNT + 32;
 
 struct TraceWorkspace {
 	uint32_t* queue_head = nullptr;
diff --git a/pearray_amd/csrc/device/render.hip b/pearray_amd/csrc/device/render.hip
--- a/pearray_amd/csrc/device/render.hip
+++ b/pearray_amd/csrc/device/render.hip
@@ -25,7 +25,7 @@
 };
 
 enum { CNT_NODES_CLOSEST = PRGPU_STAT_COUNT, CNT_TRIS_CLOSEST, CNT_NODES_ANY, CNT_TRIS_ANY, CNT_WAVE_ITERS_CLOSEST, CNT_WAVE_ITERS_ANY, CNT_SHADE_BATCHES, CNT_SHADE_LANES, CNT_SHADE_TICKS, CNT_IDLE_TICKS, CNT_TOTAL_TICKS, CNT_LEAF_TICKS, CNT_INNER_TICKS, CNT_TOTAL_CYCLES, CNT_REFILL_TICKS, CNT_FIN_TICKS, CNT_CAMERA_TICKS, CNT_VERTEX_TICKS,
-	   CNT_CLS_TICKS0, CNT_CLS_BATCHES0 = CNT_CLS_TICKS0 + 4, CNT_CLS_LANES0 = CNT_CLS_BATCHES0 + 4 };
+	   CNT_CLS_TICKS0, CNT_CLS_BATCHES0 = CNT_CLS_TICKS0 + 4, CNT_CLS_LANES0 = CNT_CLS_BATCHES0 + 4, CNT_LEAVES_1TRI = CNT_CLS_LANES0 + 4, CNT_LEAVES_2TRI };
 
 #ifndef PR_PEEK
 #define PR_PEEK 0
@@ -205,14 +205,29 @@
 	trav_inner_rec<M>(s, st, q0, q1, q2, q3, wide, &top);
 }
 
+__device__ __forceinline__ void leaf_fetch_tail(const float4* __restrict__ rec, uint32_t ref, float4& q3, float4& q4, float4& q5, float4& q6, float4& q7)
+{
+	float z;
+	asm("v_mov_b32 %0, 0" : "=v"(z));
+	q3 = q4 = q5 = q6 = q7 = make_float4(z, z, z, z);
+	if ((ref & REC_COUNT_BITS) != 0u) {
+		q3 = rec[3];
+		q4 = rec[4];
+	}
+	if ((ref & (2u << REC_COUNT_SHIFT)) != 0u) {
+		q5 = rec[5];
+		q6 = rec[6];
+		q7 = rec[7];
+	}
+}
 template <int M, bool SPH, bool CLS = false>
-__device__ __forceinline__ void leaf_test(Trav& s, const float4& q0, const float4& q1, const float4& q2, const float4& q3, const float4& q4, const float4& q5,
-										  const float4& q6, const float4& q7)
+__device__ __forceinline__ void leaf_test(Trav& s, uint32_t count, const float4* __restrict__ rec, const float4& q0, const float4& q1, const float4& q2, const float4& q3,
+										  const float4& q4, const float4& q5, const float4& q6, const float4& q7)
 {
 	const bool ANY = M == MODE_ANY || (M == MODE_MIXED && s.any);
 	const float f[32] = { q0.x, q0.y, q0.z, q0.w, q1.x, q1.y, q1.z, q1.w, q2.x, q2.y, q2.z, q2.w, q3.x, q3.y, q3.z, q3.w,
 						  q4.x, q4.y, q4.z, q4.w, q5.x, q5.y, q5.z, q5.w, q6.x, q6.y, q6.z, q6.w, q7.x, q7.y, q7.z, q7.w };
-	const uint32_t count = __float_as_uint(f[30]);
+	int won = -1;
 #pragma unroll
 	for (int k = 0; k < 3; ++k) {
 		if ((uint32_t)k < count) {
@@ -235,18 +250,21 @@
 				} else if (t < s.best.t || (t == s.best.t && tri < s.best.tri)) {
 					s.best = Hit{ t, u, v, tri };
 					if (CLS)
-						s.cls = (__float_as_uint(f[31]) >> (8 * k)) & 0xFFu;
+						won = k;
 				}
 			}
 		}
 	}
+	if (CLS && won >= 0)
+		s.cls = (__float_as_uint(reinterpret_cast<const float*>(rec)[31]) >> (8 * won)) & 0xFFu;
 }
 template <int M, bool SPH, bool CLS = false, typename STK>
-__device__ __forceinline__ void trav_leaf_rec(Trav& s, STK& st, const float4& q0, const float4& q1, const float4& q2, const float4& q3, const float4& q4,
-											  const float4& q5, const float4& q6, const float4& q7, const uint2* top = nullptr)
+__device__ __forceinline__ void trav_leaf_rec(Trav& s, STK& st, const float4* __restrict__ rec, const float4& q0, const float4& q1, const float4& q2, const uint2* top = nullptr)
 {
 	const bool ANY = M == MODE_ANY || (M == MODE_MIXED && s.any);
-	leaf_test<M, SPH, CLS>(s, q0, q1, q2, q3, q4, q5, q6, q7);
+	float4 q3, q4, q5, q6, q7;
+	leaf_fetch_tail(rec, s.cur, q3, q4, q5, q6, q7);
+	leaf_test<M, SPH, CLS>(s, leaf_ref_count(s.cur), rec, q0, q1, q2, q3, q4, q5, q6, q7);
 	s.cur = REC_EMPTY;
 	if (ANY && s.best.tri != INVALID) {
 		st.reset();
@@ -257,10 +275,10 @@
 template <int M>
 __device__ __forceinline__ void trav_leaf(const DevScene& sc, Trav& s, Stack& st)
 {
-	const float4* __restrict__ rec = rec_ptr(sc.recs, s.cur);
-	const float4 q0 = rec[0], q1 = rec[1], q2 = rec[2], q3 = rec[3], q4 = rec[4], q5 = rec[5], q6 = rec[6], q7 = rec[7];
+	const float4* __restrict__ rec = rec_ptr(sc.recs, s.cur, REC_LEAF_ADDR);
+	const float4 q0 = rec[0], q1 = rec[1], q2 = rec[2];
 	const uint2 top = st.peek();
-	trav_leaf_rec<M, true>(s, st, q0, q1, q2, q3, q4, q5, q6, q7, &top);
+	trav_leaf_rec<M, true>(s, st, rec, q0, q1, q2, &top);
 }
 
 template <bool CLS>
@@ -2264,6 +2282,7 @@
 	uint32_t spins	  = 0;
 	unsigned long long t_idle_since = 0;
 	uint32_t cn_c = 0, cl_c = 0, cn_a = 0, cl_a = 0, witers = 0, wleaf = 0, sbatches = 0, slanes = 0;
+	uint32_t cl_fill[2] = { 0u, 0u };
 	unsigned long long t_shade = 0, t_idle = 0, t_leaf = 0, t_inner = 0, t_refill = 0, t_fin = 0, t_cam = 0, t_vert = 0;
 	unsigned long long t_cls[4] = { 0, 0, 0, 0 };
 	uint32_t b_cls[4] = { 0, 0, 0, 0 }, l_cls[4] = { 0, 0, 0, 0 };
@@ -2569,7 +2588,7 @@
 			const bool do_inner = n_inner >= n_leaf;
 			const unsigned long long t0s = COUNT ? wall_clock64() : 0ull;
 			if (lane_in(do_inner ? m_inner : m_leaf)) {
-				const float4* __restrict__ rec = rec_ptr(sc.recs, s.cur);
+				const float4* __restrict__ rec = rec_ptr(sc.recs, s.cur, do_inner ? REC_INNER_ADDR : REC_LEAF_ADDR);
 				const float4 q0 = rec[0], q1 = rec[1], q2 = rec[2];
 				const bool wide = WIDE == 2 ? sc.bvh_wide != 0u : WIDE == 1;
 				float4 qw		= make_float4(0.0f, 0.0f, 0.0f, 0.0f);
@@ -2584,12 +2603,13 @@
 					}
 					trav_inner_rec<MODE_MIXED>(s, st, q0, q1, q2, qw, wide, top);
 				} else {
-					const float4 q3 = rec[3], q4 = rec[4], q5 = rec[5], q6 = rec[6], q7 = rec[7];
 					if (COUNT) {
 						cl_c += s.any ? 0 : 1;
 						cl_a += s.any ? 1 : 0;
+						cl_fill[0] += leaf_ref_count(s.cur) == 1u ? 1u : 0u;
+						cl_fill[1] += leaf_ref_count(s.cur) == 2u ? 1u : 0u;
 					}
-					trav_leaf_rec<MODE_MIXED, (FEATS & FEAT_SPHERES) != 0, (NQ > 1)>(s, st, q0, q1, q2, q3, q4, q5, q6, q7, top);
+					trav_leaf_rec<MODE_MIXED, (FEATS & FEAT_SPHERES) != 0, (NQ > 1)>(s, st, rec, q0, q1, q2, top);
 				}
 			}
 			if (COUNT) {
@@ -2668,6 +2688,10 @@
 			atomicAdd(&a.gstats[CNT_NODES_ANY], (unsigned long long)cn_a);
 		if (cl_a)
 			atomicAdd(&a.gstats[CNT_TRIS_ANY], (unsigned long long)cl_a);
+		if (cl_fill[0])
+			atomicAdd(&a.gstats[CNT_LEAVES_1TRI], (unsigned long long)cl_fill[0]);
+		if (cl_fill[1])
+			atomicAdd(&a.gstats[CNT_LEAVES_2TRI], (unsigned long long)cl_fill[1]);
 		if (witers)
 			atomicAdd(&a.gstats[CNT_WAVE_ITERS_CLOSEST], (unsigned long long)witers);
 		if (wleaf)
@@ -2775,7 +2799,7 @@
 #pragma unroll
 			for (int k = 0; k < NW; ++k)
 				if (lf[k])
-					__hip_atomic_store(&q[(pos++) & (SQ - 1u)], (((base + (key[k] & 0xFFu)) >> REC_UNIT_SHIFT) << 8) | tid, __ATOMIC_RELEASE, __HIP_MEMORY_SCOPE_WORKGROUP);
+					__hip_atomic_store(&q[(pos++) & (SQ - 1u)], (((base + (key[k] & 0xFFu)) >> 1) << 8) | tid, __ATOMIC_RELEASE, __HIP_MEMORY_SCOPE_WORKGROUP);
 		}
 	}
 	if (!active)
@@ -2862,7 +2886,7 @@
 			return false;
 		if (lane < nt) {
 			const uint32_t task	 = ring_take(sh.q, SQ - 1u, first + lane);
-			const uint32_t owner = task & 0xFFu, unit = task >> 8;
+			const uint32_t owner = task & 0xFFu, ref = (task >> 8) << 1;
 			RayPre r;
 			const float4 ra = sh.rc[0][owner], rb = sh.rc[1][owner];
 			r.o				  = v3(ra.x, ra.y, ra.z);
@@ -2874,11 +2898,13 @@
 			r.Sy			  = rb.y;
 			r.Sz			  = rb.z;
 			const float tmin  = rb.w;
-			const float4* __restrict__ rec = reinterpret_cast<const float4*>(sc.recs + unit);
-			const float4 q0 = rec[0], q1 = rec[1], q2 = rec[2], q3 = rec[3], q4 = rec[4], q5 = rec[5], q6 = rec[6], q7 = rec[7];
+			const float4* __restrict__ rec = rec_ptr(sc.recs, ref, REC_LEAF_ADDR);
+			const float4 q0 = rec[0], q1 = rec[1], q2 = rec[2];
+			float4 q3, q4, q5, q6, q7;
+			leaf_fetch_tail(rec, ref, q3, q4, q5, q6, q7);
 			const float f[32] = { q0.x, q0.y, q0.z, q0.w, q1.x, q1.y, q1.z, q1.w, q2.x, q2.y, q2.z, q2.w, q3.x, q3.y, q3.z, q3.w,
 								  q4.x, q4.y, q4.z, q4.w, q5.x, q5.y, q5.z, q5.w, q6.x, q6.y, q6.z, q6.w, q7.x, q7.y, q7.z, q7.w };
-			const uint32_t count = __float_as_uint(f[30]);
+			const uint32_t count = leaf_ref_count(ref);
 			unsigned long long key = ~0ull;
 #pragma unroll
 			for (int k = 0; k < 3; ++k) {
diff --git a/pearray_amd/csrc/prgpu_api.hip b/pearray_amd/csrc/prgpu_api.hip
--- a/pearray_amd/csrc/prgpu_api.hip
+++ b/pearray_amd/csrc/prgpu_api.hip
@@ -179,6 +179,7 @@
 	std::vector<void*> allocations;
 	uint32_t bvh_units = 0;
 	uint32_t bvh_stack_bound = 0, bvh_top = 0;
+	uint32_t bvh_leaf_fill[3] = { 0u, 0u, 0u };
 	float bvh_cost4 = 0.0f, bvh_cost6 = 0.0f;
 	int pp_shader_waves = -1;
 	double pp_shading_share = 0.0;
@@ -564,6 +565,7 @@
 	bin.width = s->knobs.bvh_width;
 	bin.top	  = s->knobs.bvh_top;
 	bin.parity = s->knobs.bvh_parity;
+	bin.corrupt_leaf_count = (s->knobs.force_features & 0x80000000u) != 0u;
 	bin.stack_capacity = prd::trace_stack_capacity();
 	prd::BvhBuildOutput bout;
 	{
@@ -581,6 +583,8 @@
 	s->bvh_cost6 = bout.cost6;
 	s->bvh_stack_bound = bout.stack_bound;
 	s->bvh_top = (uint32_t)bout.top;
+	for (int k = 0; k < 3; ++k)
+		s->bvh_leaf_fill[k] = bout.leaf_fill[k];
 	sc.n_leaf  = bout.n_leaf;
 	s->bvh_units = bout.n_units;
 	{
@@ -1454,6 +1458,8 @@
 	out->shade_ticks		= host[PRGPU_STAT_COUNT + 8];
 	out->idle_ticks			= host[PRGPU_STAT_COUNT + 9];
 	out->total_ticks		= host[PRGPU_STAT_COUNT + 10];
+	out->leaves_1tri		= host[PRGPU_STAT_COUNT + 30];
+	out->leaves_2tri		= host[PRGPU_STAT_COUNT + 31];
 	if (read_knobs().debug_counters)
 		if (host[PRGPU_STAT_COUNT + 10]) {
 			const double T = double(host[PRGPU_STAT_COUNT + 10]);
@@ -1548,7 +1554,7 @@
 	TRY_OR_CLEAN(hipMemcpyAsync(d_tmax, tmax, size_t(n) * 4, hipMemcpyHostToDevice, s->stream));
 	s->time_begin(1, s->stream);
 	const bool split = read_knobs().trace_split;
-	if (split && s->sc.n_leaf > 0 && s->bvh_units < (1u << 24) && !(s->sc.features & (prd::FEAT_SPHERES | prd::FEAT_QUADRICS))) {
+	if (split && s->sc.n_leaf > 0 && s->bvh_units < (1u << 23) && !(s->sc.features & (prd::FEAT_SPHERES | prd::FEAT_QUADRICS))) {
 		prd::launch_service_closest_split(s->sc, n, d_org, d_dir, d_tmin, d_tmax, d_e, d_p, d_u, d_v, d_t, s->ws, const_cast<uint32_t*>(s->sc.tri_slot), s->gstats, s->stream);
 	} else
 		prd::launch_service_closest(s->sc, n, d_org, d_dir, d_tmin, d_tmax, d_e, d_p, d_u, d_v, d_t, s->ws, s->gstats, s->stream);
@@ -1868,6 +1874,8 @@
 	out->bvh_cost_6_wide = s->bvh_cost6;
 	out->bvh_stack_bound = s->bvh_stack_bound;
 	out->bvh_top		 = s->bvh_top;
+	for (int k = 0; k < 3; ++k)
+		out->bvh_leaf_fill[k] = s->bvh_leaf_fill[k];
 	return PRGPU_OK;
 }
 
```

Result: slower. 209.9 Msamples/s (-2.0%).
